# mikemey/cellcomm

Hardware: NVIDIA B200
Metric: BiGAN train cells/sec (higher is better)
Workload: dtype bf16

## Files before the change

cellcomm_b200/csrc/common.cuh:

```cuda
#pragma once
#include <cuda_bf16.h>
#include <cuda_runtime.h>
#include <stdint.h>

#include <atomic>
#include <cstdarg>
#include <cstdio>
#include <string>

#include "../../include/cellcomm_b200.h"

namespace cc {

void set_error(const char* fmt, ...);
extern std::atomic<long long> g_launches;

inline void count_launch(int n = 1) { g_launches.fetch_add(n, std::memory_order_relaxed); }

#define CC_CHECK_CUDA(expr)                                                            \
  do {                                                                                 \
    cudaError_t _e = (expr);                                                           \
    if (_e != cudaSuccess) {                                                           \
      cc::set_error("%s failed: %s (%s:%d)", #expr, cudaGetErrorString(_e), __FILE__,  \
                    __LINE__);                                                         \
      return -2;                                                                       \
    }                                                                                  \
  } while (0)

#define CC_REQUIRE(cond, ...)      \
  do {                             \
    if (!(cond)) {                 \
      cc::set_error(__VA_ARGS__);  \
      return -1;                   \
    }                              \
  } while (0)

#define CC_CHECK_LAUNCH()               \
  do {                                  \
    cc::count_launch();                 \
    CC_CHECK_CUDA(cudaGetLastError());  \
  } while (0)

typedef __nv_bfloat16 bf16;

__device__ __forceinline__ float bf2f(bf16 v) { return __bfloat162float(v); }
__device__ __forceinline__ bf16 f2bf(float v) { return __float2bfloat16_rn(v); }

__device__ __forceinline__ float sigmoidf_(float x) { return 1.f / (1.f + __expf(-x)); }

struct Philox {
  static constexpr uint32_t kM0 = 0xD2511F53u, kM1 = 0xCD9E8D57u;
  static constexpr uint32_t kW0 = 0x9E3779B9u, kW1 = 0xBB67AE85u;
  __host__ __device__ static inline void round(uint32_t (&c)[4], uint32_t k0, uint32_t k1) {
    uint64_t p0 = (uint64_t)kM0 * c[0];
    uint64_t p1 = (uint64_t)kM1 * c[2];
    uint32_t hi0 = (uint32_t)(p0 >> 32), lo0 = (uint32_t)p0;
    uint32_t hi1 = (uint32_t)(p1 >> 32), lo1 = (uint32_t)p1;
    uint32_t n0 = hi1 ^ c[1] ^ k0;
    uint32_t n2 = hi0 ^ c[3] ^ k1;
    c[0] = n0;
    c[1] = lo1;
    c[2] = n2;
    c[3] = lo0;
  }
  __host__ __device__ static inline void block(uint64_t seed, uint64_t ctr_hi, uint64_t ctr_lo,
                                               uint32_t (&out)[4]) {
    uint32_t c[4] = {(uint32_t)ctr_lo, (uint32_t)(ctr_lo >> 32), (uint32_t)ctr_hi,
                     (uint32_t)(ctr_hi >> 32)};
    uint32_t k0 = (uint32_t)seed, k1 = (uint32_t)(seed >> 32);
#pragma unroll
    for (int i = 0; i < 10; ++i) {
      round(c, k0, k1);
      k0 += kW0;
      k1 += kW1;
    }
    out[0] = c[0];
    out[1] = c[1];
    out[2] = c[2];
    out[3] = c[3];
  }
};

__host__ __device__ inline float u32_to_unit(uint32_t x) { return (float)(x >> 8) * (1.0f / 16777216.0f); }

}
```

cellcomm_b200/csrc/gather.cu:

```cuda
#include "common.cuh"

namespace cc {

constexpr int GATHER_THREADS = 256;

__global__ void __launch_bounds__(GATHER_THREADS)
gather_rows_kernel(const long long* __restrict__ rowptr, const int* __restrict__ colidx,
                   const float* __restrict__ values, const long long* __restrict__ row_idx,
                   long long row_start, long long n_rows, long long n_cols,
                   bf16* __restrict__ out16, long long ld16, float* __restrict__ out32,
                   long long ld32, int use_smem) {
  extern __shared__ __align__(16) unsigned char smem[];
  bf16* srow = reinterpret_cast<bf16*>(smem);
  const int tid = threadIdx.x;
  for (long long i = blockIdx.x; i < n_rows; i += gridDim.x) {
    const long long r = row_idx ? row_idx[i] : row_start + i;
    const long long beg = rowptr[r], end = rowptr[r + 1];
    if (out16 != nullptr) {
      bf16* orow = out16 + i * ld16;
      if (use_smem) {
        const long long nvec = n_cols / 8, nz = (n_cols + 7) / 8;
        uint4* s4 = reinterpret_cast<uint4*>(srow);
        for (long long v = tid; v < nz; v += GATHER_THREADS) s4[v] = make_uint4(0, 0, 0, 0);
        __syncthreads();
        for (long long e = beg + tid; e < end; e += GATHER_THREADS)
          srow[colidx[e]] = f2bf(values[e]);
        __syncthreads();
        uint4* o4 = reinterpret_cast<uint4*>(orow);
        for (long long v = tid; v < nvec; v += GATHER_THREADS) o4[v] = s4[v];
        for (long long c = nvec * 8 + tid; c < n_cols; c += GATHER_THREADS) orow[c] = srow[c];
        __syncthreads();
      } else {
        for (long long c = tid; c < n_cols; c += GATHER_THREADS) orow[c] = f2bf(0.f);
        __syncthreads();
        for (long long e = beg + tid; e < end; e += GATHER_THREADS)
          orow[colidx[e]] = f2bf(values[e]);
        __syncthreads();
      }
    }
    if (out32 != nullptr) {
      float* orow = out32 + i * ld32;
      for (long long c = tid; c < n_cols; c += GATHER_THREADS) orow[c] = 0.f;
      __syncthreads();
      for (long long e = beg + tid; e < end; e += GATHER_THREADS) orow[colidx[e]] = values[e];
      __syncthreads();
    }
  }
}

}

extern "C" int cc_gather_rows(const int64_t* rowptr_dev, const int32_t* colidx_dev,
                              const float* values_dev, const int64_t* row_idx_dev,
                              int64_t row_start, int64_t n_rows, int64_t n_cols, void* out16,
                              int64_t ld16, float* out32, int64_t ld32, cc_stream_t stream) {
  using namespace cc;
  if (n_rows <= 0) return 0;
  CC_REQUIRE(out16 == nullptr || ld16 >= n_cols, "cc_gather_rows: ld16 %lld < cols %lld",
             (long long)ld16, (long long)n_cols);
  CC_REQUIRE(out32 == nullptr || ld32 >= n_cols, "cc_gather_rows: ld32 %lld < cols %lld",
             (long long)ld32, (long long)n_cols);
  static int sms = 0, max_smem = 0;
  if (sms == 0) {
    int dev = 0;
    CC_CHECK_CUDA(cudaGetDevice(&dev));
    CC_CHECK_CUDA(cudaDeviceGetAttribute(&sms, cudaDevAttrMultiProcessorCount, dev));
    CC_CHECK_CUDA(cudaDeviceGetAttribute(&max_smem, cudaDevAttrMaxSharedMemoryPerBlockOptin, dev));
    CC_CHECK_CUDA(cudaFuncSetAttribute(gather_rows_kernel,
                                       cudaFuncAttributeMaxDynamicSharedMemorySize, max_smem));
  }
  size_t smem = 0;
  int use_smem = 0;
  if (out16 != nullptr && ld16 % 8 == 0 && (((uintptr_t)out16) & 15) == 0 &&
      (size_t)(n_cols + 7) / 8 * 16 <= (size_t)max_smem) {
    use_smem = 1;
    smem = (size_t)(n_cols + 7) / 8 * 16;
  }
  long long grid = n_rows;
  const long long cap = (long long)sms * 16;
  if (grid > cap) grid = cap;
  gather_rows_kernel<<<(unsigned)grid, GATHER_THREADS, smem, (cudaStream_t)stream>>>(
      (const long long*)rowptr_dev, colidx_dev, values_dev, (const long long*)row_idx_dev,
      row_start, n_rows, n_cols, (bf16*)out16, ld16, out32, ld32, use_smem);
  CC_CHECK_LAUNCH();
  return 0;
}
```

cellcomm_b200/csrc/gemm_sm100.cu:

```cuda
#include <cuda.h>

#include <mutex>
#include <unordered_map>

#include "common.cuh"

namespace cc {

constexpr int BM = 128;
constexpr int BK = 64;
constexpr int UMMA_K = 16;
constexpr int MAX_SEG = CC_GEMM_MAX_SEG;

struct EpiParams {
  int M, N;
  float alpha;
  const float* bias;
  int act;
  const bf16* dact_y;
  long long ld_dact;
  int dact;
  bf16* out16;
  long long ld16;
  int beta16;
  bf16* out16_lo;
  long long ld16_lo;
  float* out32;
  long long ld32;
  int beta32;
  float* rms_p32;
  float* rms_ms;
  float* rms_mom;
  bf16* rms_p16;
  long long rms_ld;
  float rms_lr, rms_rho, rms_momentum, rms_eps;
  int rms_cs;
  int rms_blocked;
  int rms_row0;
  bf16* rms_p16lo;
  int rms_keep_operands;
  int route_world;
  unsigned int route_shard;
  long long route_off0;
  float* route_base[CC_PEER_MAX];
};

struct GemmParams {
  EpiParams epi;
  int nseg;
  int kblocks[MAX_SEG];
  int total_kblocks;
  int kb_per_split;
  int psplits;
  float* partial;
  long long partial_ld;
  long long partial_stride;
  unsigned long long adesc_hi, bdesc_hi;
  unsigned int a_kstep, b_kstep;
  unsigned int idesc;
  int bn_eff;
  int b_boxes;
  int b_half_rows;
  int cluster;
  int pair;
  unsigned int stage_tx;
};

struct TmaMaps {
  CUtensorMap a[MAX_SEG];
  CUtensorMap b[MAX_SEG];
};

__device__ __forceinline__ uint32_t smem_u32(const void* p) {
  return (uint32_t)__cvta_generic_to_shared(p);
}
__device__ __forceinline__ void mbar_init(uint32_t bar, uint32_t count) {
  asm volatile("mbarrier.init.shared::cta.b64 [%0], %1;" ::"r"(bar), "r"(count));
}
__device__ __forceinline__ void mbar_expect_tx(uint32_t bar, uint32_t bytes) {
  asm volatile("mbarrier.arrive.expect_tx.shared::cta.b64 _, [%0], %1;" ::"r"(bar), "r"(bytes)
               : "memory");
}
__device__ __forceinline__ bool mbar_try_wait(uint32_t bar, uint32_t parity) {
  uint32_t ok;
  asm volatile(
      "{\n\t.reg .pred p;\n\t"
      "mbarrier.try_wait.parity.shared::cta.b64 p, [%1], %2;\n\t"
      "selp.u32 %0, 1, 0, p;\n\t}"
      : "=r"(ok)
      : "r"(bar), "r"(parity)
      : "memory");
  return ok != 0;
}
__device__ __forceinline__ void mbar_wait(uint32_t bar, uint32_t parity, int tag) {
  long long t0 = 0;
  uint32_t spins = 0;
  while (!mbar_try_wait(bar, parity)) {
    if (++spins == 4096u) t0 = clock64();
    if (spins > 4096u && (spins & 1023u) == 0 && clock64() - t0 > 4000000000LL) {
      printf("cc_gemm: mbarrier timeout tag=%d block=(%d,%d,%d) thread=%d parity=%u\n", tag,
             blockIdx.x, blockIdx.y, blockIdx.z, threadIdx.x, parity);
      __trap();
    }
  }
}
__device__ __forceinline__ void tma_load_2d(uint32_t dst, const CUtensorMap* map, uint32_t bar,
                                            int c0, int c1) {
  asm volatile(
      "cp.async.bulk.tensor.2d.shared::cluster.global.mbarrier::complete_tx::bytes [%0], [%1, "
      "{%3, %4}], [%2];" ::"r"(dst),
      "l"(map), "r"(bar), "r"(c0), "r"(c1)
      : "memory");
}
__device__ __forceinline__ void tcgen05_fence_before() {
  asm volatile("tcgen05.fence::before_thread_sync;" ::: "memory");
}
__device__ __forceinline__ void tcgen05_fence_after() {
  asm volatile("tcgen05.fence::after_thread_sync;" ::: "memory");
}
__device__ __forceinline__ void umma_bf16(uint32_t tmem_d, uint64_t adesc, uint64_t bdesc,
                                          uint32_t idesc, uint32_t accumulate) {
  asm volatile(
      "{\n\t.reg .pred p;\n\t"
      "setp.ne.b32 p, %4, 0;\n\t"
      "tcgen05.mma.cta_group::1.kind::f16 [%0], %1, %2, %3, p;\n\t}" ::"r"(tmem_d),
      "l"(adesc), "l"(bdesc), "r"(idesc), "r"(accumulate)
      : "memory");
}
__device__ __forceinline__ void umma_commit(uint32_t bar) {
  asm volatile("tcgen05.commit.cta_group::1.mbarrier::arrive::one.shared::cluster.b64 [%0];" ::"r"(
                   bar)
               : "memory");
}
__device__ __forceinline__ void tmem_ld32(uint32_t taddr, uint32_t (&r)[32]) {
  asm volatile(
      "tcgen05.ld.sync.aligned.32x32b.x32.b32 "
      "{%0, %1, %2, %3, %4, %5, %6, %7, %8, %9, %10, %11, %12, %13, %14, %15, "
      "%16, %17, %18, %19, %20, %21, %22, %23, %24, %25, %26, %27, %28, %29, %30, %31}, [%32];"
      : "=r"(r[0]), "=r"(r[1]), "=r"(r[2]), "=r"(r[3]), "=r"(r[4]), "=r"(r[5]), "=r"(r[6]),
        "=r"(r[7]), "=r"(r[8]), "=r"(r[9]), "=r"(r[10]), "=r"(r[11]), "=r"(r[12]), "=r"(r[13]),
        "=r"(r[14]), "=r"(r[15]), "=r"(r[16]), "=r"(r[17]), "=r"(r[18]), "=r"(r[19]),
        "=r"(r[20]), "=r"(r[21]), "=r"(r[22]), "=r"(r[23]), "=r"(r[24]), "=r"(r[25]),
        "=r"(r[26]), "=r"(r[27]), "=r"(r[28]), "=r"(r[29]), "=r"(r[30]), "=r"(r[31])
      : "r"(taddr));
}
__device__ __forceinline__ void tmem_ld_wait() {
  asm volatile("tcgen05.wait::ld.sync.aligned;" ::: "memory");
}

__device__ __forceinline__ bool elect_one() {
  uint32_t pred;
  asm volatile(
      "{\n\t.reg .pred p;\n\t"
      "elect.sync _|p, 0xffffffff;\n\t"
      "selp.u32 %0, 1, 0, p;\n\t}"
      : "=r"(pred));
  return pred != 0;
}

__device__ __forceinline__ void epilogue_store32(const EpiParams& e, int r, int c0, float (&v)[32]) {
  if (r >= e.M) return;
  const int ncols = min(32, e.N - c0);
  if (ncols <= 0) return;
#pragma unroll
  for (int j = 0; j < 32; ++j) {
    float x = v[j] * e.alpha;
    if (e.bias != nullptr && j < ncols) x += __ldg(e.bias + c0 + j);
    if (e.act == CC_ACT_SIGMOID) x = sigmoidf_(x);
    else if (e.act == CC_ACT_RELU) x = fmaxf(x, 0.f);
    v[j] = x;
  }
  if (e.dact != 0) {
    const bf16* yrow = e.dact_y + (long long)r * e.ld_dact + c0;
#pragma unroll
    for (int j = 0; j < 32; ++j) {
      if (j < ncols) {
        float y = bf2f(yrow[j]);
        v[j] *= (e.dact == CC_ACT_SIGMOID) ? y * (1.f - y) : (y > 0.f ? 1.f : 0.f);
      }
    }
  }
  if (e.out32 != nullptr) {
    float* o = e.out32 + (long long)r * e.ld32 + c0;
    if (ncols == 32 && (((uintptr_t)o) & 15) == 0 && !e.beta32) {
#pragma unroll
      for (int j = 0; j < 32; j += 4)
        *reinterpret_cast<float4*>(o + j) = make_float4(v[j], v[j + 1], v[j + 2], v[j + 3]);
    } else {
#pragma unroll
      for (int j = 0; j < 32; ++j)
        if (j < ncols) o[j] = e.beta32 ? o[j] + v[j] : v[j];
    }
  }
  if (e.out16 != nullptr) {
    bf16* o = e.out16 + (long long)r * e.ld16 + c0;
    if (ncols == 32 && (((uintptr_t)o) & 15) == 0 && !e.beta16) {
#pragma unroll
      for (int j = 0; j < 32; j += 8) {
        __nv_bfloat162 p0 = __floats2bfloat162_rn(v[j], v[j + 1]);
        __nv_bfloat162 p1 = __floats2bfloat162_rn(v[j + 2], v[j + 3]);
        __nv_bfloat162 p2 = __floats2bfloat162_rn(v[j + 4], v[j + 5]);
        __nv_bfloat162 p3 = __floats2bfloat162_rn(v[j + 6], v[j + 7]);
        uint4 u;
        u.x = *reinterpret_cast<uint32_t*>(&p0);
        u.y = *reinterpret_cast<uint32_t*>(&p1);
        u.z = *reinterpret_cast<uint32_t*>(&p2);
        u.w = *reinterpret_cast<uint32_t*>(&p3);
        *reinterpret_cast<uint4*>(o + j) = u;
      }
    } else {
#pragma unroll
      for (int j = 0; j < 32; ++j)
        if (j < ncols) o[j] = f2bf(e.beta16 ? bf2f(o[j]) + v[j] : v[j]);
    }
    if (e.out16_lo != nullptr) {
      bf16* l = e.out16_lo + (long long)r * e.ld16_lo + c0;
#pragma unroll
      for (int j = 0; j < 32; ++j)
        if (j < ncols) l[j] = f2bf(v[j] - bf2f(f2bf(v[j])));
    }
  }
}

constexpr int EPI_LD = 36;

__device__ __forceinline__ float4 act4(float4 v, int act) {
  if (act == CC_ACT_SIGMOID) {
// ... 136 lines not shown
          if (e.rms_cs & 1) {
            __stcs(reinterpret_cast<float4*>(e.rms_ms + off), ss);
            __stcs(reinterpret_cast<float4*>(e.rms_mom + off), mm);
            __stcs(reinterpret_cast<float4*>(e.rms_p32 + off), ww);
          } else {
            *reinterpret_cast<float4*>(e.rms_ms + off) = ss;
            *reinterpret_cast<float4*>(e.rms_mom + off) = mm;
            *reinterpret_cast<float4*>(e.rms_p32 + off) = ww;
          }
          if (e.rms_p16 != nullptr) {
            __nv_bfloat162 lo = __floats2bfloat162_rn(ww.x, ww.y);
            __nv_bfloat162 hi = __floats2bfloat162_rn(ww.z, ww.w);
            uint2 u;
            u.x = *reinterpret_cast<uint32_t*>(&lo);
            u.y = *reinterpret_cast<uint32_t*>(&hi);
            *reinterpret_cast<uint2*>(e.rms_p16 + off) = u;
          }
        }
      }
    } else {
      for_each_valid(g, nrow, ncol, [&](int t, int k, float& gv) {
        const long long off = off0 + t * step + k;
        const float ms = e.rms_rho * e.rms_ms[off] + (1.f - e.rms_rho) * gv * gv;
        const float mo = e.rms_momentum * e.rms_mom[off] + e.rms_lr * gv * rsqrtf(ms + e.rms_eps);
        const float w = e.rms_p32[off] - mo;
        e.rms_ms[off] = ms;
        e.rms_mom[off] = mo;
        e.rms_p32[off] = w;
        if (e.rms_p16 != nullptr) e.rms_p16[off] = f2bf(w);
      });
    }
  }
  if (e.route_world > 0) {
    const long long rel0 = e.route_off0 + (long long)rbase * e.ld32 + c;
    const long long step = 4 * e.ld32;
    const unsigned last = (unsigned)e.route_world - 1u;
    const bool vec = ncol == 4 && (e.ld32 & 3) == 0 && ((c & 3) == 0);
#pragma unroll
    for (int t = 0; t < 8; ++t) {
      if (t < nrow) {
        const long long rel = rel0 + t * step;
        const unsigned owner = min((unsigned)((unsigned long long)rel / e.route_shard), last);
        float* dst = e.route_base[owner] + rel;
        if (vec) {
          *reinterpret_cast<float4*>(dst) = g[t];
        } else {
          dst[0] = g[t].x;
          if (ncol > 1) dst[1] = g[t].y;
          if (ncol > 2) dst[2] = g[t].z;
          if (ncol > 3) dst[3] = g[t].w;
        }
      }
    }
  } else if (e.out32 != nullptr) {
    float* o = e.out32 + out32_off + (long long)rbase * e.ld32 + c;
    const long long step = 4 * e.ld32;
    if (ncol == 4 && !e.beta32 && (e.ld32 & 3) == 0 && ((c & 3) == 0) &&
        ((((uintptr_t)e.out32) & 15) == 0)) {
#pragma unroll
      for (int t = 0; t < 8; ++t)
        if (t < nrow) *reinterpret_cast<float4*>(o + t * step) = g[t];
    } else {
      const int beta = e.beta32;
      for_each_valid(g, nrow, ncol, [&](int t, int k, float& gv) {
        float* ot = o + t * step + k;
        *ot = beta ? *ot + gv : gv;
      });
    }
  }
  if (e.out16 != nullptr) {
    bf16* o = e.out16 + (long long)rbase * e.ld16 + c;
    const long long step = 4 * e.ld16;
    if (ncol == 4 && !e.beta16 && (e.ld16 & 3) == 0 && ((c & 3) == 0) &&
        ((((uintptr_t)e.out16) & 7) == 0)) {
#pragma unroll
      for (int t = 0; t < 8; ++t) {
        if (t < nrow) {
          __nv_bfloat162 lo = __floats2bfloat162_rn(g[t].x, g[t].y);
          __nv_bfloat162 hi = __floats2bfloat162_rn(g[t].z, g[t].w);
          uint2 u;
          u.x = *reinterpret_cast<uint32_t*>(&lo);
          u.y = *reinterpret_cast<uint32_t*>(&hi);
          *reinterpret_cast<uint2*>(o + t * step) = u;
        }
      }
    } else {
      const int beta = e.beta16;
      for_each_valid(g, nrow, ncol, [&](int t, int k, float& gv) {
        bf16* ot = o + t * step + k;
        *ot = f2bf(beta ? bf2f(*ot) + gv : gv);
      });
    }
    if (e.out16_lo != nullptr) {
      bf16* l = e.out16_lo + (long long)rbase * e.ld16_lo + c;
      const long long lstep = 4 * e.ld16_lo;
      if (ncol == 4 && (e.ld16_lo & 3) == 0 && ((c & 3) == 0) && ((((uintptr_t)e.out16_lo) & 7) == 0)) {
#pragma unroll
        for (int t = 0; t < 8; ++t) {
          if (t < nrow) {
            const float4 v = g[t];
            __nv_bfloat162 lo = __floats2bfloat162_rn(v.x - bf2f(f2bf(v.x)), v.y - bf2f(f2bf(v.y)));
            __nv_bfloat162 hi = __floats2bfloat162_rn(v.z - bf2f(f2bf(v.z)), v.w - bf2f(f2bf(v.w)));
            uint2 u;
            u.x = *reinterpret_cast<uint32_t*>(&lo);
            u.y = *reinterpret_cast<uint32_t*>(&hi);
            *reinterpret_cast<uint2*>(l + t * lstep) = u;
          }
        }
      } else {
        for_each_valid(g, nrow, ncol, [&](int t, int k, float& gv) {
          l[t * lstep + k] = f2bf(gv - bf2f(f2bf(gv)));
        });
      }
    }
  }
}

template <int BN, int STAGES, bool A_MN, bool B_MN>
__global__ void __launch_bounds__(128, 2)
gemm_tcgen05_kernel(const __grid_constant__ TmaMaps maps, const GemmParams p) {
  constexpr uint32_t A_BYTES = BM * BK * 2;
  constexpr uint32_t B_BYTES = BN * BK * 2;
  constexpr uint32_t STAGE_BYTES = A_BYTES + B_BYTES;
  constexpr uint32_t TMEM_COLS = BN;

  extern __shared__ uint8_t smem_raw[];
  const uint32_t smem_base = (smem_u32(smem_raw) + 1023u) & ~1023u;
  const uint32_t bar_base = smem_base + STAGES * STAGE_BYTES;
  auto full_bar = [&](int s) { return bar_base + 8u * s; };
  auto empty_bar = [&](int s) { return bar_base + 8u * (STAGES + s); };
  const uint32_t tmem_full_bar = bar_base + 8u * (2 * STAGES);
  const uint32_t tmem_slot = bar_base + 8u * (2 * STAGES + 1);
  uint8_t* smem_gen = smem_raw + (smem_base - smem_u32(smem_raw));
  volatile uint32_t* tmem_slot_ptr =
      reinterpret_cast<volatile uint32_t*>(smem_gen + STAGES * STAGE_BYTES + 8u * (2 * STAGES + 1));

  const int warp = threadIdx.x >> 5;
  const int lane = threadIdx.x & 31;
  const int m0 = blockIdx.y * BM;
  const int n0 = blockIdx.x * BN;
  const int kb_begin = blockIdx.z * p.kb_per_split;
  const int kb_end = min(p.total_kblocks, kb_begin + p.kb_per_split);
  const int nkb = kb_end - kb_begin;

  if (threadIdx.x == 0) {
#pragma unroll
    for (int s = 0; s < STAGES; ++s) {
      mbar_init(full_bar(s), 1);
      mbar_init(empty_bar(s), 1);
    }
    mbar_init(tmem_full_bar, 1);
    asm volatile("fence.mbarrier_init.release.cluster;" ::: "memory");
    asm volatile("fence.proxy.async.shared::cta;" ::: "memory");
  }
  if (warp == 1) {
    asm volatile("tcgen05.alloc.cta_group::1.sync.aligned.shared::cta.b32 [%0], %1;" ::"r"(tmem_slot),
                 "r"(TMEM_COLS)
                 : "memory");
    asm volatile("tcgen05.relinquish_alloc_permit.cta_group::1.sync.aligned;" ::: "memory");
  }
  tcgen05_fence_before();
  __syncthreads();
  tcgen05_fence_after();
  const uint32_t tmem_acc = *tmem_slot_ptr;

  if (warp == 0) {
    int seg = 0, kb_in_seg = kb_begin;
    while (seg < p.nseg - 1 && kb_in_seg >= p.kblocks[seg]) {
      kb_in_seg -= p.kblocks[seg];
      ++seg;
    }
    for (int i = 0; i < nkb; ++i) {
      const int s = i % STAGES;
      const uint32_t ph = (uint32_t)(i / STAGES) & 1u;
      mbar_wait(empty_bar(s), ph ^ 1u, 1);
      if (elect_one()) {
        const uint32_t a_dst = smem_base + s * STAGE_BYTES;
        const uint32_t b_dst = a_dst + A_BYTES;
        const int k0 = kb_in_seg * BK;
        mbar_expect_tx(full_bar(s), STAGE_BYTES);
        if (A_MN) {
#pragma unroll
          for (int j = 0; j < BM / 64; ++j)
            tma_load_2d(a_dst + j * (64 * BK * 2), &maps.a[seg], full_bar(s), m0 + 64 * j, k0);
        } else {
          tma_load_2d(a_dst, &maps.a[seg], full_bar(s), k0, m0);
        }
        if (B_MN) {
#pragma unroll
          for (int j = 0; j < BN / 64; ++j)
            tma_load_2d(b_dst + j * (64 * BK * 2), &maps.b[seg], full_bar(s), n0 + 64 * j, k0);
        } else {
          tma_load_2d(b_dst, &maps.b[seg], full_bar(s), k0, n0);
        }
      }
      __syncwarp();
      if (++kb_in_seg >= p.kblocks[seg] && seg < p.nseg - 1) {
        kb_in_seg = 0;
        ++seg;
      }
    }
  } else if (warp == 1) {
    for (int i = 0; i < nkb; ++i) {
      const int s = i % STAGES;
      const uint32_t ph = (uint32_t)(i / STAGES) & 1u;
      mbar_wait(full_bar(s), ph, 2);
      tcgen05_fence_after();
      if (elect_one()) {
        const uint32_t a_src = smem_base + s * STAGE_BYTES;
        const uint32_t b_src = a_src + A_BYTES;
#pragma unroll
        for (int k = 0; k < BK / UMMA_K; ++k) {
          const uint64_t adesc = p.adesc_hi | (uint64_t)(((a_src + k * p.a_kstep) & 0x3FFFFu) >> 4);
          const uint64_t bdesc = p.bdesc_hi | (uint64_t)(((b_src + k * p.b_kstep) & 0x3FFFFu) >> 4);
          umma_bf16(tmem_acc, adesc, bdesc, p.idesc, (i > 0 || k > 0) ? 1u : 0u);
        }
        umma_commit(empty_bar(s));
        if (i == nkb - 1) umma_commit(tmem_full_bar);
      }
      __syncwarp();
    }
  }

  mbar_wait(tmem_full_bar, 0, 3);
  tcgen05_fence_after();
  {
    const int r = m0 + warp * 32 + lane;
    const uint32_t t_row = tmem_acc + ((uint32_t)(warp * 32) << 16);
    const bool split = (p.partial != nullptr);
#pragma unroll 1
    for (int c = 0; c < BN; c += 32) {
      if (n0 + c >= p.epi.N) break;
      uint32_t raw[32];
      tmem_ld32(t_row + (uint32_t)c, raw);
      tmem_ld_wait();
      float v[32];
#pragma unroll
      for (int j = 0; j < 32; ++j) v[j] = __uint_as_float(raw[j]);
      if (split) {
        if (r < p.epi.M) {
          float* o = p.partial + (long long)blockIdx.z * p.partial_stride +
                     (long long)r * p.partial_ld + n0 + c;
#pragma unroll
          for (int j = 0; j < 32; j += 4)
            *reinterpret_cast<float4*>(o + j) = make_float4(v[j], v[j + 1], v[j + 2], v[j + 3]);
        }
      } else {
        epilogue_store32(p.epi, r, n0 + c, v);
      }
    }
  }
  tcgen05_fence_before();
  __syncthreads();
  if (warp == 1) {
    asm volatile("tcgen05.dealloc.cta_group::1.sync.aligned.b32 %0, %1;" ::"r"(tmem_acc),
                 "r"(TMEM_COLS)
                 : "memory");
  }
}

__device__ __forceinline__ void mbar_arrive(uint32_t bar) {
  asm volatile("mbarrier.arrive.shared::cta.b64 _, [%0];" ::"r"(bar) : "memory");
}
__device__ __forceinline__ uint32_t cluster_ctarank() {
  uint32_t r;
  asm volatile("mov.u32 %0, %%cluster_ctarank;" : "=r"(r));
  return r;
}
__device__ __forceinline__ void cluster_sync_all() {
  asm volatile("barrier.cluster.arrive.release.aligned;" ::: "memory");
  asm volatile("barrier.cluster.wait.acquire.aligned;" ::: "memory");
}
__device__ __forceinline__ void tma_load_2d_mc(uint32_t dst, const CUtensorMap* map, uint32_t bar,
                                               int c0, int c1, uint16_t mask) {
  asm volatile(
      "cp.async.bulk.tensor.2d.shared::cluster.global.mbarrier::complete_tx::bytes"
      ".multicast::cluster [%0], [%1, {%3, %4}], [%2], %5;" ::"r"(dst),
      "l"(map), "r"(bar), "r"(c0), "r"(c1), "h"(mask)
      : "memory");
}
__device__ __forceinline__ uint64_t l2_policy_evict_last() {
  uint64_t pol;
  asm volatile("createpolicy.fractional.L2::evict_last.b64 %0, 1.0;" : "=l"(pol));
  return pol;
}
__device__ __forceinline__ void tma_load_2d_pol(uint32_t dst, const CUtensorMap* map, uint32_t bar,
                                                int c0, int c1, uint64_t pol) {
  asm volatile(
      "cp.async.bulk.tensor.2d.shared::cluster.global.mbarrier::complete_tx::bytes.L2::cache_hint "
      "[%0], [%1, {%3, %4}], [%2], %5;" ::"r"(dst),
      "l"(map), "r"(bar), "r"(c0), "r"(c1), "l"(pol)
      : "memory");
}
__device__ __forceinline__ void tma_load_2d_mc_pol(uint32_t dst, const CUtensorMap* map,
                                                   uint32_t bar, int c0, int c1, uint16_t mask,
                                                   uint64_t pol) {
  asm volatile(
      "cp.async.bulk.tensor.2d.shared::cluster.global.mbarrier::complete_tx::bytes"
      ".multicast::cluster.L2::cache_hint [%0], [%1, {%3, %4}], [%2], %5, %6;" ::"r"(dst),
      "l"(map), "r"(bar), "r"(c0), "r"(c1), "h"(mask), "l"(pol)
      : "memory");
}
__device__ __forceinline__ void umma_commit_mc(uint32_t bar, uint16_t mask) {
  asm volatile(
      "tcgen05.commit.cta_group::1.mbarrier::arrive::one.shared::cluster.multicast::cluster.b64 "
      "[%0], %1;" ::"r"(bar),
      "h"(mask)
      : "memory");
}

__device__ __forceinline__ uint32_t mapa_cluster(uint32_t local, uint32_t cta) {
  uint32_t r;
  asm volatile("mapa.shared::cluster.u32 %0, %1, %2;" : "=r"(r) : "r"(local), "r"(cta));
  return r;
}
__device__ __forceinline__ void mbar_arrive_cluster(uint32_t cluster_addr) {
  asm volatile("mbarrier.arrive.release.cluster.shared::cluster.b64 _, [%0];" ::"r"(cluster_addr)
// ... 10 lines not shown
__device__ __forceinline__ void umma_bf16_pair(uint32_t tmem_d, uint64_t adesc, uint64_t bdesc,
                                               uint32_t idesc, uint32_t accumulate) {
  asm volatile(
      "{\n\t.reg .pred p;\n\t"
      "setp.ne.b32 p, %4, 0;\n\t"
      "tcgen05.mma.cta_group::2.kind::f16 [%0], %1, %2, %3, p;\n\t}" ::"r"(tmem_d),
      "l"(adesc), "l"(bdesc), "r"(idesc), "r"(accumulate)
      : "memory");
}
__device__ __forceinline__ void umma_commit_pair(uint32_t bar, uint16_t mask) {
  asm volatile(
      "tcgen05.commit.cta_group::2.mbarrier::arrive::one.shared::cluster.multicast::cluster.b64 "
      "[%0], %1;" ::"r"(bar),
      "h"(mask)
      : "memory");
}

__device__ __forceinline__ void rms_blocked_chunk(const EpiParams& e, int lane, int r0, int c0,
                                                  const uint32_t (&raw)[32]) {
  const int r = r0 + lane;
  if (r >= e.M) return;
  const int row = e.rms_row0 + r;
  const long long sb =
      ((long long)(row >> 5) * (e.rms_ld >> 5) + (c0 >> 5)) * 1024 + (long long)(row & 31) * 4;
  float* pw = e.rms_p32 + sb;
  float* ps = e.rms_ms + sb;
  float* pm = e.rms_mom + sb;
  float4 w[8], s[8], m[8];
#pragma unroll
  for (int t = 0; t < 8; ++t) {
    w[t] = __ldcs(reinterpret_cast<const float4*>(pw + t * 128));
    s[t] = __ldcs(reinterpret_cast<const float4*>(ps + t * 128));
    m[t] = __ldcs(reinterpret_cast<const float4*>(pm + t * 128));
  }
  const float rho = e.rms_rho, omr = 1.f - e.rms_rho, mu = e.rms_momentum, lr = e.rms_lr,
              eps = e.rms_eps;
  const int nvalid = e.N - c0;
  uint32_t h[16], hl[16];
#pragma unroll
  for (int t = 0; t < 8; ++t) {
    float g0 = (4 * t + 0 < nvalid) ? __uint_as_float(raw[4 * t + 0]) : 0.f;
    float g1 = (4 * t + 1 < nvalid) ? __uint_as_float(raw[4 * t + 1]) : 0.f;
    float g2 = (4 * t + 2 < nvalid) ? __uint_as_float(raw[4 * t + 2]) : 0.f;
    float g3 = (4 * t + 3 < nvalid) ? __uint_as_float(raw[4 * t + 3]) : 0.f;
    float4 ss, mm, ww;
    ss.x = rho * s[t].x + omr * g0 * g0;
    ss.y = rho * s[t].y + omr * g1 * g1;
    ss.z = rho * s[t].z + omr * g2 * g2;
    ss.w = rho * s[t].w + omr * g3 * g3;
    mm.x = mu * m[t].x + lr * g0 * rsqrtf(ss.x + eps);
    mm.y = mu * m[t].y + lr * g1 * rsqrtf(ss.y + eps);
    mm.z = mu * m[t].z + lr * g2 * rsqrtf(ss.z + eps);
    mm.w = mu * m[t].w + lr * g3 * rsqrtf(ss.w + eps);
    ww.x = w[t].x - mm.x;
    ww.y = w[t].y - mm.y;
    ww.z = w[t].z - mm.z;
    ww.w = w[t].w - mm.w;
    __stcs(reinterpret_cast<float4*>(ps + t * 128), ss);
    __stcs(reinterpret_cast<float4*>(pm + t * 128), mm);
    __stcs(reinterpret_cast<float4*>(pw + t * 128), ww);
    __nv_bfloat162 lo = __floats2bfloat162_rn(ww.x, ww.y);
    __nv_bfloat162 hi = __floats2bfloat162_rn(ww.z, ww.w);
    h[2 * t] = *reinterpret_cast<uint32_t*>(&lo);
    h[2 * t + 1] = *reinterpret_cast<uint32_t*>(&hi);
    if (e.rms_p16lo != nullptr) {
      __nv_bfloat162 l0 = __floats2bfloat162_rn(ww.x - __uint_as_float(h[2 * t] << 16),
                                                ww.y - __uint_as_float(h[2 * t] & 0xFFFF0000u));
      __nv_bfloat162 l1 = __floats2bfloat162_rn(ww.z - __uint_as_float(h[2 * t + 1] << 16),
                                                ww.w - __uint_as_float(h[2 * t + 1] & 0xFFFF0000u));
      hl[2 * t] = *reinterpret_cast<uint32_t*>(&l0);
      hl[2 * t + 1] = *reinterpret_cast<uint32_t*>(&l1);
    }
    if (e.out32 != nullptr)
      *reinterpret_cast<float4*>(e.out32 + (long long)r * e.ld32 + c0 + 4 * t) =
          make_float4(g0, g1, g2, g3);
  }
  if (e.rms_p16 != nullptr) {
    uint4* dst = reinterpret_cast<uint4*>(e.rms_p16 + (long long)r * e.rms_ld + c0);
#pragma unroll
    for (int t = 0; t < 4; ++t) dst[t] = make_uint4(h[4 * t], h[4 * t + 1], h[4 * t + 2], h[4 * t + 3]);
  }
  if (e.rms_p16lo != nullptr) {
    uint4* dst = reinterpret_cast<uint4*>(e.rms_p16lo + (long long)r * e.rms_ld + c0);
#pragma unroll
    for (int t = 0; t < 4; ++t)
      dst[t] = make_uint4(hl[4 * t], hl[4 * t + 1], hl[4 * t + 2], hl[4 * t + 3]);
  }
}

template <int BN, int STAGES, bool A_MN, bool B_MN, bool MATH, int EPI_WARPS, bool N_FAST = false,
          int CLUSTER = 1, bool PAIR = false, bool RMS_DIRECT = false>
__global__ void __launch_bounds__(64 + 32 * EPI_WARPS, 1)
gemm_tcgen05_persistent_kernel(const __grid_constant__ TmaMaps maps,
                               const __grid_constant__ GemmParams p,
                               const int tiles_m, const int tiles_n) {
  static_assert(!PAIR || CLUSTER == 2, "a CTA pair is a cluster of two");
  constexpr uint32_t A_BYTES = BM * BK * 2;
  constexpr uint32_t B_BYTES = (PAIR ? BN / 2 : BN) * BK * 2;
  constexpr uint32_t STAGE_BYTES = A_BYTES + B_BYTES;
  constexpr uint32_t TMEM_COLS = 2 * BN;
  static_assert(TMEM_COLS <= 512, "TMEM has 512 columns");
  static_assert(CLUSTER == 1 || CLUSTER == 2, "cluster of 1 or 2 CTAs");

  extern __shared__ uint8_t smem_raw[];
  const uint32_t smem_base = (smem_u32(smem_raw) + 1023u) & ~1023u;
  const uint32_t bar_base = smem_base + STAGES * STAGE_BYTES;
  auto full_bar = [&](int s) { return bar_base + 8u * s; };
  auto empty_bar = [&](int s) { return bar_base + 8u * (STAGES + s); };
  auto tfull_bar = [&](int a) { return bar_base + 8u * (2 * STAGES + a); };
  auto tempty_bar = [&](int a) { return bar_base + 8u * (2 * STAGES + 2 + a); };
  const uint32_t tmem_slot = bar_base + 8u * (2 * STAGES + 4);
  uint8_t* smem_gen = smem_raw + (smem_base - smem_u32(smem_raw));
  volatile uint32_t* tmem_slot_ptr =
      reinterpret_cast<volatile uint32_t*>(smem_gen + STAGES * STAGE_BYTES + 8u * (2 * STAGES + 4));
  float* epi_stage = reinterpret_cast<float*>(smem_gen + STAGES * STAGE_BYTES + 8u * (2 * STAGES + 6));

  const int warp = threadIdx.x >> 5;
  const int lane = threadIdx.x & 31;
  const int nkb = p.total_kblocks;
  const int rank = (CLUSTER == 2) ? (int)cluster_ctarank() : 0;
  const int tiles_mu = (tiles_m + CLUSTER - 1) / CLUSTER;
  const int num_tiles = tiles_mu * tiles_n;
  const int psplits = p.psplits > 1 ? p.psplits : 1;
  const int num_units = num_tiles * psplits;
  const int unit0 = (int)blockIdx.x / CLUSTER, unit_step = (int)gridDim.x / CLUSTER;
  auto unit_tile = [&](int u) { return psplits > 1 ? u % num_tiles : u; };
  auto unit_split = [&](int u) { return psplits > 1 ? u / num_tiles : 0; };
  auto unit_m0 = [&](int u) {
    const int t = unit_tile(u);
    return ((N_FAST ? t / tiles_n : t % tiles_mu) * CLUSTER + rank) * BM;
  };
  auto unit_n0 = [&](int u) {
    const int t = unit_tile(u);
    return (N_FAST ? t % tiles_n : t / tiles_mu) * p.bn_eff;
  };
  auto unit_kb0 = [&](int u) { return unit_split(u) * p.kb_per_split; };
  auto unit_nkb = [&](int u) {
    return psplits > 1 ? min(p.kb_per_split, p.total_kblocks - unit_kb0(u)) : p.total_kblocks;
  };

  if (threadIdx.x == 0) {
#pragma unroll
    for (int s = 0; s < STAGES; ++s) {
      mbar_init(full_bar(s), PAIR ? 2 : 1);
      mbar_init(empty_bar(s), PAIR ? 1 : CLUSTER);
    }
#pragma unroll
    for (int a = 0; a < 2; ++a) {
      mbar_init(tfull_bar(a), 1);
      mbar_init(tempty_bar(a), PAIR ? 2 * EPI_WARPS : EPI_WARPS);
    }
    asm volatile("fence.mbarrier_init.release.cluster;" ::: "memory");
    asm volatile("fence.proxy.async.shared::cta;" ::: "memory");
  }
  if (warp == 1) {
    if (PAIR) {
      asm volatile("tcgen05.alloc.cta_group::2.sync.aligned.shared::cta.b32 [%0], %1;" ::"r"(tmem_slot),
                   "r"(TMEM_COLS)
                   : "memory");
      asm volatile("tcgen05.relinquish_alloc_permit.cta_group::2.sync.aligned;" ::: "memory");
    } else {
      asm volatile("tcgen05.alloc.cta_group::1.sync.aligned.shared::cta.b32 [%0], %1;" ::"r"(tmem_slot),
                   "r"(TMEM_COLS)
                   : "memory");
      asm volatile("tcgen05.relinquish_alloc_permit.cta_group::1.sync.aligned;" ::: "memory");
    }
  }
  tcgen05_fence_before();
  __syncthreads();
  if (CLUSTER == 2) cluster_sync_all();
  tcgen05_fence_after();
  const uint32_t tmem_acc = *tmem_slot_ptr;

  if (warp == 0 && PAIR) {
    uint32_t it = 0;
    const int half = p.bn_eff / 2;
    for (int u = unit0; u < num_units; u += unit_step) {
      const int m0 = unit_m0(u), n0 = unit_n0(u) + rank * half;
      int seg = 0, kb_in_seg = 0;
      for (int i = 0; i < nkb; ++i, ++it) {
        const int s = it % STAGES;
        const uint32_t ph = (it / STAGES) & 1u;
        mbar_wait(empty_bar(s), ph ^ 1u, 11);
        if (elect_one()) {
          const uint32_t a_dst = smem_base + s * STAGE_BYTES;
          const uint32_t b_dst = a_dst + A_BYTES;
          const uint32_t lbar = mapa_cluster(full_bar(s), 0);
          const int k0 = kb_in_seg * BK;
          if (rank == 0) mbar_expect_tx(full_bar(s), 2 * p.stage_tx);
          else mbar_arrive_cluster(lbar);
          if (A_MN) {
#pragma unroll
            for (int j = 0; j < BM / 64; ++j)
              tma_load_2d_pair(a_dst + j * (64 * BK * 2), &maps.a[seg], lbar, m0 + 64 * j, k0);
          } else {
            tma_load_2d_pair(a_dst, &maps.a[seg], lbar, k0, m0);
          }
          if (B_MN) {
#pragma unroll
            for (int j = 0; j < BN / 128; ++j)
              if (j < p.b_boxes)
                tma_load_2d_pair(b_dst + j * (64 * BK * 2), &maps.b[seg], lbar, n0 + 64 * j, k0);
          } else {
            tma_load_2d_pair(b_dst, &maps.b[seg], lbar, k0, n0);
          }
        }
        __syncwarp();
        if (++kb_in_seg >= p.kblocks[seg] && seg < p.nseg - 1) {
          kb_in_seg = 0;
          ++seg;
        }
      }
    }
  } else if (warp == 0) {
    uint32_t it = 0;
    const uint64_t keep = (RMS_DIRECT && p.epi.rms_keep_operands) ? l2_policy_evict_last() : 0;
    for (int u = unit0; u < num_units; u += unit_step) {
      const int m0 = unit_m0(u), n0 = unit_n0(u);
      const int nkb_u = unit_nkb(u);
      int seg = 0, kb_in_seg = unit_kb0(u);
      while (seg < p.nseg - 1 && kb_in_seg >= p.kblocks[seg]) {
        kb_in_seg -= p.kblocks[seg];
        ++seg;
      }
      for (int i = 0; i < nkb_u; ++i, ++it) {
        const int s = it % STAGES;
        const uint32_t ph = (it / STAGES) & 1u;
        mbar_wait(empty_bar(s), ph ^ 1u, 11);
        if (elect_one()) {
          const uint32_t a_dst = smem_base + s * STAGE_BYTES;
          const uint32_t b_dst = a_dst + A_BYTES;
          const int k0 = kb_in_seg * BK;
          mbar_expect_tx(full_bar(s), p.stage_tx);
          if (RMS_DIRECT && A_MN && B_MN && keep != 0) {
#pragma unroll
            for (int j = 0; j < BM / 64; ++j)
              tma_load_2d_pol(a_dst + j * (64 * BK * 2), &maps.a[seg], full_bar(s), m0 + 64 * j, k0,
                              keep);
#pragma unroll
            for (int j = 0; j < BN / 64; ++j) {
              if (j >= p.b_boxes) continue;
              if (CLUSTER == 2) {
                if ((j & 1) == rank)
                  tma_load_2d_mc_pol(b_dst + j * (64 * BK * 2), &maps.b[seg], full_bar(s),
                                     n0 + 64 * j, k0, (uint16_t)3, keep);
              } else {
                tma_load_2d_pol(b_dst + j * (64 * BK * 2), &maps.b[seg], full_bar(s), n0 + 64 * j,
                                k0, keep);
              }
            }
          } else if (A_MN) {
#pragma unroll
            for (int j = 0; j < BM / 64; ++j)
              tma_load_2d(a_dst + j * (64 * BK * 2), &maps.a[seg], full_bar(s), m0 + 64 * j, k0);
          } else {
            tma_load_2d(a_dst, &maps.a[seg], full_bar(s), k0, m0);
          }
          if (RMS_DIRECT && A_MN && B_MN && keep != 0) {
          } else if (CLUSTER == 2) {
            if (B_MN) {
#pragma unroll
              for (int j = 0; j < BN / 64; ++j)
                if (j < p.b_boxes && (j & 1) == rank)
                  tma_load_2d_mc(b_dst + j * (64 * BK * 2), &maps.b[seg], full_bar(s), n0 + 64 * j,
                                 k0, (uint16_t)3);
            } else {
              tma_load_2d_mc(b_dst + rank * p.b_half_rows * (BK * 2), &maps.b[seg], full_bar(s), k0,
                             n0 + rank * p.b_half_rows, (uint16_t)3);
            }
          } else if (B_MN) {
#pragma unroll
            for (int j = 0; j < BN / 64; ++j)
              if (j < p.b_boxes)
                tma_load_2d(b_dst + j * (64 * BK * 2), &maps.b[seg], full_bar(s), n0 + 64 * j, k0);
          } else {
            tma_load_2d(b_dst, &maps.b[seg], full_bar(s), k0, n0);
          }
        }
        __syncwarp();
        if (++kb_in_seg >= p.kblocks[seg] && seg < p.nseg - 1) {
          kb_in_seg = 0;
          ++seg;
        }
      }
    }
  } else if (warp == 1) {
    uint32_t it = 0, tl = 0;
    for (int u = unit0; (!PAIR || rank == 0) && u < num_units; u += unit_step, ++tl) {
      const uint32_t acc = tl & 1u, aph = (tl >> 1) & 1u;
      mbar_wait(tempty_bar(acc), aph ^ 1u, 12);
      tcgen05_fence_after();
      const uint32_t d_tmem = tmem_acc + acc * BN;
      const int nkb = unit_nkb(u);
      for (int i = 0; i < nkb; ++i, ++it) {
        const int s = it % STAGES;
        const uint32_t ph = (it / STAGES) & 1u;
        mbar_wait(full_bar(s), ph, 13);
        tcgen05_fence_after();
        if (elect_one()) {
          const uint32_t a_src = smem_base + s * STAGE_BYTES;
          const uint32_t b_src = a_src + A_BYTES;
#pragma unroll
          for (int k = 0; k < BK / UMMA_K; ++k) {
            const uint64_t adesc = p.adesc_hi | (uint64_t)(((a_src + k * p.a_kstep) & 0x3FFFFu) >> 4);
            const uint64_t bdesc = p.bdesc_hi | (uint64_t)(((b_src + k * p.b_kstep) & 0x3FFFFu) >> 4);
            if (PAIR) umma_bf16_pair(d_tmem, adesc, bdesc, p.idesc, (i > 0 || k > 0) ? 1u : 0u);
            else umma_bf16(d_tmem, adesc, bdesc, p.idesc, (i > 0 || k > 0) ? 1u : 0u);
          }
          if (PAIR) {
            umma_commit_pair(empty_bar(s), (uint16_t)3);
            if (i == nkb - 1) umma_commit_pair(tfull_bar(acc), (uint16_t)3);
          } else {
            if (CLUSTER == 2) umma_commit_mc(empty_bar(s), (uint16_t)3);
            else umma_commit(empty_bar(s));
            if (i == nkb - 1) umma_commit(tfull_bar(acc));
          }
        }
        __syncwarp();
      }
    }
  } else {
    const int q = warp & 3;
    const int ew = warp - 2;
    constexpr int COLS_PER_WARP = BN / (EPI_WARPS / 4);
    const int col_lo = (ew >> 2) * COLS_PER_WARP;
    uint32_t tl = 0;
    for (int u = unit0; u < num_units; u += unit_step, ++tl) {
      const int m0 = unit_m0(u), n0 = unit_n0(u);
      const uint32_t acc = tl & 1u, aph = (tl >> 1) & 1u;
      mbar_wait(tfull_bar(acc), aph, 14);
      tcgen05_fence_after();
      const uint32_t t_row = tmem_acc + ((uint32_t)(q * 32) << 16) + acc * BN;
      if (m0 < p.epi.M) {
#pragma unroll 1
        for (int c = col_lo; c < col_lo + COLS_PER_WARP; c += 32) {
          if (c >= p.bn_eff || n0 + c >= p.epi.N) break;
          uint32_t raw[32];
          tmem_ld32(t_row + (uint32_t)c, raw);
          tmem_ld_wait();
          if constexpr (RMS_DIRECT) rms_blocked_chunk(p.epi, lane, m0 + q * 32, n0 + c, raw);
          else epilogue_chunk<MATH>(p.epi, epi_stage + ew * (32 * EPI_LD), lane, m0 + q * 32, n0 + c, raw,
                                    (long long)unit_split(u) * p.partial_stride);
        }
      }
      tcgen05_fence_before();
      __syncwarp();
      if (lane == 0) {
        if (PAIR) mbar_arrive_cluster(mapa_cluster(tempty_bar(acc), 0));
        else mbar_arrive(tempty_bar(acc));
      }
    }
  }
  tcgen05_fence_before();
  __syncthreads();
  if (CLUSTER == 2) cluster_sync_all();
  if (warp == 1) {
    if (PAIR)
      asm volatile("tcgen05.dealloc.cta_group::2.sync.aligned.b32 %0, %1;" ::"r"(tmem_acc),
                   "r"(TMEM_COLS)
                   : "memory");
    else
      asm volatile("tcgen05.dealloc.cta_group::1.sync.aligned.b32 %0, %1;" ::"r"(tmem_acc),
                   "r"(TMEM_COLS)
                   : "memory");
  }
}

}
#include "wgrad_rmsprop_kernel.cuh"
namespace cc {

__global__ void splitk_finalize_kernel(const EpiParams e, const float* __restrict__ partial,
                                       long long partial_ld, long long partial_stride, int splits) {
  const int groups = (e.N + 3) / 4;
  const long long idx = (long long)blockIdx.x * blockDim.x + threadIdx.x;
  if (idx >= (long long)e.M * groups) return;
  const int r = (int)(idx / groups);
  const int c0 = (int)(idx % groups) * 4;
  const float* src = partial + (long long)r * partial_ld + c0;
  float4 a = make_float4(0.f, 0.f, 0.f, 0.f);
  for (int s0 = 0; s0 < splits; s0 += 8) {
    float4 q[8];
#pragma unroll
    for (int u = 0; u < 8; ++u)
      q[u] = (s0 + u < splits)
                 ? __ldcs(reinterpret_cast<const float4*>(src + (long long)(s0 + u) * partial_stride))
                 : make_float4(0.f, 0.f, 0.f, 0.f);
#pragma unroll
    for (int u = 0; u < 8; ++u) {
      if (s0 + u < splits) {
        a.x += q[u].x;
        a.y += q[u].y;
        a.z += q[u].z;
        a.w += q[u].w;
      }
    }
  }
  float v[4] = {a.x, a.y, a.z, a.w};
  const int ncols = min(4, e.N - c0);
#pragma unroll
  for (int j = 0; j < 4; ++j) {
    float x = v[j] * e.alpha;
    if (e.bias != nullptr && j < ncols) x += __ldg(e.bias + c0 + j);
    if (e.act == CC_ACT_SIGMOID) x = sigmoidf_(x);
    else if (e.act == CC_ACT_RELU) x = fmaxf(x, 0.f);
    v[j] = x;
  }
  if (e.dact != 0) {
    const bf16* yrow = e.dact_y + (long long)r * e.ld_dact + c0;
#pragma unroll
    for (int j = 0; j < 4; ++j) {
      if (j < ncols) {
        const float y = bf2f(yrow[j]);
        v[j] *= (e.dact == CC_ACT_SIGMOID) ? y * (1.f - y) : (y > 0.f ? 1.f : 0.f);
      }
    }
  }
  if (e.out32 != nullptr) {
    float* o = e.out32 + (long long)r * e.ld32 + c0;
    if (ncols == 4 && (((uintptr_t)o) & 15) == 0 && !e.beta32) {
      *reinterpret_cast<float4*>(o) = make_float4(v[0], v[1], v[2], v[3]);
    } else {
#pragma unroll
      for (int j = 0; j < 4; ++j)
        if (j < ncols) o[j] = e.beta32 ? o[j] + v[j] : v[j];
    }
  }
  if (e.out16 != nullptr) {
    bf16* o = e.out16 + (long long)r * e.ld16 + c0;
    if (ncols == 4 && (((uintptr_t)o) & 7) == 0 && !e.beta16) {
      __nv_bfloat162 p0 = __floats2bfloat162_rn(v[0], v[1]);
      __nv_bfloat162 p1 = __floats2bfloat162_rn(v[2], v[3]);
      uint2 u;
      u.x = *reinterpret_cast<uint32_t*>(&p0);
      u.y = *reinterpret_cast<uint32_t*>(&p1);
      *reinterpret_cast<uint2*>(o) = u;
    } else {
#pragma unroll
      for (int j = 0; j < 4; ++j)
        if (j < ncols) o[j] = f2bf(e.beta16 ? bf2f(o[j]) + v[j] : v[j]);
    }
    if (e.out16_lo != nullptr) {
      bf16* l = e.out16_lo + (long long)r * e.ld16_lo + c0;
#pragma unroll
      for (int j = 0; j < 4; ++j)
        if (j < ncols) l[j] = f2bf(v[j] - bf2f(f2bf(v[j])));
    }
  }
}

typedef CUresult (*PFN_encodeTiled)(CUtensorMap*, CUtensorMapDataType, cuuint32_t, void*,
                                    const cuuint64_t*, const cuuint64_t*, const cuuint32_t*,
                                    const cuuint32_t*, CUtensorMapInterleave, CUtensorMapSwizzle,
                                    CUtensorMapL2promotion, CUtensorMapFloatOOBfill);

static PFN_encodeTiled get_encode_fn() {
  static PFN_encodeTiled fn = nullptr;
  static std::once_flag once;
  std::call_once(once, [] {
    void* ptr = nullptr;
    cudaDriverEntryPointQueryResult qres;
    if (cudaGetDriverEntryPoint("cuTensorMapEncodeTiled", &ptr, cudaEnableDefault, &qres) ==
            cudaSuccess &&
        qres == cudaDriverEntryPointSuccess)
      fn = (PFN_encodeTiled)ptr;
  });
  return fn;
}

struct MapKey {
  const void* ptr;
  uint64_t inner, outer, ld;
  uint32_t box_inner, box_outer;
  uint32_t kind;
  bool operator==(const MapKey& o) const {
    return ptr == o.ptr && inner == o.inner && outer == o.outer && ld == o.ld &&
           box_inner == o.box_inner && box_outer == o.box_outer && kind == o.kind;
  }
};
struct MapKeyHash {
  size_t operator()(const MapKey& k) const {
    uint64_t h = (uint64_t)(uintptr_t)k.ptr * 0x9E3779B97F4A7C15ull;
    h ^= k.inner + 0x9E3779B97F4A7C15ull + (h << 6) + (h >> 2);
    h ^= k.outer + 0x9E3779B97F4A7C15ull + (h << 6) + (h >> 2);
    h ^= k.ld + 0x9E3779B97F4A7C15ull + (h << 6) + (h >> 2);
    h ^= ((uint64_t)k.box_inner << 32 | k.box_outer) + 0x9E3779B97F4A7C15ull + (h << 6) + (h >> 2);
    h ^= k.kind + 0x9E3779B97F4A7C15ull + (h << 6) + (h >> 2);
    return (size_t)h;
  }
};

enum MapKind : uint32_t {
  MAP_BF16_SW128 = 0,
  MAP_F32_SW128 = 1,
  MAP_BF16_SW64 = 2,
  MAP_F32_SW128_L2_256 = 3
};

static int make_map_kind(CUtensorMap* out, const void* ptr, uint64_t inner, uint64_t outer,
                         uint64_t ld, uint32_t box_inner, uint32_t box_outer, MapKind kind) {
  static std::mutex mu;
  static std::unordered_map<MapKey, CUtensorMap, MapKeyHash> cache;
  MapKey key{ptr, inner, outer, ld, box_inner, box_outer, (uint32_t)kind};
  {
    std::lock_guard<std::mutex> g(mu);
    auto it = cache.find(key);
    if (it != cache.end()) {
      *out = it->second;
      return 0;
    }
  }
  const bool f32 = kind == MAP_F32_SW128 || kind == MAP_F32_SW128_L2_256;
  const uint64_t esize = f32 ? 4 : 2;
  PFN_encodeTiled enc = get_encode_fn();
  CC_REQUIRE(enc != nullptr, "cuTensorMapEncodeTiled is unavailable (no CUDA driver?)");
  CC_REQUIRE(((uintptr_t)ptr & 15) == 0, "cc_gemm: operand base %p is not 16-byte aligned", ptr);
  CC_REQUIRE((ld * esize) % 16 == 0, "cc_gemm: operand ld=%llu is not a multiple of 16 bytes",
             (unsigned long long)ld);
  CC_REQUIRE(inner > 0 && outer > 0, "cc_gemm: empty operand");
  cuuint64_t dims[2] = {inner, outer};
  cuuint64_t strides[1] = {ld * esize};
  cuuint32_t box[2] = {box_inner, box_outer};
  cuuint32_t estr[2] = {1, 1};
  CUresult r = enc(out,
                   f32 ? CU_TENSOR_MAP_DATA_TYPE_FLOAT32 : CU_TENSOR_MAP_DATA_TYPE_BFLOAT16,
                   2, const_cast<void*>(ptr), dims, strides, box, estr,
                   CU_TENSOR_MAP_INTERLEAVE_NONE,
                   kind == MAP_BF16_SW64 ? CU_TENSOR_MAP_SWIZZLE_64B : CU_TENSOR_MAP_SWIZZLE_128B,
                   (kind == MAP_BF16_SW128 || kind == MAP_F32_SW128_L2_256)
                       ? CU_TENSOR_MAP_L2_PROMOTION_L2_256B
                       : CU_TENSOR_MAP_L2_PROMOTION_L2_128B,
                   CU_TENSOR_MAP_FLOAT_OOB_FILL_NONE);
  CC_REQUIRE(r == CUDA_SUCCESS,
             "cuTensorMapEncodeTiled failed (%d) ptr=%p inner=%llu outer=%llu ld=%llu box=%ux%u",
             (int)r, ptr, (unsigned long long)inner, (unsigned long long)outer,
             (unsigned long long)ld, box_inner, box_outer);
  {
    std::lock_guard<std::mutex> g(mu);
    if (cache.size() > (1u << 16)) cache.clear();
    cache.emplace(key, *out);
  }
  return 0;
}

static int make_map(CUtensorMap* out, const void* ptr, uint64_t inner, uint64_t outer, uint64_t ld,
                    uint32_t box_inner, uint32_t box_outer) {
  return make_map_kind(out, ptr, inner, outer, ld, box_inner, box_outer, MAP_BF16_SW128);
}

static uint64_t desc_hi(uint32_t lbo_bytes, uint32_t sbo_bytes) {
  uint64_t d = 0;
  d |= (uint64_t)((lbo_bytes >> 4) & 0x3FFF) << 16;
  d |= (uint64_t)((sbo_bytes >> 4) & 0x3FFF) << 32;
  d |= (uint64_t)1 << 46;
  d |= (uint64_t)2 << 61;
  return d;
}

static int env_int(const char* name, int dflt) {
  const char* v = getenv(name);
  return v ? atoi(v) : dflt;
}

struct GemmEnv {
  int sms;
  int bn;
  int splits;
  int persistent;
  int cluster;
  int rms_cluster;
  int bn_eff;
  int mn_lbo;
  int mn_sbo;
  int mn_kstep;
  int k_lbo;
  int k_sbo;
  int rms_cs;
  int rms_warps;
  int rms_nfast;
  int rms_tma;
  int rms_p16_tma;
  int rms_interleave;
  int rms_pair;
  int pair;
  int rms_l2_256;
  int rms_keep;
  int persistent_splitk;
};
static GemmEnv g_env;
static std::atomic<int> g_env_state{0};
static std::mutex g_env_mu;
static int g_num_sms = 0;

static const GemmEnv& gemm_env() {
  if (g_env_state.load(std::memory_order_acquire) == 0) {
    std::lock_guard<std::mutex> lock(g_env_mu);
    GemmEnv e;
    e.sms = env_int("CC_GEMM_SMS", 0);
    e.bn = env_int("CC_GEMM_BN", 0);
    e.splits = env_int("CC_GEMM_SPLITS", 0);
    e.persistent = env_int("CC_GEMM_PERSISTENT", 1);
    e.cluster = env_int("CC_GEMM_CLUSTER", 2);
    e.rms_cluster = env_int("CC_GEMM_RMS_CLUSTER", -1);
    e.bn_eff = env_int("CC_GEMM_BN_EFF", 0);
    e.mn_lbo = env_int("CC_GEMM_MN_LBO", 64 * BK * 2);
    e.mn_sbo = env_int("CC_GEMM_MN_SBO", 1024);
    e.mn_kstep = env_int("CC_GEMM_MN_KSTEP", UMMA_K * 128);
    e.k_lbo = env_int("CC_GEMM_K_LBO", 16);
    e.k_sbo = env_int("CC_GEMM_K_SBO", 1024);
    e.rms_cs = env_int("CC_GEMM_RMS_CS", 1);
    e.rms_warps = env_int("CC_GEMM_RMS_WARPS", 8);
    e.rms_nfast = env_int("CC_GEMM_RMS_NFAST", -1);
    e.rms_tma = env_int("CC_GEMM_RMS_TMA", -1);
    e.rms_p16_tma = env_int("CC_GEMM_RMS_P16_TMA", 0);
    e.rms_interleave = env_int("CC_GEMM_RMS_INTERLEAVE", 1);
    e.rms_pair = env_int("CC_GEMM_RMS_PAIR", 0);
    e.pair = env_int("CC_GEMM_PAIR", 0);
    e.rms_l2_256 = env_int("CC_GEMM_RMS_L2_256", 0);
    e.rms_keep = env_int("CC_GEMM_RMS_KEEP_OPERANDS", 0);
    e.persistent_splitk = env_int("CC_GEMM_PERSISTENT_SPLITK", 1);
    g_env = e;
    g_env_state.store(1, std::memory_order_release);
  }
  return g_env;
}

template <int BN, int STAGES>
static constexpr size_t smem_bytes() {
  return (size_t)STAGES * (BM * BK * 2 + BN * BK * 2) + 8 * (2 * STAGES + 2) + 1024;
}

template <int BN, int STAGES, bool A_MN, bool B_MN>
static int launch_cfg(const TmaMaps& maps, const GemmParams& p, dim3 grid, cudaStream_t st) {
  auto kern = gemm_tcgen05_kernel<BN, STAGES, A_MN, B_MN>;
  static bool attr_set = false;
  constexpr size_t smem = smem_bytes<BN, STAGES>();
  if (!attr_set) {
    CC_CHECK_CUDA(cudaFuncSetAttribute(kern, cudaFuncAttributeMaxDynamicSharedMemorySize, (int)smem));
    attr_set = true;
  }
  kern<<<grid, 128, smem, st>>>(maps, p);
  CC_CHECK_LAUNCH();
  return 0;
}

template <int BN, int STAGES>
static int launch_major(const TmaMaps& maps, const GemmParams& p, dim3 grid, bool a_mn, bool b_mn,
                        cudaStream_t st) {
  if (!a_mn && b_mn) return launch_cfg<BN, STAGES, false, true>(maps, p, grid, st);
  if (!a_mn && !b_mn) return launch_cfg<BN, STAGES, false, false>(maps, p, grid, st);
  if (a_mn && b_mn) return launch_cfg<BN, STAGES, true, true>(maps, p, grid, st);
  return launch_cfg<BN, STAGES, true, false>(maps, p, grid, st);
}

template <int BN, int STAGES, int EPI_WARPS, bool PAIR = false, bool RMS_DIRECT = false>
static constexpr size_t smem_bytes_persistent() {
  return (size_t)STAGES * (BM * BK * 2 + (PAIR ? BN / 2 : BN) * BK * 2) + 8 * (2 * STAGES + 6) + 16 +
         (RMS_DIRECT ? 0 : EPI_WARPS * 32 * EPI_LD * 4) + 1024;
}

template <int BN, int STAGES, bool A_MN, bool B_MN, bool MATH, int EPI_WARPS, bool N_FAST, int CLUSTER,
          bool PAIR = false, bool RMS_DIRECT = false>
static int launch_persistent_one(const TmaMaps& maps, const GemmParams& p, int mt, int nt,
                                 int num_sms, cudaStream_t st) {
  auto kern = gemm_tcgen05_persistent_kernel<BN, STAGES, A_MN, B_MN, MATH, EPI_WARPS, N_FAST, CLUSTER,
                                             PAIR, RMS_DIRECT>;
  static bool attr_set = false;
  static int max_ctas = 0;
  constexpr size_t smem = smem_bytes_persistent<BN, STAGES, EPI_WARPS, PAIR, RMS_DIRECT>();
  static_assert(smem <= 232448, "shared memory per CTA");
  constexpr int threads = 64 + 32 * EPI_WARPS;
  if (!attr_set) {
    CC_CHECK_CUDA(cudaFuncSetAttribute(kern, cudaFuncAttributeMaxDynamicSharedMemorySize, (int)smem));
    max_ctas = num_sms;
    if (CLUSTER > 1) {
      cudaLaunchConfig_t q{};
      q.gridDim = dim3((unsigned)(num_sms / CLUSTER * CLUSTER));
      q.blockDim = dim3(threads);
      q.dynamicSmemBytes = smem;
      cudaLaunchAttribute qa[1];
      qa[0].id = cudaLaunchAttributeClusterDimension;
      qa[0].val.clusterDim.x = CLUSTER;
      qa[0].val.clusterDim.y = 1;
      qa[0].val.clusterDim.z = 1;
      q.attrs = qa;
      q.numAttrs = 1;
      int nclusters = 0;
      CC_CHECK_CUDA(cudaOccupancyMaxActiveClusters(&nclusters, kern, &q));
      CC_REQUIRE(nclusters >= 1, "cc_gemm: no %d-CTA cluster fits on this device", CLUSTER);
      if (nclusters * CLUSTER < max_ctas) max_ctas = nclusters * CLUSTER;
    }
    attr_set = true;
  }
  const int units = ((mt + CLUSTER - 1) / CLUSTER) * nt * (p.psplits > 1 ? p.psplits : 1);
  int grid = units * CLUSTER < max_ctas ? units * CLUSTER : max_ctas / CLUSTER * CLUSTER;
  cudaLaunchConfig_t cfg{};
  cfg.gridDim = dim3((unsigned)grid);
  cfg.blockDim = dim3(threads);
  cfg.dynamicSmemBytes = smem;
  cfg.stream = st;
  cudaLaunchAttribute attr[1];
  attr[0].id = cudaLaunchAttributeClusterDimension;
  attr[0].val.clusterDim.x = CLUSTER;
  attr[0].val.clusterDim.y = 1;
  attr[0].val.clusterDim.z = 1;
  cfg.attrs = attr;
  cfg.numAttrs = 1;
  CC_CHECK_CUDA(cudaLaunchKernelEx(&cfg, kern, maps, p, mt, nt));
  count_launch();
  return 0;
}

template <int BN, int STAGES, int EPI_WARPS>
static constexpr int pair_stages() {
  return BN == 256 ? (EPI_WARPS == 8 ? 5 : 6) : STAGES;
}

template <int BN, int STAGES, bool A_MN, bool B_MN, bool MATH, int EPI_WARPS = 4, bool N_FAST = false>
static int launch_persistent_cfg(const TmaMaps& maps, const GemmParams& p, int mt, int nt,
                                 int num_sms, cudaStream_t st) {
  if (BN == 256 && p.cluster == 2 && p.pair)
    return launch_persistent_one<BN, pair_stages<BN, STAGES, EPI_WARPS>(), A_MN, B_MN, MATH, EPI_WARPS,
                                 N_FAST, 2, BN == 256>(maps, p, mt, nt, num_sms, st);
  if (p.cluster == 2)
    return launch_persistent_one<BN, STAGES, A_MN, B_MN, MATH, EPI_WARPS, N_FAST, 2>(maps, p, mt, nt, num_sms, st);
  return launch_persistent_one<BN, STAGES, A_MN, B_MN, MATH, EPI_WARPS, N_FAST, 1>(maps, p, mt, nt, num_sms, st);
}

template <int BN, int STAGES, bool MATH>
static int launch_persistent_m(const TmaMaps& maps, const GemmParams& p, int mt, int nt,
                               int num_sms, bool a_mn, bool b_mn, cudaStream_t st) {
  if (!a_mn && b_mn) return launch_persistent_cfg<BN, STAGES, false, true, MATH>(maps, p, mt, nt, num_sms, st);
  if (!a_mn && !b_mn) return launch_persistent_cfg<BN, STAGES, false, false, MATH>(maps, p, mt, nt, num_sms, st);
  if (a_mn && b_mn) return launch_persistent_cfg<BN, STAGES, true, true, MATH>(maps, p, mt, nt, num_sms, st);
  return launch_persistent_cfg<BN, STAGES, true, false, MATH>(maps, p, mt, nt, num_sms, st);
}

template <int BN, int STAGES>
static int launch_persistent(const TmaMaps& maps, const GemmParams& p, int mt, int nt, int num_sms,
                             bool a_mn, bool b_mn, cudaStream_t st) {
  const EpiParams& e = p.epi;
  const bool math = e.alpha != 1.f || e.bias != nullptr || e.act != 0 || e.dact != 0;
  if (math) return launch_persistent_m<BN, STAGES, true>(maps, p, mt, nt, num_sms, a_mn, b_mn, st);
  return launch_persistent_m<BN, STAGES, false>(maps, p, mt, nt, num_sms, a_mn, b_mn, st);
}

template <bool N_FAST, int CLUSTER, bool PAIR = false>
static int launch_rms_tma(const RmsMaps& maps, const GemmParams& p, int mt, int nt, int num_sms,
                          cudaStream_t st) {
  static_assert(!PAIR || CLUSTER == 2, "the CTA pair is a cluster of two");
  void (*kern)(const RmsMaps, const GemmParams, const int, const int);
  if (PAIR) kern = wgrad_rmsprop_pair_kernel<N_FAST>;
  else kern = wgrad_rmsprop_tma_kernel<N_FAST, CLUSTER>;
  static bool attr_set = false;
  static int max_ctas = 0;
  constexpr size_t smem = PAIR ? RMSP_SMEM_BYTES : RMS_SMEM_BYTES;
  constexpr int threads = 64 + 32 * RMS_EPI_WARPS;
  if (!attr_set) {
    CC_CHECK_CUDA(cudaFuncSetAttribute(kern, cudaFuncAttributeMaxDynamicSharedMemorySize, (int)smem));
    max_ctas = num_sms;
    if (CLUSTER > 1) {
      cudaLaunchConfig_t q{};
      q.gridDim = dim3((unsigned)(num_sms / CLUSTER * CLUSTER));
      q.blockDim = dim3(threads);
      q.dynamicSmemBytes = smem;
      cudaLaunchAttribute qa[1];
      qa[0].id = cudaLaunchAttributeClusterDimension;
      qa[0].val.clusterDim.x = CLUSTER;
      qa[0].val.clusterDim.y = 1;
      qa[0].val.clusterDim.z = 1;
      q.attrs = qa;
      q.numAttrs = 1;
      int nclusters = 0;
      CC_CHECK_CUDA(cudaOccupancyMaxActiveClusters(&nclusters, kern, &q));
      CC_REQUIRE(nclusters >= 1, "cc_gemm: no %d-CTA cluster fits on this device", CLUSTER);
      if (nclusters * CLUSTER < max_ctas) max_ctas = nclusters * CLUSTER;
    }
    attr_set = true;
  }
  const int units = ((mt + CLUSTER - 1) / CLUSTER) * nt;
  int grid = units * CLUSTER < max_ctas ? units * CLUSTER : max_ctas / CLUSTER * CLUSTER;
  cudaLaunchConfig_t cfg{};
  cfg.gridDim = dim3((unsigned)grid);
  cfg.blockDim = dim3(threads);
  cfg.dynamicSmemBytes = smem;
  cfg.stream = st;
  cudaLaunchAttribute attr[1];
  attr[0].id = cudaLaunchAttributeClusterDimension;
  attr[0].val.clusterDim.x = CLUSTER;
  attr[0].val.clusterDim.y = 1;
  attr[0].val.clusterDim.z = 1;
  cfg.attrs = attr;
  cfg.numAttrs = 1;
  CC_CHECK_CUDA(cudaLaunchKernelEx(&cfg, kern, maps, p, mt, nt));
  count_launch();
  return 0;
}

int gemm_impl(const cc_gemm_desc* d, cudaStream_t st) {
  const GemmEnv& ENV = gemm_env();
  CC_REQUIRE(d != nullptr, "cc_gemm: null descriptor");
  CC_REQUIRE(d->M > 0 && d->N > 0, "cc_gemm: empty output %dx%d", d->M, d->N);
  CC_REQUIRE(d->nseg >= 1 && d->nseg <= MAX_SEG, "cc_gemm: nseg=%d out of range", d->nseg);
  CC_REQUIRE(d->out16 != nullptr || d->out32 != nullptr || d->rms_p32 != nullptr,
             "cc_gemm: no output");
  CC_REQUIRE(d->rms_p32 == nullptr || (d->rms_ms != nullptr && d->rms_mom != nullptr),
             "cc_gemm: fused RMSprop needs ms and mom");
  CC_REQUIRE(d->route_world >= 0 && d->route_world <= CC_PEER_MAX, "cc_gemm: route_world=%d",
             d->route_world);
  CC_REQUIRE(d->out16_lo == nullptr || (d->out16 != nullptr && d->beta16 == 0),
             "cc_gemm: out16_lo needs a plain out16 (the high-order term)");
  if (d->rms_blocked) {
    CC_REQUIRE(d->rms_p32 != nullptr && d->a_mn_major && d->b_mn_major && d->N > 128 &&
                   d->alpha == 1.f && d->bias == nullptr && d->act == 0 && d->dact_y == nullptr &&
                   d->out16 == nullptr && d->beta32 == 0 && d->route_world == 0 &&
                   d->force_splits <= 1 && (d->force_bn == 0 || d->force_bn == 256),
               "cc_gemm: rms_blocked is for plain weight-gradient GEMMs (X^T dZ, N > 128)");
    CC_REQUIRE(d->rms_row0 >= 0 && (d->rms_ld & 31) == 0 &&
                   ((((uintptr_t)d->rms_p32) | ((uintptr_t)d->rms_ms) | ((uintptr_t)d->rms_mom) |
                     ((uintptr_t)d->rms_p16) | ((uintptr_t)d->rms_p16_lo) | ((uintptr_t)d->out32)) & 15) == 0 &&
                   (d->out32 == nullptr || (d->ld32 & 3) == 0),
               "cc_gemm: rms_blocked needs 16-byte aligned blocks, rms_ld %% 32 == 0 (rms_ld=%lld)",
               (long long)d->rms_ld);
  }
  CC_REQUIRE(d->rms_p16_lo == nullptr || d->rms_blocked,
             "cc_gemm: rms_p16_lo is written by the blocked fused-optimiser epilogue only");
  if (d->route_world > 0) {
    CC_REQUIRE(d->out32 != nullptr && d->beta32 == 0 && d->workspace == nullptr &&
                   d->rms_p32 == nullptr,
               "cc_gemm: a routed output needs a plain fp32 output without split-K");
    CC_REQUIRE(d->route_shard > 0 && (d->route_shard & 7) == 0 && d->route_shard < (1ll << 32) &&
                   d->route_off0 >= 0 && (d->route_off0 & 3) == 0,
               "cc_gemm: route_shard=%lld route_off0=%lld", (long long)d->route_shard,
               (long long)d->route_off0);
    for (int q = 0; q < d->route_world; ++q)
      CC_REQUIRE(d->route_base[q] != nullptr, "cc_gemm: route_base[%d] is null", q);
  }
  if (g_num_sms == 0) {
    int dev = 0;
    CC_CHECK_CUDA(cudaGetDevice(&dev));
    CC_CHECK_CUDA(cudaDeviceGetAttribute(&g_num_sms, cudaDevAttrMultiProcessorCount, dev));
    const int cap = ENV.sms;
    if (cap >= 2 && cap < g_num_sms) g_num_sms = cap / 2 * 2;
  }
  const bool a_mn = d->a_mn_major != 0, b_mn = d->b_mn_major != 0;

  int bn = d->force_bn ? d->force_bn : ENV.bn;
  if (bn == 0) bn = (d->N > 128) ? 256 : 128;
  CC_REQUIRE(bn == 128 || bn == 256, "cc_gemm: BN=%d unsupported", bn);

  GemmParams p{};
  TmaMaps maps;
  memset(&maps, 0, sizeof(maps));
  p.nseg = d->nseg;
  int total = 0;
  for (int s = 0; s < d->nseg; ++s) {
    CC_REQUIRE(d->k[s] > 0, "cc_gemm: segment %d has k=%d", s, d->k[s]);
    p.kblocks[s] = (d->k[s] + BK - 1) / BK;
    total += p.kblocks[s];
  }
  p.total_kblocks = total;

  const int mt = (d->M + BM - 1) / BM;
  int nt = (d->N + bn - 1) / bn;
  int splits = 1;
  const long long Mpad = (long long)mt * BM, Npad = (long long)nt * bn;
  if (d->workspace != nullptr && d->rms_p32 == nullptr) {
    int want = d->force_splits ? d->force_splits : ENV.splits;
    if (want == 0) {
      const int tiles = mt * nt;
      if (2 * tiles <= g_num_sms && total >= 8) {
        want = (2 * g_num_sms) / tiles;
        if (want < 1) want = 1;
        if (want > total / 4) want = total / 4;
      } else {
        want = 1;
      }
    }
    if (want > total) want = total;
    const long long cap = d->workspace_elems / (Mpad * Npad);
    if (want > cap) want = (int)cap;
    if (want >= 2) splits = want;
  }
  p.kb_per_split = (total + splits - 1) / splits;
  splits = (total + p.kb_per_split - 1) / p.kb_per_split;
  if (splits >= 2) {
    p.partial = d->workspace;
    p.partial_ld = Npad;
    p.partial_stride = Mpad * Npad;
  } else {
    p.partial = nullptr;
    p.kb_per_split = total;
    splits = 1;
  }
  const bool psk = splits >= 2 && ENV.persistent != 0 && ENV.persistent_splitk != 0;
  const bool persistent =
      (splits == 1 || psk) && (ENV.persistent != 0 || d->rms_p32 != nullptr ||
                               d->route_world > 0);

  const bool rms_cluster = ENV.rms_cluster < 0 ? total > 8 : ENV.rms_cluster != 0;
  p.cluster = (persistent && mt >= 2 && ENV.cluster == 2 &&
               (d->rms_p32 == nullptr || rms_cluster)) ? 2 : 1;
  int bn_eff = bn;
  if (persistent && bn == 256 && d->rms_p32 == nullptr && splits == 1) {
    const int forced = ENV.bn_eff;
    if (forced >= 32 && forced <= 256 && forced % 32 == 0) {
      bn_eff = forced;
    } else {
      long long best = -1;
      const int mu = (mt + p.cluster - 1) / p.cluster, slots = g_num_sms / p.cluster;
      for (int cand = 256; cand >= 128; cand -= 64) {
        const long long units = (long long)mu * ((d->N + cand - 1) / cand);
        const long long cost = ((units + slots - 1) / slots) * (cand + 128);
        if (best < 0 || cost < best) {
          best = cost;
          bn_eff = cand;
        }
      }
    }
    nt = (d->N + bn_eff - 1) / bn_eff;
  }
  p.bn_eff = bn_eff;
  p.b_boxes = (bn_eff + 63) / 64;
  p.b_half_rows = bn_eff / 2;
  p.stage_tx = (unsigned)(BM * BK * 2 + (b_mn ? p.b_boxes * 64 * BK * 2 : bn_eff * BK * 2));
  p.pair = (p.cluster == 2 && bn == 256 && ENV.pair != 0 && splits == 1 &&
            (b_mn ? bn_eff % 128 == 0 : bn_eff % 32 == 0)) ? 1 : 0;
  if (p.pair) {
    p.b_boxes = bn_eff / 128;
    p.stage_tx = (unsigned)(BM * BK * 2 + (bn_eff / 2) * BK * 2);
  }

  for (int s = 0; s < d->nseg; ++s) {
    int rc;
    if (a_mn)
      rc = make_map(&maps.a[s], d->a[s], (uint64_t)d->M, (uint64_t)d->k[s], (uint64_t)d->lda[s], 64, BK);
    else
      rc = make_map(&maps.a[s], d->a[s], (uint64_t)d->k[s], (uint64_t)d->M, (uint64_t)d->lda[s], BK, BM);
    if (rc) return rc;
    if (b_mn)
      rc = make_map(&maps.b[s], d->b[s], (uint64_t)d->N, (uint64_t)d->k[s], (uint64_t)d->ldb[s], 64, BK);
    else
      rc = make_map(&maps.b[s], d->b[s], (uint64_t)d->k[s], (uint64_t)d->N, (uint64_t)d->ldb[s], BK,
                    (uint32_t)(persistent ? (p.cluster == 2 ? bn_eff / 2 : bn_eff) : bn));
    if (rc) return rc;
  }

  const uint32_t mn_lbo = (uint32_t)ENV.mn_lbo;
  const uint32_t mn_sbo = (uint32_t)ENV.mn_sbo;
  const uint32_t mn_kstep = (uint32_t)ENV.mn_kstep;
  const uint32_t k_lbo = (uint32_t)ENV.k_lbo;
  const uint32_t k_sbo = (uint32_t)ENV.k_sbo;
  p.adesc_hi = a_mn ? desc_hi(mn_lbo, mn_sbo) : desc_hi(k_lbo, k_sbo);
  p.bdesc_hi = b_mn ? desc_hi(mn_lbo, mn_sbo) : desc_hi(k_lbo, k_sbo);
  p.a_kstep = a_mn ? mn_kstep : UMMA_K * 2;
  p.b_kstep = b_mn ? mn_kstep : UMMA_K * 2;
  p.idesc = (1u << 4) | (1u << 7) | (1u << 10) | ((a_mn ? 1u : 0u) << 15) |
            ((b_mn ? 1u : 0u) << 16) | ((uint32_t)((persistent ? bn_eff : bn) >> 3) << 17) |
            ((uint32_t)(((persistent && p.pair) ? 2 * BM : BM) >> 4) << 24);

  EpiParams& e = p.epi;
  e.M = d->M;
  e.N = d->N;
  e.alpha = d->alpha;
  e.bias = d->bias;
  e.act = d->act;
  e.dact_y = (const bf16*)d->dact_y;
  e.ld_dact = d->ld_dact;
  e.dact = d->dact_y ? d->dact : 0;
  e.out16 = (bf16*)d->out16;
  e.ld16 = d->ld16;
  e.beta16 = d->beta16;
  e.out16_lo = (bf16*)d->out16_lo;
  e.ld16_lo = d->ld16_lo;
  e.out32 = d->out32;
  e.ld32 = d->ld32;
  e.beta32 = d->beta32;
  e.rms_p32 = d->rms_p32;
  e.rms_ms = d->rms_ms;
  e.rms_mom = d->rms_mom;
  e.rms_p16 = (bf16*)d->rms_p16;
  e.rms_ld = d->rms_ld;
  e.rms_lr = d->rms_lr;
  e.rms_rho = d->rms_rho;
  e.rms_momentum = d->rms_momentum;
  e.rms_eps = d->rms_eps;
  e.rms_cs = (ENV.rms_cs ? 1 : 0) | (ENV.rms_l2_256 ? 8 : 0);
  e.rms_blocked = d->rms_blocked;
  e.rms_row0 = d->rms_row0;
  e.rms_p16lo = d->rms_blocked ? (bf16*)d->rms_p16_lo : nullptr;
  e.rms_keep_operands = ENV.rms_keep;
  e.route_world = d->route_world;
  e.route_shard = (unsigned)d->route_shard;
  e.route_off0 = d->route_off0;
  for (int q = 0; q < CC_PEER_MAX; ++q)
    e.route_base[q] = q < d->route_world ? d->route_base[q] : nullptr;

  if (persistent) {
    if (bn == 256 && d->rms_p32 != nullptr && a_mn && b_mn && d->alpha == 1.f &&
        d->bias == nullptr && d->act == 0 && e.dact == 0 && ENV.rms_warps == 8) {
      int nfast = ENV.rms_nfast;
      if (nfast < 0) nfast = ((long long)total * BK * d->N * 2 <= (48ll << 20)) ? 1 : 0;
      if (d->rms_blocked) {
        if (p.cluster == 2)
          return nfast ? launch_persistent_one<256, 4, true, true, false, 8, true, 2, false, true>(
                             maps, p, mt, nt, g_num_sms, st)
                       : launch_persistent_one<256, 4, true, true, false, 8, false, 2, false, true>(
                             maps, p, mt, nt, g_num_sms, st);
        return nfast ? launch_persistent_one<256, 4, true, true, false, 8, true, 1, false, true>(
                           maps, p, mt, nt, g_num_sms, st)
                     : launch_persistent_one<256, 4, true, true, false, 8, false, 1, false, true>(
                           maps, p, mt, nt, g_num_sms, st);
      }
      int use_tma = ENV.rms_tma;
      if (use_tma < 0) use_tma = total <= 4 ? 1 : 0;
      const bool tma_ok =
          use_tma != 0 && (d->rms_ld & 7) == 0 && d->beta32 == 0 &&
          ((((uintptr_t)d->rms_p32) | ((uintptr_t)d->rms_ms) | ((uintptr_t)d->rms_mom) |
            ((uintptr_t)d->rms_p16)) & 15) == 0 && d->out16 == nullptr;
      if (tma_ok) {
        RmsMaps rm;
        memset(&rm, 0, sizeof(rm));
        for (int s = 0; s < d->nseg; ++s) {
          rm.a[s] = maps.a[s];
          rm.b[s] = maps.b[s];
        }
        const MapKind sk = ENV.rms_l2_256 ? MAP_F32_SW128_L2_256 : MAP_F32_SW128;
        int rc = make_map_kind(&rm.p32, d->rms_p32, (uint64_t)d->N, (uint64_t)d->M,
                               (uint64_t)d->rms_ld, 32, 32, sk);
        if (!rc) rc = make_map_kind(&rm.ms, d->rms_ms, (uint64_t)d->N, (uint64_t)d->M,
                                    (uint64_t)d->rms_ld, 32, 32, sk);
        if (!rc) rc = make_map_kind(&rm.mom, d->rms_mom, (uint64_t)d->N, (uint64_t)d->M,
                                    (uint64_t)d->rms_ld, 32, 32, sk);
        if (!rc && d->rms_p16 != nullptr)
          rc = make_map_kind(&rm.p16, d->rms_p16, (uint64_t)d->N, (uint64_t)d->M,
                             (uint64_t)d->rms_ld, 32, 32, MAP_BF16_SW64);
        if (rc) return rc;
        if (ENV.rms_p16_tma == 0) p.epi.rms_cs |= 2;
        if (ENV.rms_interleave != 0) p.epi.rms_cs |= 4;
        p.idesc = (p.idesc & ~(0x1Fu << 24)) | ((uint32_t)(BM >> 4) << 24);
        if (p.cluster == 2 && ENV.rms_pair != 0)
          return nfast ? launch_rms_tma<true, 2, true>(rm, p, mt, nt, g_num_sms, st)
                       : launch_rms_tma<false, 2, true>(rm, p, mt, nt, g_num_sms, st);
        if (p.cluster == 2)
          return nfast ? launch_rms_tma<true, 2>(rm, p, mt, nt, g_num_sms, st)
                       : launch_rms_tma<false, 2>(rm, p, mt, nt, g_num_sms, st);
        return nfast ? launch_rms_tma<true, 1>(rm, p, mt, nt, g_num_sms, st)
                     : launch_rms_tma<false, 1>(rm, p, mt, nt, g_num_sms, st);
      }
      if (nfast != 0)
        return launch_persistent_cfg<256, 3, true, true, false, 8, true>(maps, p, mt, nt, g_num_sms, st);
      return launch_persistent_cfg<256, 3, true, true, false, 8>(maps, p, mt, nt, g_num_sms, st);
    }
    if (splits >= 2) {
      CC_REQUIRE(d->rms_p32 == nullptr, "cc_gemm: fused RMSprop is not available with split-K");
      GemmParams pp = p;
      pp.psplits = splits;
      EpiParams pe{};
      pe.M = d->M;
      pe.N = d->N;
      pe.alpha = 1.f;
      pe.out32 = p.partial;
      pe.ld32 = p.partial_ld;
      pp.epi = pe;
      int rc = bn == 256
                   ? launch_persistent_m<256, 4, false>(maps, pp, mt, nt, g_num_sms, a_mn, b_mn, st)
                   : launch_persistent_m<128, 6, false>(maps, pp, mt, nt, g_num_sms, a_mn, b_mn, st);
      if (rc) return rc;
      const long long work = (long long)d->M * ((d->N + 3) / 4);
      const int threads = 256;
      splitk_finalize_kernel<<<(unsigned)((work + threads - 1) / threads), threads, 0, st>>>(
          p.epi, p.partial, p.partial_ld, p.partial_stride, splits);
      CC_CHECK_LAUNCH();
      return 0;
    }
    if (bn == 256) return launch_persistent<256, 4>(maps, p, mt, nt, g_num_sms, a_mn, b_mn, st);
    return launch_persistent<128, 6>(maps, p, mt, nt, g_num_sms, a_mn, b_mn, st);
  }
  CC_REQUIRE(d->rms_p32 == nullptr, "cc_gemm: fused RMSprop is not available with split-K");

  dim3 grid((unsigned)nt, (unsigned)mt, (unsigned)splits);
  int rc;
  if (bn == 256)
    rc = launch_major<256, 2>(maps, p, grid, a_mn, b_mn, st);
  else
    rc = launch_major<128, 3>(maps, p, grid, a_mn, b_mn, st);
  if (rc) return rc;
  if (splits >= 2) {
    const long long work = (long long)d->M * ((d->N + 3) / 4);
    const int threads = 256;
    splitk_finalize_kernel<<<(unsigned)((work + threads - 1) / threads), threads, 0, st>>>(
        p.epi, p.partial, p.partial_ld, p.partial_stride, splits);
    CC_CHECK_LAUNCH();
  }
  return 0;
}

}

extern "C" void cc_reload_env(void) {
  std::lock_guard<std::mutex> lock(cc::g_env_mu);
  cc::g_env_state.store(0, std::memory_order_release);
  cc::g_num_sms = 0;
}

extern "C" int cc_gemm(const cc_gemm_desc* desc, cc_stream_t stream) {
  return cc::gemm_impl(desc, (cudaStream_t)stream);
}

extern "C" int64_t cc_gemm_workspace_elems(int32_t M, int32_t N) {
  const long long Mpad = ((long long)M + 127) / 128 * 128, Npad = ((long long)N + 255) / 256 * 256;
  long long a = 296LL * 128 * 256 * 2;
  long long b = 8 * Mpad * Npad;
  return a > b ? a : b;
}
```

cellcomm_b200/csrc/generate.cu:

```cuda
#include "common.cuh"

namespace cc {

constexpr int kFillVec = 4;

__device__ __forceinline__ float4 load_vec4(const float* __restrict__ row, long long c,
                                            long long cols, bool vec) {
  if (vec) return *reinterpret_cast<const float4*>(row + c);
  float4 v = make_float4(0.f, 0.f, 0.f, 0.f);
  if (c + 0 < cols) v.x = row[c + 0];
  if (c + 1 < cols) v.y = row[c + 1];
  if (c + 2 < cols) v.z = row[c + 2];
  if (c + 3 < cols) v.w = row[c + 3];
  return v;
}

__device__ __forceinline__ void round4(float4 v, long long c, long long cols, float (&f)[4]) {
  f[0] = rintf(v.x);
  f[1] = rintf(v.y);
  f[2] = rintf(v.z);
  f[3] = rintf(v.w);
#pragma unroll
  for (int k = 0; k < 4; ++k)
    if (c + k >= cols) f[k] = 0.f;
}

__device__ __forceinline__ int nz4(const float (&f)[4]) {
  return (f[0] != 0.f) + (f[1] != 0.f) + (f[2] != 0.f) + (f[3] != 0.f);
}

template <typename T>
__device__ __forceinline__ T block_inclusive_scan(T v, T* scratch, T* total) {
  const int lane = threadIdx.x & 31, warp = threadIdx.x >> 5, nwarps = blockDim.x >> 5;
#pragma unroll
  for (int o = 1; o < 32; o <<= 1) {
    const T u = __shfl_up_sync(0xffffffffu, v, o);
    if (lane >= o) v += u;
  }
  if (lane == 31) scratch[warp] = v;
  __syncthreads();
  if (warp == 0) {
    T w = lane < nwarps ? scratch[lane] : T(0);
#pragma unroll
    for (int o = 1; o < 32; o <<= 1) {
      const T u = __shfl_up_sync(0xffffffffu, w, o);
      if (lane >= o) w += u;
    }
    scratch[lane] = w;
  }
  __syncthreads();
  if (warp > 0) v += scratch[warp - 1];
  *total = scratch[nwarps - 1];
  __syncthreads();
  return v;
}

template <bool VEC>
__global__ void __launch_bounds__(512, 4)
round_csr_count_kernel(const float* __restrict__ x, long long ldx, long long cols,
                       long long* __restrict__ rowptr) {
  __shared__ long long scratch[32];
  const long long r = blockIdx.x;
  const float* row = x + r * ldx;
  long long n = 0;
  for (long long c = 4ll * threadIdx.x; c < cols; c += 4ll * blockDim.x) {
    float f[4];
    round4(load_vec4(row, c, cols, VEC), c, cols, f);
    n += nz4(f);
  }
  long long total;
  block_inclusive_scan(n, scratch, &total);
  if (threadIdx.x == 0) rowptr[1 + r] = total;
}

__global__ void __launch_bounds__(1024)
round_csr_scan_kernel(long long rows, long long* __restrict__ rowptr) {
  __shared__ long long scratch[32];
  long long carry = rowptr[0];
  for (long long r0 = 0; r0 < rows; r0 += blockDim.x) {
    const long long r = r0 + threadIdx.x;
    const long long v = r < rows ? rowptr[1 + r] : 0;
    long long total;
    const long long incl = block_inclusive_scan(v, scratch, &total);
    if (r < rows) rowptr[1 + r] = carry + incl;
    carry += total;
  }
}

template <bool VEC>
__global__ void __launch_bounds__(512, 2)
round_csr_fill_kernel(const float* __restrict__ x, long long ldx, long long cols,
                      const long long* __restrict__ rowptr, int* __restrict__ colidx,
                      float* __restrict__ values) {
  static_assert(kFillVec <= 4, "four 16-bit count fields in a uint64");
  __shared__ unsigned long long scratch[32];
  const long long r = blockIdx.x;
  const float* row = x + r * ldx;
  long long out = rowptr[r] - rowptr[0];
  if (rowptr[r + 1] == rowptr[r]) return;
  const long long B = blockDim.x;
  for (long long base = 0; base < cols; base += 4 * kFillVec * B) {
    float f[kFillVec][4];
    unsigned long long packed = 0;
#pragma unroll
    for (int j = 0; j < kFillVec; ++j) {
      const long long c = base + 4 * (j * B + threadIdx.x);
      if (c < cols) {
        round4(load_vec4(row, c, cols, VEC), c, cols, f[j]);
      } else {
        f[j][0] = f[j][1] = f[j][2] = f[j][3] = 0.f;
      }
      packed |= (unsigned long long)nz4(f[j]) << (16 * j);
    }
    if (!__syncthreads_or(packed != 0)) continue;
    unsigned long long total;
    const unsigned long long incl = block_inclusive_scan(packed, scratch, &total);
    const unsigned long long excl = incl - packed;
    long long pos = out;
#pragma unroll
    for (int j = 0; j < kFillVec; ++j) {
      long long o = pos + (long long)((excl >> (16 * j)) & 0xffffu);
      const long long c = base + 4 * (j * B + threadIdx.x);
#pragma unroll
      for (int k = 0; k < 4; ++k)
        if (f[j][k] != 0.f) {
          colidx[o] = (int)(c + k);
          values[o] = f[j][k];
          ++o;
        }
      pos += (long long)((total >> (16 * j)) & 0xffffu);
    }
    out = pos;
  }
}

static int row_threads(long long cols, int per_thread) {
  int t = 32;
  while (t < 512 && (long long)t * per_thread < cols) t <<= 1;
  return t;
}

static int check_tile(const char* fn, const float* x, int64_t ldx, int64_t rows, int64_t cols,
                      const void* rowptr) {
  CC_REQUIRE(rows >= 0 && cols >= 0, "%s: rows %lld / cols %lld < 0", fn, (long long)rows,
             (long long)cols);
  CC_REQUIRE(ldx >= cols, "%s: ldx %lld < cols %lld", fn, (long long)ldx, (long long)cols);
  CC_REQUIRE(cols <= INT32_MAX, "%s: cols %lld do not fit the int32 column index", fn,
             (long long)cols);
  CC_REQUIRE(rows <= INT32_MAX, "%s: %lld rows: launch one tile at a time", fn, (long long)rows);
  CC_REQUIRE(rows == 0 || ((cols == 0 || x != nullptr) && rowptr != nullptr), "%s: null pointer",
             fn);
  return 0;
}

static bool vec_ok(const float* x, int64_t ldx) {
  return ldx % 4 == 0 && (((uintptr_t)x) & 15) == 0;
}

}

extern "C" int cc_round_csr_count(const float* x, int64_t ldx, int64_t rows, int64_t cols,
                                  int64_t* rowptr, cc_stream_t stream) {
  using namespace cc;
  if (int rc = check_tile("cc_round_csr_count", x, ldx, rows, cols, rowptr)) return rc;
  if (rows == 0) return 0;
  cudaStream_t st = (cudaStream_t)stream;
  const int threads = row_threads(cols, 4 * 4);
  if (vec_ok(x, ldx))
    round_csr_count_kernel<true><<<(unsigned)rows, threads, 0, st>>>(x, ldx, cols,
                                                                     (long long*)rowptr);
  else
    round_csr_count_kernel<false><<<(unsigned)rows, threads, 0, st>>>(x, ldx, cols,
                                                                      (long long*)rowptr);
  CC_CHECK_LAUNCH();
  round_csr_scan_kernel<<<1, 1024, 0, st>>>(rows, (long long*)rowptr);
  CC_CHECK_LAUNCH();
  return 0;
}

extern "C" int cc_round_csr_fill(const float* x, int64_t ldx, int64_t rows, int64_t cols,
                                 const int64_t* rowptr, int32_t* colidx, float* values,
                                 cc_stream_t stream) {
  using namespace cc;
  if (int rc = check_tile("cc_round_csr_fill", x, ldx, rows, cols, rowptr)) return rc;
  if (rows == 0 || cols == 0) return 0;
  cudaStream_t st = (cudaStream_t)stream;
  const int threads = row_threads(cols, 4 * kFillVec);
  if (vec_ok(x, ldx))
    round_csr_fill_kernel<true><<<(unsigned)rows, threads, 0, st>>>(
        x, ldx, cols, (const long long*)rowptr, colidx, values);
  else
    round_csr_fill_kernel<false><<<(unsigned)rows, threads, 0, st>>>(
        x, ldx, cols, (const long long*)rowptr, colidx, values);
  CC_CHECK_LAUNCH();
  return 0;
}
```

cellcomm_b200/csrc/score.cu:

```cuda
#include "common.cuh"

namespace cc {

constexpr long long kScoreMaxCols = 1ll << 18;

template <bool VEC>
__global__ void __launch_bounds__(512, 4)
recon_sqerr_kernel(const float* __restrict__ pred, long long ld, long long cols,
                   const long long* __restrict__ rowptr, const int* __restrict__ colidx,
                   const float* __restrict__ values, long long row0, float scale,
                   float* __restrict__ out) {
  extern __shared__ unsigned bits[];
  __shared__ float warp_sum[32];
  const long long r = blockIdx.x;
  const float* row = pred + r * ld;
  const long long beg = rowptr[row0 + r], end = rowptr[row0 + r + 1];
  const long long words = (cols + 31) >> 5;
  for (long long w = threadIdx.x; w < words; w += blockDim.x) bits[w] = 0u;
  __syncthreads();
  for (long long e = beg + threadIdx.x; e < end; e += blockDim.x) {
    const long long c = colidx[e];
    if (c >= 0 && c < cols) atomicOr(&bits[c >> 5], 1u << (c & 31));
  }
  __syncthreads();

  float acc = 0.f;
  for (long long c = 4ll * threadIdx.x; c < cols; c += 4ll * blockDim.x) {
    float p[4];
    if (VEC) {
      const float4 v = *reinterpret_cast<const float4*>(row + c);
      p[0] = v.x, p[1] = v.y, p[2] = v.z, p[3] = v.w;
    } else {
#pragma unroll
      for (int k = 0; k < 4; ++k) p[k] = c + k < cols ? row[c + k] : 0.f;
    }
    const unsigned m = bits[c >> 5] >> (c & 31);
#pragma unroll
    for (int k = 0; k < 4; ++k)
      if (c + k < cols && !((m >> k) & 1u)) acc += p[k] * p[k];
  }
  for (long long e = beg + threadIdx.x; e < end; e += blockDim.x) {
    const long long c = colidx[e];
    if (c >= 0 && c < cols) {
      const float d = row[c] - values[e];
      acc += d * d;
    }
  }

  const int lane = threadIdx.x & 31, warp = threadIdx.x >> 5, nwarps = blockDim.x >> 5;
#pragma unroll
  for (int o = 16; o > 0; o >>= 1) acc += __shfl_xor_sync(0xffffffffu, acc, o);
  if (lane == 0) warp_sum[warp] = acc;
  __syncthreads();
  if (warp == 0) {
    float s = lane < nwarps ? warp_sum[lane] : 0.f;
#pragma unroll
    for (int o = 16; o > 0; o >>= 1) s += __shfl_xor_sync(0xffffffffu, s, o);
    if (lane == 0) out[r] = scale * s;
  }
}

}

extern "C" int cc_recon_sqerr(const float* pred, int64_t ld, int64_t rows, int64_t cols,
                              const int64_t* rowptr, const int32_t* colidx, const float* values,
                              int64_t row0, float scale, float* out, cc_stream_t stream) {
  using namespace cc;
  CC_REQUIRE(rows >= 0 && cols >= 0 && row0 >= 0, "cc_recon_sqerr: rows %lld / cols %lld / "
             "row0 %lld < 0", (long long)rows, (long long)cols, (long long)row0);
  CC_REQUIRE(ld >= cols, "cc_recon_sqerr: ld %lld < cols %lld", (long long)ld, (long long)cols);
  CC_REQUIRE(cols <= kScoreMaxCols, "cc_recon_sqerr: %lld columns exceed the %lld the "
             "shared-memory bitmap holds", (long long)cols, kScoreMaxCols);
  CC_REQUIRE(rows <= INT32_MAX, "cc_recon_sqerr: %lld rows: launch one tile at a time",
             (long long)rows);
  if (rows == 0) return 0;
  CC_REQUIRE((cols == 0 || pred != nullptr) && rowptr != nullptr && out != nullptr,
             "cc_recon_sqerr: null pointer");
  int threads = 32;
  while (threads < 512 && (long long)threads * 16 < cols) threads <<= 1;
  const size_t smem = (size_t)((cols + 31) >> 5) * sizeof(unsigned);
  cudaStream_t st = (cudaStream_t)stream;
  const bool vec = ld % 4 == 0 && (((uintptr_t)pred) & 15) == 0;
  if (vec)
    recon_sqerr_kernel<true><<<(unsigned)rows, threads, smem, st>>>(
        pred, ld, cols, (const long long*)rowptr, colidx, values, row0, scale, out);
  else
    recon_sqerr_kernel<false><<<(unsigned)rows, threads, smem, st>>>(
        pred, ld, cols, (const long long*)rowptr, colidx, values, row0, scale, out);
  CC_CHECK_LAUNCH();
  return 0;
}
```

cellcomm_b200/csrc/tail_kernels.cu:

```cuda
#include "common.cuh"

namespace cc {

static int num_sms() {
  static int n = 0;
  if (n == 0) {
    int dev = 0;
    if (cudaGetDevice(&dev) != cudaSuccess ||
        cudaDeviceGetAttribute(&n, cudaDevAttrMultiProcessorCount, dev) != cudaSuccess)
      n = 148;
  }
  return n;
}

static unsigned ew_grid(long long work, int threads) {
  long long blocks = (work + threads - 1) / threads;
  const long long cap = (long long)num_sms() * 8;
  if (blocks > cap) blocks = cap;
  if (blocks < 1) blocks = 1;
  return (unsigned)blocks;
}

struct alignas(16) bf16x8 {
  __nv_bfloat162 v[4];
};

struct Mat {
  void* p;
  long long ld;
  int f32;
};
static inline Mat mat(const void* p, long long ld, int f32) {
  return Mat{const_cast<void*>(p), ld, f32};
}

__device__ __forceinline__ void load8(const Mat& m, long long r, long long c0, int n,
                                      float (&f)[8]) {
  if (m.f32) {
    const float* p = reinterpret_cast<const float*>(m.p) + r * m.ld + c0;
    if (n == 8 && (m.ld % 4) == 0 && ((((uintptr_t)m.p) & 15) == 0)) {
      const float4 a = *reinterpret_cast<const float4*>(p);
      const float4 b = *reinterpret_cast<const float4*>(p + 4);
      f[0] = a.x; f[1] = a.y; f[2] = a.z; f[3] = a.w;
      f[4] = b.x; f[5] = b.y; f[6] = b.z; f[7] = b.w;
    } else {
#pragma unroll
      for (int i = 0; i < 8; ++i) f[i] = (i < n) ? p[i] : 0.f;
    }
  } else {
    const bf16* p = reinterpret_cast<const bf16*>(m.p) + r * m.ld + c0;
    if (n == 8 && (m.ld % 8) == 0 && ((((uintptr_t)m.p) & 15) == 0)) {
      bf16x8 q = *reinterpret_cast<const bf16x8*>(p);
#pragma unroll
      for (int i = 0; i < 4; ++i) {
        float2 t = __bfloat1622float2(q.v[i]);
        f[2 * i] = t.x;
        f[2 * i + 1] = t.y;
      }
    } else {
#pragma unroll
      for (int i = 0; i < 8; ++i) f[i] = (i < n) ? bf2f(p[i]) : 0.f;
    }
  }
}
__device__ __forceinline__ void store8(const Mat& m, long long r, long long c0, int n,
                                       const float (&f)[8]) {
  if (m.f32) {
    float* p = reinterpret_cast<float*>(m.p) + r * m.ld + c0;
    if (n == 8 && (m.ld % 4) == 0 && ((((uintptr_t)m.p) & 15) == 0)) {
      *reinterpret_cast<float4*>(p) = make_float4(f[0], f[1], f[2], f[3]);
      *reinterpret_cast<float4*>(p + 4) = make_float4(f[4], f[5], f[6], f[7]);
    } else {
#pragma unroll
      for (int i = 0; i < 8; ++i)
        if (i < n) p[i] = f[i];
    }
  } else {
    bf16* p = reinterpret_cast<bf16*>(m.p) + r * m.ld + c0;
    if (n == 8 && (m.ld % 8) == 0 && ((((uintptr_t)m.p) & 15) == 0)) {
      bf16x8 q;
#pragma unroll
      for (int i = 0; i < 4; ++i) q.v[i] = __floats2bfloat162_rn(f[2 * i], f[2 * i + 1]);
      *reinterpret_cast<bf16x8*>(p) = q;
    } else {
#pragma unroll
      for (int i = 0; i < 8; ++i)
        if (i < n) p[i] = f2bf(f[i]);
    }
  }
}
__device__ __forceinline__ float load1(const Mat& m, long long r, long long c) {
  return m.f32 ? reinterpret_cast<const float*>(m.p)[r * m.ld + c]
               : bf2f(reinterpret_cast<const bf16*>(m.p)[r * m.ld + c]);
}
__device__ __forceinline__ void store1(const Mat& m, long long r, long long c, float v) {
  if (m.f32) reinterpret_cast<float*>(m.p)[r * m.ld + c] = v;
  else reinterpret_cast<bf16*>(m.p)[r * m.ld + c] = f2bf(v);
}

template <typename F>
__device__ __forceinline__ void for_each_chunk8(long long rows, long long cols, F f) {
  const long long cpr = (cols + 7) / 8;
  const long long T = (long long)gridDim.x * blockDim.x;
  const long long tid = (long long)blockIdx.x * blockDim.x + threadIdx.x;
  if (cpr <= T && cpr < (1ll << 31)) {
    const unsigned lanes = (unsigned)(T / cpr);
    const unsigned lane = (unsigned)(tid / cpr);
    if (lane >= lanes) return;
    const long long c0 = (tid - (long long)lane * cpr) * 8;
    const int n = (int)min((long long)8, cols - c0);
    for (long long r = lane; r < rows; r += lanes) f(r, c0, n);
  } else {
    const long long total = rows * cpr;
    for (long long i = tid; i < total; i += T) {
      const long long r = i / cpr;
      const long long c0 = (i - r * cpr) * 8;
      const int n = (int)min((long long)8, cols - c0);
      f(r, c0, n);
    }
  }
}

__device__ __forceinline__ void load8_param(const float* __restrict__ p, long long c0, int n,
                                            float (&f)[8]) {
  if (n == 8 && ((((uintptr_t)(p + c0)) & 15) == 0)) {
    const float4 a = __ldg(reinterpret_cast<const float4*>(p + c0));
    const float4 b = __ldg(reinterpret_cast<const float4*>(p + c0 + 4));
    f[0] = a.x; f[1] = a.y; f[2] = a.z; f[3] = a.w;
    f[4] = b.x; f[5] = b.y; f[6] = b.z; f[7] = b.w;
  } else {
#pragma unroll
    for (int i = 0; i < 8; ++i) f[i] = (i < n) ? __ldg(p + c0 + i) : 0.f;
  }
}

__device__ __forceinline__ void rng8(uint64_t seed, uint64_t step, uint32_t stream_id, long long r,
                                     long long c0, long long cols, float (&u)[8]) {
  const uint64_t blocks_per_row = (uint64_t)((cols + 3) / 4);
  const uint64_t hi = ((uint64_t)stream_id << 40) ^ step;
  uint32_t o[4];
  Philox::block(seed, hi, (uint64_t)r * blocks_per_row + (uint64_t)(c0 / 4), o);
#pragma unroll
  for (int i = 0; i < 4; ++i) u[i] = u32_to_unit(o[i]);
  Philox::block(seed, hi, (uint64_t)r * blocks_per_row + (uint64_t)(c0 / 4) + 1, o);
#pragma unroll
  for (int i = 0; i < 4; ++i) u[4 + i] = u32_to_unit(o[i]);
}

__global__ void dropout_kernel(const Mat x, const Mat out, long long rows, long long cols,
                               float rate, const uint8_t* __restrict__ mask, long long ldm,
                               uint64_t seed, const uint64_t* __restrict__ counter,
                               uint32_t stream_id) {
  const float scale = 1.f / (1.f - rate);
  const uint64_t step = counter ? *counter : 0;
  for_each_chunk8(rows, cols, [&](long long r, long long c0, int n) {
    float f[8];
    load8(x, r, c0, n, f);
    if (mask != nullptr) {
      const uint8_t* m = mask + r * ldm + c0;
#pragma unroll
      for (int i = 0; i < 8; ++i)
        if (i < n) f[i] = m[i] ? f[i] * scale : 0.f;
    } else {
      float u[8];
      rng8(seed, step, stream_id, r, c0, cols, u);
#pragma unroll
      for (int i = 0; i < 8; ++i) f[i] = (u[i] >= rate) ? f[i] * scale : 0.f;
    }
    store8(out, r, c0, n, f);
  });
}

__global__ void dropout_mask_kernel(uint8_t* __restrict__ mask, long long ldm, long long rows,
                                    long long cols, float rate, uint64_t seed,
                                    const uint64_t* __restrict__ counter, uint32_t stream_id) {
  const uint64_t step = counter ? *counter : 0;
  for_each_chunk8(rows, cols, [&](long long r, long long c0, int n) {
    float u[8];
    rng8(seed, step, stream_id, r, c0, cols, u);
    for (int i = 0; i < n; ++i) mask[r * ldm + c0 + i] = (u[i] >= rate) ? 1 : 0;
  });
}

__global__ void uniform_kernel(float* __restrict__ out32, bf16* __restrict__ out16, long long ld,
                               long long rows, long long cols, uint64_t seed,
                               const uint64_t* __restrict__ counter, uint32_t stream_id) {
  const uint64_t step = counter ? *counter : 0;
  for_each_chunk8(rows, cols, [&](long long r, long long c0, int n) {
    float u[8];
    rng8(seed, step, stream_id, r, c0, cols, u);
    for (int i = 0; i < n; ++i) {
      if (out32) out32[r * ld + c0 + i] = u[i];
      if (out16) out16[r * ld + c0 + i] = f2bf(u[i]);
    }
  });
}

__global__ void counter_add_kernel(uint64_t* counter, uint64_t inc) { *counter += inc; }

__global__ void act_bwd_kernel(const Mat dy, const Mat y, const Mat dz, long long rows,
                               long long cols, int act) {
  for_each_chunk8(rows, cols, [&](long long r, long long c0, int n) {
    float g[8], a[8];
    load8(dy, r, c0, n, g);
    load8(y, r, c0, n, a);
#pragma unroll
    for (int i = 0; i < 8; ++i)
      g[i] *= (act == CC_ACT_SIGMOID) ? a[i] * (1.f - a[i])
                                      : (act == CC_ACT_RELU ? (a[i] > 0.f ? 1.f : 0.f) : 1.f);
    store8(dz, r, c0, n, g);
  });
}

__global__ void copy2d_kernel(const Mat src, const Mat dst, long long rows, long long cols,
                              int beta, float scale) {
  for_each_chunk8(rows, cols, [&](long long r, long long c0, int n) {
    float f[8];
    load8(src, r, c0, n, f);
#pragma unroll
    for (int i = 0; i < 8; ++i) f[i] *= scale;
    if (beta) {
      float o[8];
      load8(dst, r, c0, n, o);
#pragma unroll
      for (int i = 0; i < 8; ++i) f[i] += o[i];
    }
    store8(dst, r, c0, n, f);
  });
}

__global__ void split_kernel(const Mat x, const Mat hi, const Mat lo, long long rows,
                             long long cols) {
  for_each_chunk8(rows, cols, [&](long long r, long long c0, int n) {
    float f[8], h[8], l[8];
    load8(x, r, c0, n, f);
#pragma unroll
    for (int i = 0; i < 8; ++i) {
      h[i] = bf2f(f2bf(f[i]));
      l[i] = f[i] - h[i];
    }
    store8(hi, r, c0, n, h);
    store8(lo, r, c0, n, l);
  });
}

__global__ void round_kernel(const Mat x, const Mat out, float* __restrict__ out32,
                             long long ldo32, long long rows, long long cols) {
  for_each_chunk8(rows, cols, [&](long long r, long long c0, int n) {
    float f[8];
    load8(x, r, c0, n, f);
#pragma unroll
    for (int i = 0; i < 8; ++i) f[i] = rintf(f[i]);
    if (out.p) store8(out, r, c0, n, f);
    if (out32)
      for (int i = 0; i < n; ++i) out32[r * ldo32 + c0 + i] = f[i];
  });
}

__global__ void bias_act_kernel(const float* __restrict__ bias, int act, bf16* __restrict__ out16,
                                long long ld16, float* __restrict__ out32, long long ld32,
                                long long rows, long long cols) {
  for (long long i = (long long)blockIdx.x * blockDim.x + threadIdx.x; i < rows * cols;
       i += (long long)gridDim.x * blockDim.x) {
    const long long r = i / cols, c = i - r * cols;
    float v = bias ? bias[c] : 0.f;
    if (act == CC_ACT_SIGMOID) v = sigmoidf_(v);
    else if (act == CC_ACT_RELU) v = fmaxf(v, 0.f);
    if (out16) out16[r * ld16 + c] = f2bf(v);
    if (out32) out32[r * ld32 + c] = v;
  }
}

__global__ void fill_f32_kernel(float* dst, float v, long long n) {
  for (long long i = (long long)blockIdx.x * blockDim.x + threadIdx.x; i < n;
       i += (long long)gridDim.x * blockDim.x)
    dst[i] = v;
}

__device__ __forceinline__ void load_quad(const Mat& m, long long r, long long c, int nv,
                                          float (&x)[4]) {
  if (m.f32) {
    const float* p = reinterpret_cast<const float*>(m.p) + r * m.ld + c;
    if (nv == 4 && (m.ld & 3) == 0 && ((((uintptr_t)m.p) & 15) == 0)) {
      const float4 t = *reinterpret_cast<const float4*>(p);
      x[0] = t.x; x[1] = t.y; x[2] = t.z; x[3] = t.w;
    } else {
#pragma unroll
      for (int i = 0; i < 4; ++i) x[i] = (i < nv) ? p[i] : 0.f;
    }
  } else {
    const bf16* p = reinterpret_cast<const bf16*>(m.p) + r * m.ld + c;
    if (nv == 4 && (m.ld & 3) == 0 && ((((uintptr_t)m.p) & 7) == 0)) {
      const uint2 t = *reinterpret_cast<const uint2*>(p);
      const float2 lo = __bfloat1622float2(*reinterpret_cast<const __nv_bfloat162*>(&t.x));
      const float2 hi = __bfloat1622float2(*reinterpret_cast<const __nv_bfloat162*>(&t.y));
      x[0] = lo.x; x[1] = lo.y; x[2] = hi.x; x[3] = hi.y;
    } else {
#pragma unroll
      for (int i = 0; i < 4; ++i) x[i] = (i < nv) ? bf2f(p[i]) : 0.f;
    }
  }
}
__device__ __forceinline__ void store_quad(const Mat& m, long long r, long long c, int nv,
                                           const float (&x)[4]) {
  if (m.f32) {
    float* p = reinterpret_cast<float*>(m.p) + r * m.ld + c;
    if (nv == 4 && (m.ld & 3) == 0 && ((((uintptr_t)m.p) & 15) == 0)) {
      *reinterpret_cast<float4*>(p) = make_float4(x[0], x[1], x[2], x[3]);
    } else {
#pragma unroll
      for (int i = 0; i < 4; ++i)
        if (i < nv) p[i] = x[i];
    }
  } else {
    bf16* p = reinterpret_cast<bf16*>(m.p) + r * m.ld + c;
    if (nv == 4 && (m.ld & 3) == 0 && ((((uintptr_t)m.p) & 7) == 0)) {
      __nv_bfloat162 lo = __floats2bfloat162_rn(x[0], x[1]);
      __nv_bfloat162 hi = __floats2bfloat162_rn(x[2], x[3]);
      uint2 t;
      t.x = *reinterpret_cast<uint32_t*>(&lo);
      t.y = *reinterpret_cast<uint32_t*>(&hi);
      *reinterpret_cast<uint2*>(p) = t;
    } else {
#pragma unroll
      for (int i = 0; i < 4; ++i)
        if (i < nv) p[i] = f2bf(x[i]);
    }
  }
}

template <int MODE>
__global__ void __launch_bounds__(256)
colreduce_kernel(const Mat a, const Mat b, long long rows, long long cols,
                 const float* __restrict__ mean, const float* __restrict__ rstd,
                 float* __restrict__ out, int accumulate, int act, float* __restrict__ part,
                 unsigned int* __restrict__ tickets,
                 const Mat dz = Mat{nullptr, 0, 0}, const Mat dzlo = Mat{nullptr, 0, 0}) {
  __shared__ float s0[8][128], s1[8][128];
  const int tx = threadIdx.x, ty = threadIdx.y;
  const long long c = (long long)blockIdx.x * 128 + tx * 4;
  const long long rows_per_slab = (rows + gridDim.y - 1) / gridDim.y;
  const long long r_begin = (long long)blockIdx.y * rows_per_slab;
  const long long r_end = min(rows, r_begin + rows_per_slab);
  const int nv = (int)max(0ll, min(4ll, cols - c));
  float acc0[4] = {0.f, 0.f, 0.f, 0.f}, acc1[4] = {0.f, 0.f, 0.f, 0.f};
  float mu[4] = {0.f, 0.f, 0.f, 0.f}, rs[4] = {0.f, 0.f, 0.f, 0.f};
  if (MODE == 2) {
#pragma unroll
    for (int i = 0; i < 4; ++i)
      if (i < nv) { mu[i] = mean[c + i]; rs[i] = rstd[c + i]; }
  }
  const bool need_b = MODE == 2 || (MODE == 3 && act != 0);
  auto consume = [&](long long r, const float (&x)[4], const float (&y)[4]) {
    if (MODE == 0) {
#pragma unroll
      for (int i = 0; i < 4; ++i) acc0[i] += x[i];
    } else if (MODE == 1) {
#pragma unroll
      for (int i = 0; i < 4; ++i) { acc0[i] += x[i]; acc1[i] += x[i] * x[i]; }
    } else if (MODE == 2) {
#pragma unroll
      for (int i = 0; i < 4; ++i) { acc0[i] += x[i]; acc1[i] += x[i] * ((y[i] - mu[i]) * rs[i]); }
    } else {
      float v[4];
#pragma unroll
      for (int i = 0; i < 4; ++i) {
        v[i] = x[i] * (act == CC_ACT_SIGMOID ? y[i] * (1.f - y[i])
                                             : (act == CC_ACT_RELU ? (y[i] > 0.f ? 1.f : 0.f) : 1.f));
        acc0[i] += v[i];
      }
      if (dz.p != nullptr) store_quad(dz, r, c, nv, v);
      if (dzlo.p != nullptr) {
        float l[4];
#pragma unroll
        for (int i = 0; i < 4; ++i) l[i] = v[i] - bf2f(f2bf(v[i]));
        store_quad(dzlo, r, c, nv, l);
      }
    }
  };
  if (nv > 0) {
    long long r = r_begin + ty;
    for (; r + 24 < r_end; r += 32) {
      float x[4][4], y[4][4];
#pragma unroll
      for (int u = 0; u < 4; ++u) {
        load_quad(a, r + 8 * u, c, nv, x[u]);
        if (need_b) load_quad(b, r + 8 * u, c, nv, y[u]);
        else y[u][0] = y[u][1] = y[u][2] = y[u][3] = 0.f;
      }
#pragma unroll
      for (int u = 0; u < 4; ++u) consume(r + 8 * u, x[u], y[u]);
    }
    for (; r < r_end; r += 8) {
      float x[4], y[4] = {0.f, 0.f, 0.f, 0.f};
      load_quad(a, r, c, nv, x);
      if (need_b) load_quad(b, r, c, nv, y);
      consume(r, x, y);
    }
  }
#pragma unroll
  for (int i = 0; i < 4; ++i) {
    s0[ty][tx * 4 + i] = acc0[i];
    s1[ty][tx * 4 + i] = acc1[i];
  }
  __syncthreads();
  constexpr bool two = MODE == 1 || MODE == 2;
  const int j = ty * 32 + tx;
  const long long cc_ = (long long)blockIdx.x * 128 + j;
  if (part == nullptr) {
    if (ty < 4 && cc_ < cols && out != nullptr) {
      float t0 = 0.f, t1 = 0.f;
#pragma unroll
      for (int y = 0; y < 8; ++y) {
        t0 += s0[y][j];
        t1 += s1[y][j];
      }
      if (gridDim.y > 1 || accumulate) {
        atomicAdd(out + cc_, t0);
        if (two) atomicAdd(out + cols + cc_, t1);
      } else {
        out[cc_] = t0;
        if (two) out[cols + cc_] = t1;
      }
    }
    return;
  }
  if (ty < 4 && cc_ < cols) {
    float t0 = 0.f, t1 = 0.f;
#pragma unroll
    for (int y = 0; y < 8; ++y) {
      t0 += s0[y][j];
      t1 += s1[y][j];
    }
    part[(long long)blockIdx.y * cols + cc_] = t0;
    if (two) part[(long long)(gridDim.y + blockIdx.y) * cols + cc_] = t1;
  }
  __threadfence();
  __syncthreads();
  __shared__ bool last;
  if (tx == 0 && ty == 0) last = atomicAdd(tickets + blockIdx.x, 1u) == gridDim.y - 1;
  __syncthreads();
  if (!last) return;
  __threadfence();
  if (ty < 4 && cc_ < cols) {
    float t0 = 0.f, t1 = 0.f;
    for (unsigned y = 0; y < gridDim.y; ++y) {
      t0 += __ldcg(part + (long long)y * cols + cc_);
      if (two) t1 += __ldcg(part + (long long)(gridDim.y + y) * cols + cc_);
    }
    if (accumulate) {
      out[cc_] += t0;
      if (two) out[cols + cc_] += t1;
    } else {
      out[cc_] = t0;
      if (two) out[cols + cc_] = t1;
    }
  }
  if (tx == 0 && ty == 0) tickets[blockIdx.x] = 0u;
}

static long long reduce_tickets() { return 2ll * num_sms(); }

static void colreduce_grid(long long rows, long long cols, unsigned& gx, unsigned& gy) {
  gx = (unsigned)((cols + 127) / 128);
  gy = 1;
  const unsigned target = 2u * (unsigned)num_sms();
  if (gx < target) {
    gy = (target + gx - 1) / gx;
    const unsigned maxy = (unsigned)((rows + 63) / 64);
    if (gy > maxy) gy = maxy;
    if (gy < 1) gy = 1;
  }
}

static long long colreduce_ws_floats(long long rows, long long cols, int outputs) {
  unsigned gx, gy;
  colreduce_grid(rows, cols, gx, gy);
  return gy > 1 ? reduce_tickets() + (long long)outputs * gy * cols : 0;
}

static long long mse_blocks(long long rows, long long cols) {
  return ew_grid(rows * ((cols + 7) / 8), 256);
}

template <int MODE>
static int launch_colreduce(const Mat& a, const Mat& b, long long rows, long long cols,
                            const float* mean, const float* rstd, float* out, int accumulate,
                            float* ws, long long ws_floats, cudaStream_t st, int act = 0,
                            const Mat dz = Mat{nullptr, 0, 0}, const Mat dzlo = Mat{nullptr, 0, 0}) {
  constexpr int outputs = (MODE == 0 || MODE == 3) ? 1 : 2;
  unsigned gx, gy;
  colreduce_grid(rows, cols, gx, gy);
  const bool fixed = ws != nullptr && gy > 1 && out != nullptr;
  if (fixed) {
    const long long need = colreduce_ws_floats(rows, cols, outputs);
    CC_REQUIRE(ws_floats >= need,
               "column reduction of [%lld, %lld]: workspace of %lld floats, needs %lld "
               "(cc_reduce_ws_floats)", rows, cols, (long long)ws_floats, need);
  } else if (gy > 1 && !accumulate && out != nullptr) {
    const long long n = outputs * cols;
    fill_f32_kernel<<<ew_grid(n, 256), 256, 0, st>>>(out, 0.f, n);
    CC_CHECK_LAUNCH();
  }
  colreduce_kernel<MODE><<<dim3(gx, gy), dim3(32, 8), 0, st>>>(
      a, b, rows, cols, mean, rstd, out, accumulate, act,
      fixed ? ws + reduce_tickets() : nullptr, fixed ? reinterpret_cast<unsigned int*>(ws) : nullptr,
      dz, dzlo);
  CC_CHECK_LAUNCH();
  return 0;
}

__global__ void bn_finalize_kernel(const float* __restrict__ sums, long long cols, double inv_n,
                                   float eps, float momentum, float* __restrict__ moving_mean,
                                   float* __restrict__ moving_var, float* __restrict__ save_mean,
                                   float* __restrict__ save_rstd) {
  const long long c = (long long)blockIdx.x * blockDim.x + threadIdx.x;
  if (c >= cols) return;
  const double mean_d = (double)sums[c] * inv_n;
  double var_d = (double)sums[cols + c] * inv_n - mean_d * mean_d;
  const float mean = (float)mean_d;
  const float var = fmaxf((float)var_d, 0.f);
  save_mean[c] = mean;
  save_rstd[c] = rsqrtf(var + eps);
  if (moving_mean) moving_mean[c] = moving_mean[c] * momentum + mean * (1.f - momentum);
  if (moving_var) moving_var[c] = moving_var[c] * momentum + var * (1.f - momentum);
}

__global__ void bn_apply_kernel(const Mat x, const Mat y, long long rows, long long cols,
                                const float* __restrict__ gamma, const float* __restrict__ beta,
                                const float* __restrict__ mean, const float* __restrict__ stat,
                                int infer, float eps) {
  for_each_chunk8(rows, cols, [&](long long r, long long c0, int n) {
    float f[8], mu[8], st[8], ga[8], be[8];
    load8(x, r, c0, n, f);
    load8_param(mean, c0, n, mu);
    load8_param(stat, c0, n, st);
    load8_param(gamma, c0, n, ga);
    load8_param(beta, c0, n, be);
#pragma unroll
    for (int i = 0; i < 8; ++i) {
      if (i < n) {
        const float rs = infer ? rsqrtf(st[i] + eps) : st[i];
        f[i] = (f[i] - mu[i]) * (ga[i] * rs) + be[i];
      }
    }
    store8(y, r, c0, n, f);
  });
}

__global__ void bn_bwd_apply_kernel(const Mat dy, const Mat x, const Mat dx, long long rows,
                                    long long cols, const float* __restrict__ gamma,
                                    const float* __restrict__ mean, const float* __restrict__ rstd,
                                    const float* __restrict__ sums2, float inv_n) {
  for_each_chunk8(rows, cols, [&](long long r, long long c0, int n) {
    float g[8], a[8], mu[8], rs[8], ga[8], s0[8], s1[8];
    load8(dy, r, c0, n, g);
    load8(x, r, c0, n, a);
    load8_param(mean, c0, n, mu);
    load8_param(rstd, c0, n, rs);
    load8_param(gamma, c0, n, ga);
    load8_param(sums2, c0, n, s0);
    load8_param(sums2 + cols, c0, n, s1);
#pragma unroll
    for (int i = 0; i < 8; ++i) {
      if (i < n) {
        const float xhat = (a[i] - mu[i]) * rs[i];
        g[i] = ga[i] * rs[i] * (g[i] - s0[i] * inv_n - xhat * s1[i] * inv_n);
      }
    }
    store8(dx, r, c0, n, g);
  });
}

__global__ void bn_param_grad_kernel(const float* __restrict__ sums2, long long cols,
                                     float* __restrict__ dgamma, float* __restrict__ dbeta) {
  const long long c = (long long)blockIdx.x * blockDim.x + threadIdx.x;
  if (c >= cols) return;
  if (dbeta) dbeta[c] = sums2[c];
  if (dgamma) dgamma[c] = sums2[cols + c];
}

__global__ void bn_infer_bwd_kernel(const Mat dy, const Mat dx, long long rows, long long cols,
                                    const float* __restrict__ gamma,
                                    const float* __restrict__ var, float eps) {
  for_each_chunk8(rows, cols, [&](long long r, long long c0, int n) {
    float g[8];
    load8(dy, r, c0, n, g);
#pragma unroll
    for (int i = 0; i < 8; ++i)
      if (i < n) g[i] *= gamma[c0 + i] * rsqrtf(var[c0 + i] + eps);
    store8(dx, r, c0, n, g);
  });
}

__global__ void softmax_fwd_kernel(const Mat x, const Mat y, float* __restrict__ y32,
                                   long long ldy32, long long rows, long long cols) {
  const long long r = (long long)blockIdx.x * blockDim.x + threadIdx.x;
  if (r >= rows) return;
  float mx = -INFINITY;
  for (long long c = 0; c < cols; ++c) mx = fmaxf(mx, load1(x, r, c));
  float sum = 0.f;
  for (long long c = 0; c < cols; ++c) sum += __expf(load1(x, r, c) - mx);
  const float inv = 1.f / sum;
  for (long long c = 0; c < cols; ++c) {
    const float v = __expf(load1(x, r, c) - mx) * inv;
    if (y.p) store1(y, r, c, v);
    if (y32) y32[r * ldy32 + c] = v;
  }
}

__global__ void softmax_bwd_kernel(const Mat dy, const Mat y, const Mat dx, long long rows,
                                   long long cols) {
  const long long r = (long long)blockIdx.x * blockDim.x + threadIdx.x;
  if (r >= rows) return;
  float dot = 0.f;
  for (long long c = 0; c < cols; ++c) dot += load1(dy, r, c) * load1(y, r, c);
  for (long long c = 0; c < cols; ++c)
    store1(dx, r, c, load1(y, r, c) * (load1(dy, r, c) - dot));
}

__global__ void argmax_onehot_kernel(const float* __restrict__ p, long long ldp,
                                     bf16* __restrict__ out16, long long ldo,
                                     float* __restrict__ out32, long long ldo32, long long rows,
                                     long long cols) {
  const long long r = (long long)blockIdx.x * blockDim.x + threadIdx.x;
  if (r >= rows) return;
  long long best = 0;
  float bv = p[r * ldp];
  for (long long c = 1; c < cols; ++c) {
    const float v = p[r * ldp + c];
    if (v > bv) {
      bv = v;
      best = c;
    }
  }
  for (long long c = 0; c < cols; ++c) {
    const float v = (c == best) ? 1.f : 0.f;
    if (out16) out16[r * ldo + c] = f2bf(v);
    if (out32) out32[r * ldo32 + c] = v;
  }
}

__device__ __forceinline__ float block_sum(float v) {
  __shared__ float sh[32];
  const int lane = threadIdx.x & 31, w = threadIdx.x >> 5;
#pragma unroll
  for (int o = 16; o > 0; o >>= 1) v += __shfl_xor_sync(0xffffffffu, v, o);
  __syncthreads();
  if (lane == 0) sh[w] = v;
  __syncthreads();
  const int nw = (blockDim.x + 31) >> 5;
  v = (threadIdx.x < nw) ? sh[threadIdx.x] : 0.f;
  if (w == 0) {
#pragma unroll
    for (int o = 16; o > 0; o >>= 1) v += __shfl_xor_sync(0xffffffffu, v, o);
  }
  return v;
}

__global__ void bce_kernel(const float* __restrict__ x, long long ldx, long long rows,
                           int from_logits, float target, float inv_n,
                           float* __restrict__ loss_out, const Mat dz) {
  float acc = 0.f;
  for (long long r = threadIdx.x; r < rows; r += blockDim.x) {
    const float raw = x[r * ldx];
    float loss, p;
    if (from_logits) {
      loss = fmaxf(raw, 0.f) - raw * target + log1pf(expf(-fabsf(raw)));
      p = 1.f / (1.f + expf(-raw));
    } else {
      const float eps = 1e-7f;
      p = raw;
      const float q = fminf(fmaxf(raw, eps), 1.f - eps);
      loss = -(target * logf(q) + (1.f - target) * logf(1.f - q));
    }
    acc += loss;
    if (dz.p) store1(dz, r, 0, (p - target) * inv_n);
  }
  acc = block_sum(acc);
  if (threadIdx.x == 0) atomicAdd(loss_out, acc * inv_n);
}

__global__ void mse_kernel(const Mat pred, const Mat target, long long rows, long long cols,
                           float inv_total, float* __restrict__ loss_out, const Mat dpred,
                           float* __restrict__ part, unsigned int* __restrict__ ticket) {
  float acc = 0.f;
  for_each_chunk8(rows, cols, [&](long long r, long long c0, int n) {
    float a[8], t[8];
    load8(pred, r, c0, n, a);
    load8(target, r, c0, n, t);
    float g[8];
#pragma unroll
    for (int i = 0; i < 8; ++i) {
      const float d = (i < n) ? a[i] - t[i] : 0.f;
      acc += d * d;
      g[i] = 2.f * d * inv_total;
    }
    if (dpred.p) store8(dpred, r, c0, n, g);
  });
  acc = block_sum(acc);
  if (part == nullptr) {
    if (threadIdx.x == 0) atomicAdd(loss_out, acc * inv_total);
    return;
  }
  __shared__ bool last;
  if (threadIdx.x == 0) {
    part[blockIdx.x] = acc;
    __threadfence();
    last = atomicAdd(ticket, 1u) == gridDim.x - 1;
  }
  __syncthreads();
  if (!last) return;
  __threadfence();
  float t = 0.f;
  for (unsigned i = threadIdx.x; i < gridDim.x; i += blockDim.x) t += __ldcg(part + i);
  t = block_sum(t);
  if (threadIdx.x == 0) {
    *loss_out += t * inv_total;
    *ticket = 0u;
  }
}

__global__ void rmsprop_kernel(float* __restrict__ p32, bf16* __restrict__ p16,
                               const float* __restrict__ g, float* __restrict__ ms,
                               float* __restrict__ mom, long long rows, long long cols,
                               long long ld, float lr, float rho, float momentum, float eps,
                               float grad_scale) {
  const bool vec = (ld % 4 == 0) && ((((uintptr_t)p32) & 15) == 0) && ((((uintptr_t)g) & 15) == 0) &&
                   ((((uintptr_t)ms) & 15) == 0) && ((((uintptr_t)mom) & 15) == 0) &&
                   (p16 == nullptr || (((uintptr_t)p16) & 7) == 0);
  const long long cpr = (cols + 3) / 4;
  const long long total = rows * cpr;
  for (long long i = (long long)blockIdx.x * blockDim.x + threadIdx.x; i < total;
       i += (long long)gridDim.x * blockDim.x) {
    const long long r = i / cpr;
    const long long c0 = (i - r * cpr) * 4;
    const int n = (int)min((long long)4, cols - c0);
    const long long off = r * ld + c0;
    float w[4], gg[4], s[4], m[4];
    if (vec && n == 4) {
      float4 a = *reinterpret_cast<const float4*>(p32 + off);
      float4 b = *reinterpret_cast<const float4*>(g + off);
      float4 c = *reinterpret_cast<const float4*>(ms + off);
      float4 d = *reinterpret_cast<const float4*>(mom + off);
      w[0] = a.x; w[1] = a.y; w[2] = a.z; w[3] = a.w;
      gg[0] = b.x; gg[1] = b.y; gg[2] = b.z; gg[3] = b.w;
      s[0] = c.x; s[1] = c.y; s[2] = c.z; s[3] = c.w;
      m[0] = d.x; m[1] = d.y; m[2] = d.z; m[3] = d.w;
    } else {
#pragma unroll
      for (int k = 0; k < 4; ++k) {
        if (k < n) {
          w[k] = p32[off + k];
          gg[k] = g[off + k];
          s[k] = ms[off + k];
          m[k] = mom[off + k];
        } else {
          w[k] = gg[k] = s[k] = m[k] = 0.f;
        }
      }
    }
#pragma unroll
    for (int k = 0; k < 4; ++k) {
      const float gk = gg[k] * grad_scale;
      s[k] = rho * s[k] + (1.f - rho) * gk * gk;
      m[k] = momentum * m[k] + lr * gk * rsqrtf(s[k] + eps);
      w[k] -= m[k];
    }
    if (vec && n == 4) {
      *reinterpret_cast<float4*>(p32 + off) = make_float4(w[0], w[1], w[2], w[3]);
      *reinterpret_cast<float4*>(ms + off) = make_float4(s[0], s[1], s[2], s[3]);
      *reinterpret_cast<float4*>(mom + off) = make_float4(m[0], m[1], m[2], m[3]);
      if (p16) {
        __nv_bfloat162 lo = __floats2bfloat162_rn(w[0], w[1]);
        __nv_bfloat162 hi = __floats2bfloat162_rn(w[2], w[3]);
        uint2 u;
        u.x = *reinterpret_cast<uint32_t*>(&lo);
        u.y = *reinterpret_cast<uint32_t*>(&hi);
        *reinterpret_cast<uint2*>(p16 + off) = u;
      }
    } else {
#pragma unroll
      for (int k = 0; k < 4; ++k) {
        if (k < n) {
          p32[off + k] = w[k];
          ms[off + k] = s[k];
          mom[off + k] = m[k];
          if (p16) p16[off + k] = f2bf(w[k]);
        }
      }
    }
  }
}

}

using namespace cc;

#define ST(s) ((cudaStream_t)(s))
#define F32(mask, bit) (((mask) >> (bit)) & 1)
#define EW_LAUNCH(kern, rows, cols, stream, ...)                                        \
  do {                                                                                  \
    if ((rows) <= 0 || (cols) <= 0) return 0;                                           \
    const long long _work = (long long)(rows) * (((cols) + 7) / 8);                     \
    kern<<<ew_grid(_work, 256), 256, 0, ST(stream)>>>(__VA_ARGS__);                     \
    CC_CHECK_LAUNCH();                                                                  \
    return 0;                                                                           \
  } while (0)

extern "C" int64_t cc_reduce_ws_floats(int64_t rows, int64_t cols) {
  if (rows <= 0 || cols <= 0) return 0;
  long long need = reduce_tickets() + mse_blocks(rows, cols);
  const long long gx_max = (cols + 127) / 128;
  for (long long gx = 1; gx <= gx_max && gx < reduce_tickets(); ++gx) {
    const long long n = colreduce_ws_floats(rows, gx == gx_max ? cols : gx * 128, 2);
    if (n > need) need = n;
  }
  return need;
}

extern "C" int cc_colsum(const void* x, int64_t ld, int64_t rows, int64_t cols, float* out,
                         int32_t beta, int32_t dtypes, cc_stream_t stream) {
  return cc_colsum_ws(x, ld, rows, cols, out, beta, dtypes, nullptr, 0, stream);
}

extern "C" int cc_colsum_ws(const void* x, int64_t ld, int64_t rows, int64_t cols, float* out,
                            int32_t beta, int32_t dtypes, float* ws, int64_t ws_floats,
                            cc_stream_t stream) {
  if (cols <= 0) return 0;
  if (rows <= 0) {
    if (!beta) {
      fill_f32_kernel<<<ew_grid(cols, 256), 256, 0, ST(stream)>>>(out, 0.f, cols);
      CC_CHECK_LAUNCH();
    }
    return 0;
  }
  return launch_colreduce<0>(mat(x, ld, F32(dtypes, 0)), mat(nullptr, 0, 0), rows, cols, nullptr,
                             nullptr, out, beta, ws, ws_floats, ST(stream));
}

extern "C" int cc_bias_grad(const void* dy, int64_t lddy, const void* y, int64_t ldy, int64_t rows,
                            int64_t cols, int32_t act, float* out, int32_t beta, void* dz,
                            int64_t lddz, void* dz_lo, int64_t lddz_lo, int32_t dtypes,
                            cc_stream_t stream) {
  return cc_bias_grad_ws(dy, lddy, y, ldy, rows, cols, act, out, beta, dz, lddz, dz_lo, lddz_lo,
                         dtypes, nullptr, 0, stream);
}

extern "C" int cc_bias_grad_ws(const void* dy, int64_t lddy, const void* y, int64_t ldy,
                               int64_t rows, int64_t cols, int32_t act, float* out, int32_t beta,
                               void* dz, int64_t lddz, void* dz_lo, int64_t lddz_lo,
                               int32_t dtypes, float* ws, int64_t ws_floats, cc_stream_t stream) {
  if (cols <= 0) return 0;
  CC_REQUIRE(out != nullptr || dz != nullptr, "cc_bias_grad: nothing to compute");
  CC_REQUIRE(dz_lo == nullptr || (dz != nullptr && !F32(dtypes, 2)),
             "cc_bias_grad: dz_lo needs a bf16 dz (the high-order term)");
  if (rows <= 0) {
    if (!beta && out != nullptr) {
      fill_f32_kernel<<<ew_grid(cols, 256), 256, 0, ST(stream)>>>(out, 0.f, cols);
      CC_CHECK_LAUNCH();
    }
    return 0;
  }
  return launch_colreduce<3>(mat(dy, lddy, F32(dtypes, 0)), mat(y, ldy, F32(dtypes, 1)), rows, cols,
                             nullptr, nullptr, out, beta, ws, ws_floats, ST(stream), act,
                             mat(dz, lddz, F32(dtypes, 2)), mat(dz_lo, lddz_lo, 0));
}

extern "C" int cc_split_bf16(const void* x, int64_t ldx, void* hi, int64_t ldhi, void* lo,
                             int64_t ldlo, int64_t rows, int64_t cols, int32_t dtypes,
                             cc_stream_t stream) {
  EW_LAUNCH(split_kernel, rows, cols, stream, mat(x, ldx, F32(dtypes, 0)), mat(hi, ldhi, 0),
            mat(lo, ldlo, 0), rows, cols);
}

extern "C" int cc_dropout(const void* x, int64_t ldx, void* out, int64_t ldo, int64_t rows,
                          int64_t cols, float rate, const uint8_t* mask_u8, int64_t ldm,
                          uint64_t seed, const uint64_t* counter_dev, uint32_t stream_id,
                          int32_t dtypes, cc_stream_t stream) {
  CC_REQUIRE(rate >= 0.f && rate < 1.f, "cc_dropout: rate %f out of range", rate);
  EW_LAUNCH(dropout_kernel, rows, cols, stream, mat(x, ldx, F32(dtypes, 0)),
            mat(out, ldo, F32(dtypes, 1)), rows, cols, rate, mask_u8, ldm, seed, counter_dev,
            stream_id);
}

extern "C" int cc_dropout_mask(uint8_t* mask_u8, int64_t ldm, int64_t rows, int64_t cols,
                               float rate, uint64_t seed, const uint64_t* counter_dev,
                               uint32_t stream_id, cc_stream_t stream) {
  EW_LAUNCH(dropout_mask_kernel, rows, cols, stream, mask_u8, ldm, rows, cols, rate, seed,
            counter_dev, stream_id);
}

extern "C" int cc_uniform(float* out32, void* out16, int64_t ld, int64_t rows, int64_t cols,
                          uint64_t seed, const uint64_t* counter_dev, uint32_t stream_id,
                          cc_stream_t stream) {
  EW_LAUNCH(uniform_kernel, rows, cols, stream, out32, (bf16*)out16, ld, rows, cols, seed,
            counter_dev, stream_id);
}

extern "C" int cc_counter_add(uint64_t* counter_dev, uint64_t inc, cc_stream_t stream) {
  counter_add_kernel<<<1, 1, 0, ST(stream)>>>(counter_dev, inc);
  CC_CHECK_LAUNCH();
  return 0;
}

extern "C" int cc_act_bwd(const void* dy, int64_t lddy, const void* y, int64_t ldy, void* dz,
                          int64_t lddz, int64_t rows, int64_t cols, int32_t act, int32_t dtypes,
                          cc_stream_t stream) {
  EW_LAUNCH(act_bwd_kernel, rows, cols, stream, mat(dy, lddy, F32(dtypes, 0)),
            mat(y, ldy, F32(dtypes, 1)), mat(dz, lddz, F32(dtypes, 2)), rows, cols, act);
}

extern "C" int cc_copy2d(const void* src, int64_t lds, void* dst, int64_t ldd, int64_t rows,
                         int64_t cols, int32_t beta, float scale, int32_t dtypes,
                         cc_stream_t stream) {
  EW_LAUNCH(copy2d_kernel, rows, cols, stream, mat(src, lds, F32(dtypes, 0)),
            mat(dst, ldd, F32(dtypes, 1)), rows, cols, beta, scale);
}

extern "C" int cc_bn_stats(const void* x, int64_t ld, int64_t rows, int64_t cols, float* sums,
                           int32_t dtypes, cc_stream_t stream) {
  return cc_bn_stats_ws(x, ld, rows, cols, sums, dtypes, nullptr, 0, stream);
}

extern "C" int cc_bn_stats_ws(const void* x, int64_t ld, int64_t rows, int64_t cols, float* sums,
                              int32_t dtypes, float* ws, int64_t ws_floats, cc_stream_t stream) {
  if (cols <= 0) return 0;
  CC_REQUIRE(rows > 0, "cc_bn_stats: empty batch");
  return launch_colreduce<1>(mat(x, ld, F32(dtypes, 0)), mat(nullptr, 0, 0), rows, cols, nullptr,
                             nullptr, sums, 0, ws, ws_floats, ST(stream));
}

extern "C" int cc_bn_train_apply(const void* x, int64_t ldx, void* y, int64_t ldy, int64_t rows,
                                 int64_t cols, const float* sums, int64_t n_total,
                                 const float* gamma, const float* beta, float eps, float momentum,
                                 float* moving_mean, float* moving_var, float* save_mean,
                                 float* save_rstd, int32_t dtypes, cc_stream_t stream) {
  if (cols <= 0) return 0;
  CC_REQUIRE(n_total > 0, "cc_bn_train_apply: n_total must be positive");
  bn_finalize_kernel<<<(unsigned)((cols + 255) / 256), 256, 0, ST(stream)>>>(
      sums, cols, 1.0 / (double)n_total, eps, momentum, moving_mean, moving_var, save_mean,
      save_rstd);
  CC_CHECK_LAUNCH();
  EW_LAUNCH(bn_apply_kernel, rows, cols, stream, mat(x, ldx, F32(dtypes, 0)),
            mat(y, ldy, F32(dtypes, 1)), rows, cols, gamma, beta, save_mean, save_rstd, 0, eps);
}

extern "C" int cc_bn_infer(const void* x, int64_t ldx, void* y, int64_t ldy, int64_t rows,
                           int64_t cols, const float* gamma, const float* beta,
                           const float* moving_mean, const float* moving_var, float eps,
                           int32_t dtypes, cc_stream_t stream) {
  EW_LAUNCH(bn_apply_kernel, rows, cols, stream, mat(x, ldx, F32(dtypes, 0)),
            mat(y, ldy, F32(dtypes, 1)), rows, cols, gamma, beta, moving_mean, moving_var, 1, eps);
}

extern "C" int cc_bn_bwd_stats(const void* dy, int64_t lddy, const void* x, int64_t ldx,
                               int64_t rows, int64_t cols, const float* save_mean,
                               const float* save_rstd, float* sums2, int32_t dtypes,
                               cc_stream_t stream) {
  return cc_bn_bwd_stats_ws(dy, lddy, x, ldx, rows, cols, save_mean, save_rstd, sums2, dtypes,
                            nullptr, 0, stream);
}

extern "C" int cc_bn_bwd_stats_ws(const void* dy, int64_t lddy, const void* x, int64_t ldx,
                                  int64_t rows, int64_t cols, const float* save_mean,
                                  const float* save_rstd, float* sums2, int32_t dtypes, float* ws,
                                  int64_t ws_floats, cc_stream_t stream) {
  if (cols <= 0) return 0;
  CC_REQUIRE(rows > 0, "cc_bn_bwd_stats: empty batch");
  return launch_colreduce<2>(mat(dy, lddy, F32(dtypes, 0)), mat(x, ldx, F32(dtypes, 1)), rows, cols,
                             save_mean, save_rstd, sums2, 0, ws, ws_floats, ST(stream));
}

extern "C" int cc_bn_bwd_apply(const void* dy, int64_t lddy, const void* x, int64_t ldx, void* dx,
                               int64_t lddx, int64_t rows, int64_t cols, const float* gamma,
                               const float* save_mean, const float* save_rstd, const float* sums2,
                               int64_t n_total, float* dgamma, float* dbeta, int32_t dtypes,
                               cc_stream_t stream) {
  if (cols <= 0) return 0;
  if (dgamma || dbeta) {
    bn_param_grad_kernel<<<(unsigned)((cols + 255) / 256), 256, 0, ST(stream)>>>(sums2, cols,
                                                                                 dgamma, dbeta);
    CC_CHECK_LAUNCH();
  }
  if (dx == nullptr) return 0;
  EW_LAUNCH(bn_bwd_apply_kernel, rows, cols, stream, mat(dy, lddy, F32(dtypes, 0)),
            mat(x, ldx, F32(dtypes, 1)), mat(dx, lddx, F32(dtypes, 2)), rows, cols, gamma,
            save_mean, save_rstd, sums2, 1.f / (float)n_total);
}

extern "C" int cc_bn_infer_bwd(const void* dy, int64_t lddy, void* dx, int64_t lddx, int64_t rows,
                               int64_t cols, const float* gamma, const float* moving_var,
                               float eps, int32_t dtypes, cc_stream_t stream) {
  EW_LAUNCH(bn_infer_bwd_kernel, rows, cols, stream, mat(dy, lddy, F32(dtypes, 0)),
            mat(dx, lddx, F32(dtypes, 1)), rows, cols, gamma, moving_var, eps);
}

extern "C" int cc_softmax_fwd(const void* x, int64_t ldx, void* y, int64_t ldy, float* y32,
                              int64_t ldy32, int64_t rows, int64_t cols, int32_t dtypes,
                              cc_stream_t stream) {
  if (rows <= 0 || cols <= 0) return 0;
  softmax_fwd_kernel<<<(unsigned)((rows + 127) / 128), 128, 0, ST(stream)>>>(
      mat(x, ldx, F32(dtypes, 0)), mat(y, ldy, F32(dtypes, 1)), y32, ldy32, rows, cols);
  CC_CHECK_LAUNCH();
  return 0;
}

extern "C" int cc_softmax_bwd(const void* dy, int64_t lddy, const void* y, int64_t ldy, void* dx,
                              int64_t lddx, int64_t rows, int64_t cols, int32_t dtypes,
                              cc_stream_t stream) {
  if (rows <= 0 || cols <= 0) return 0;
  softmax_bwd_kernel<<<(unsigned)((rows + 127) / 128), 128, 0, ST(stream)>>>(
      mat(dy, lddy, F32(dtypes, 0)), mat(y, ldy, F32(dtypes, 1)), mat(dx, lddx, F32(dtypes, 2)),
      rows, cols);
  CC_CHECK_LAUNCH();
  return 0;
}

extern "C" int cc_bce_fwd_bwd(const float* x32, int64_t ldx, int64_t rows, int32_t from_logits,
                              float target, int64_t n_total, float* loss_out, void* dz,
                              int64_t lddz, int32_t dtypes, cc_stream_t stream) {
  CC_REQUIRE(rows > 0 && n_total > 0, "cc_bce_fwd_bwd: empty batch");
  bce_kernel<<<1, 256, 0, ST(stream)>>>(x32, ldx, rows, from_logits, target, 1.f / (float)n_total,
                                        loss_out, mat(dz, lddz, F32(dtypes, 0)));
  CC_CHECK_LAUNCH();
  return 0;
}

extern "C" int cc_mse_fwd_bwd(const void* pred, int64_t ldp, const void* target, int64_t ldt,
                              int64_t rows, int64_t cols, int64_t n_total, float* loss_out,
                              void* dpred, int64_t lddp, int32_t dtypes, cc_stream_t stream) {
  return cc_mse_fwd_bwd_ws(pred, ldp, target, ldt, rows, cols, n_total, loss_out, dpred, lddp,
                           dtypes, nullptr, 0, stream);
}

extern "C" int cc_mse_fwd_bwd_ws(const void* pred, int64_t ldp, const void* target, int64_t ldt,
                                 int64_t rows, int64_t cols, int64_t n_total, float* loss_out,
                                 void* dpred, int64_t lddp, int32_t dtypes, float* ws,
                                 int64_t ws_floats, cc_stream_t stream) {
  CC_REQUIRE(target != nullptr, "cc_mse_fwd_bwd: no target");
  if (rows <= 0 || cols <= 0) return 0;
  const float inv_total = 1.f / ((float)n_total * (float)cols);
  const long long blocks = mse_blocks(rows, cols);
  if (ws != nullptr) {
    const long long need = reduce_tickets() + blocks;
    CC_REQUIRE(ws_floats >= need,
               "cc_mse_fwd_bwd_ws of [%lld, %lld]: workspace of %lld floats, needs %lld "
               "(cc_reduce_ws_floats)", (long long)rows, (long long)cols, (long long)ws_floats,
               need);
  }
  mse_kernel<<<(unsigned)blocks, 256, 0, ST(stream)>>>(
      mat(pred, ldp, F32(dtypes, 0)), mat(target, ldt, F32(dtypes, 1)), rows, cols, inv_total,
      loss_out, mat(dpred, lddp, F32(dtypes, 2)), ws ? ws + reduce_tickets() : nullptr,
      reinterpret_cast<unsigned int*>(ws));
  CC_CHECK_LAUNCH();
  return 0;
}

extern "C" int cc_round_half_even(const void* x, int64_t ldx, void* out, int64_t ldo, float* out32,
                                  int64_t ldo32, int64_t rows, int64_t cols, int32_t dtypes,
                                  cc_stream_t stream) {
  EW_LAUNCH(round_kernel, rows, cols, stream, mat(x, ldx, F32(dtypes, 0)),
            mat(out, ldo, F32(dtypes, 1)), out32, ldo32, rows, cols);
}

extern "C" int cc_argmax_onehot(const float* p32, int64_t ldp, void* out16, int64_t ldo,
                                float* out32, int64_t ldo32, int64_t rows, int64_t cols,
                                cc_stream_t stream) {
  if (rows <= 0 || cols <= 0) return 0;
  argmax_onehot_kernel<<<(unsigned)((rows + 127) / 128), 128, 0, ST(stream)>>>(
      p32, ldp, (bf16*)out16, ldo, out32, ldo32, rows, cols);
  CC_CHECK_LAUNCH();
  return 0;
}

extern "C" int cc_rmsprop_step(float* p32, void* p16, const float* g, float* ms, float* mom,
                               int64_t rows, int64_t cols, int64_t ld, float lr, float rho,
                               float momentum, float eps, float grad_scale, cc_stream_t stream) {
  if (rows <= 0 || cols <= 0) return 0;
  const long long work = (long long)rows * ((cols + 3) / 4);
  static int bps = 0;
  if (bps == 0) {
    const char* v = getenv("CC_RMS_BLOCKS_PER_SM");
    bps = v ? atoi(v) : 8;
    if (bps < 1 || bps > 8) bps = 8;
  }
  long long blocks = (work + 255) / 256;
  if (blocks > (long long)num_sms() * bps) blocks = (long long)num_sms() * bps;
  rmsprop_kernel<<<(unsigned)blocks, 256, 0, ST(stream)>>>(p32, (bf16*)p16, g, ms, mom, rows,
                                                             cols, ld, lr, rho, momentum, eps,
                                                             grad_scale);
  CC_CHECK_LAUNCH();
  return 0;
}

extern "C" int cc_bias_act(const float* bias, int32_t act, void* out16, int64_t ld16, float* out32,
                           int64_t ld32, int64_t rows, int64_t cols, cc_stream_t stream) {
  if (rows <= 0 || cols <= 0) return 0;
  bias_act_kernel<<<ew_grid(rows * cols, 256), 256, 0, ST(stream)>>>(bias, act, (bf16*)out16, ld16,
                                                                    out32, ld32, rows, cols);
  CC_CHECK_LAUNCH();
  return 0;
}

extern "C" int cc_fill_f32(float* dst, float value, int64_t n, cc_stream_t stream) {
  if (n <= 0) return 0;
  fill_f32_kernel<<<ew_grid(n, 256), 256, 0, ST(stream)>>>(dst, value, n);
  CC_CHECK_LAUNCH();
  return 0;
}
```

cellcomm_b200/csrc/wgrad_rmsprop_kernel.cuh:

```cuda
#pragma once

namespace cc {

struct RmsMaps {
  CUtensorMap a[MAX_SEG];
  CUtensorMap b[MAX_SEG];
  CUtensorMap p32, ms, mom, p16;
};

__device__ __forceinline__ uint64_t l2_evict_first_policy() {
  uint64_t pol;
  asm volatile("createpolicy.fractional.L2::evict_first.b64 %0, 1.0;" : "=l"(pol));
  return pol;
}
__device__ __forceinline__ void tma_load_2d_hint(uint32_t dst, const CUtensorMap* map, uint32_t bar,
                                                 int c0, int c1, uint64_t pol) {
  asm volatile(
      "cp.async.bulk.tensor.2d.shared::cluster.global.mbarrier::complete_tx::bytes.L2::cache_hint "
      "[%0], [%1, {%3, %4}], [%2], %5;" ::"r"(dst),
      "l"(map), "r"(bar), "r"(c0), "r"(c1), "l"(pol)
      : "memory");
}
__device__ __forceinline__ void tma_store_2d_hint(const CUtensorMap* map, uint32_t src, int c0,
                                                  int c1, uint64_t pol) {
  asm volatile(
      "cp.async.bulk.tensor.2d.global.shared::cta.bulk_group.L2::cache_hint [%0, {%2, %3}], [%1], %4;" ::
          "l"(map),
      "r"(src), "r"(c0), "r"(c1), "l"(pol)
      : "memory");
}
__device__ __forceinline__ void bulk_commit() { asm volatile("cp.async.bulk.commit_group;" ::: "memory"); }
__device__ __forceinline__ void bulk_wait_read0() {
  asm volatile("cp.async.bulk.wait_group.read 0;" ::: "memory");
}
__device__ __forceinline__ void fence_proxy_async_smem() {
  asm volatile("fence.proxy.async.shared::cta;" ::: "memory");
}
__device__ __forceinline__ float4 lds128(uint32_t addr) {
  float4 v;
  asm volatile("ld.shared.v4.f32 {%0, %1, %2, %3}, [%4];"
               : "=f"(v.x), "=f"(v.y), "=f"(v.z), "=f"(v.w)
               : "r"(addr));
  return v;
}
__device__ __forceinline__ void sts128(uint32_t addr, float4 v) {
  asm volatile("st.shared.v4.f32 [%0], {%1, %2, %3, %4};" ::"r"(addr), "f"(v.x), "f"(v.y), "f"(v.z),
               "f"(v.w)
               : "memory");
}
__device__ __forceinline__ void sts128u(uint32_t addr, uint4 v) {
  asm volatile("st.shared.v4.b32 [%0], {%1, %2, %3, %4};" ::"r"(addr), "r"(v.x), "r"(v.y), "r"(v.z),
               "r"(v.w)
               : "memory");
}

constexpr int RMS_BN = 256;
constexpr int RMS_STAGES = 2;
constexpr int RMS_EPI_WARPS = 8;
constexpr uint32_t RMS_F32_BLOCK = 32 * 32 * 4;
constexpr uint32_t RMS_B16_BLOCK = 32 * 32 * 2;
constexpr uint32_t RMS_EPI_BUF = 3 * RMS_F32_BLOCK + RMS_B16_BLOCK;
constexpr uint32_t RMS_STAGE_BYTES = BM * BK * 2 + RMS_BN * BK * 2;
constexpr size_t RMS_SMEM_BYTES = (size_t)RMS_STAGES * RMS_STAGE_BYTES +
                                  (size_t)RMS_EPI_WARPS * RMS_EPI_BUF + 8 * (2 * RMS_STAGES + 4 + RMS_EPI_WARPS) +
                                  16 + 1024;

__device__ __forceinline__ void rms_epilogue_tile(const EpiParams& e, const RmsMaps& maps,
                                                  const uint32_t t_row, const int r0, const int n0,
                                                  const int col_lo, const int col_hi,
                                                  const int col_step, const int lane,
                                                  const uint32_t buf_w, const uint32_t sbar,
                                                  uint32_t& sphase, const uint64_t pol,
                                                  const bool p16_direct) {
  if (r0 >= e.M) return;
  const uint32_t buf_s = buf_w + RMS_F32_BLOCK;
  const uint32_t buf_m = buf_s + RMS_F32_BLOCK;
  const uint32_t buf_h = buf_m + RMS_F32_BLOCK;
  const bool has16 = e.rms_p16 != nullptr;
  const float rho = e.rms_rho, omr = 1.f - e.rms_rho, mu = e.rms_momentum, lr = e.rms_lr,
              eps = e.rms_eps;
  const uint32_t row128 = (uint32_t)lane * 128u, sw128 = (uint32_t)(lane & 7);
  const uint32_t row64 = (uint32_t)lane * 64u, sw64 = (uint32_t)((lane >> 1) & 3);
#pragma unroll 1
  for (int c = col_lo; c < col_hi; c += col_step) {
    const int c0 = n0 + c;
    if (c0 >= e.N) break;
    if (elect_one()) {
      bulk_wait_read0();
      mbar_expect_tx(sbar, 3 * RMS_F32_BLOCK);
      tma_load_2d_hint(buf_w, &maps.p32, sbar, c0, r0, pol);
      tma_load_2d_hint(buf_s, &maps.ms, sbar, c0, r0, pol);
      tma_load_2d_hint(buf_m, &maps.mom, sbar, c0, r0, pol);
    }
    __syncwarp();
    uint32_t raw[32];
    tmem_ld32(t_row + (uint32_t)c, raw);
    tmem_ld_wait();
    if (e.out32 != nullptr && r0 + lane < e.M) {
      float* o = e.out32 + (long long)(r0 + lane) * e.ld32 + c0;
      const int nc = min(32, e.N - c0);
      if (nc == 32 && (e.ld32 & 3) == 0) {
#pragma unroll
        for (int j = 0; j < 32; j += 4)
          *reinterpret_cast<uint4*>(o + j) = make_uint4(raw[j], raw[j + 1], raw[j + 2], raw[j + 3]);
      } else {
#pragma unroll
        for (int j = 0; j < 32; ++j)
          if (j < nc) o[j] = __uint_as_float(raw[j]);
      }
    }
    mbar_wait(sbar, sphase, 25);
    sphase ^= 1u;
#pragma unroll
    for (int j = 0; j < 8; ++j) {
      const uint32_t off = row128 + ((((uint32_t)j) ^ sw128) << 4);
      const float4 w = lds128(buf_w + off), s = lds128(buf_s + off), m = lds128(buf_m + off);
      const float g0 = __uint_as_float(raw[4 * j]), g1 = __uint_as_float(raw[4 * j + 1]),
                  g2 = __uint_as_float(raw[4 * j + 2]), g3 = __uint_as_float(raw[4 * j + 3]);
      float4 ss, mm, ww;
      ss.x = fmaf(rho, s.x, omr * g0 * g0);
      ss.y = fmaf(rho, s.y, omr * g1 * g1);
      ss.z = fmaf(rho, s.z, omr * g2 * g2);
      ss.w = fmaf(rho, s.w, omr * g3 * g3);
      mm.x = fmaf(mu, m.x, lr * g0 * rsqrtf(ss.x + eps));
      mm.y = fmaf(mu, m.y, lr * g1 * rsqrtf(ss.y + eps));
      mm.z = fmaf(mu, m.z, lr * g2 * rsqrtf(ss.z + eps));
      mm.w = fmaf(mu, m.w, lr * g3 * rsqrtf(ss.w + eps));
      ww.x = w.x - mm.x;
      ww.y = w.y - mm.y;
      ww.z = w.z - mm.z;
      ww.w = w.w - mm.w;
      sts128(buf_s + off, ss);
      sts128(buf_m + off, mm);
      sts128(buf_w + off, ww);
      __nv_bfloat162 lo = __floats2bfloat162_rn(ww.x, ww.y);
      __nv_bfloat162 hi = __floats2bfloat162_rn(ww.z, ww.w);
      raw[2 * j] = *reinterpret_cast<uint32_t*>(&lo);
      raw[2 * j + 1] = *reinterpret_cast<uint32_t*>(&hi);
    }
    if (has16 && !p16_direct) {
#pragma unroll
      for (int t = 0; t < 4; ++t)
        sts128u(buf_h + row64 + ((((uint32_t)t) ^ sw64) << 4),
                make_uint4(raw[4 * t], raw[4 * t + 1], raw[4 * t + 2], raw[4 * t + 3]));
    } else if (has16 && r0 + lane < e.M) {
      bf16* o = e.rms_p16 + (long long)(r0 + lane) * e.rms_ld + c0;
      if (c0 + 32 <= e.N) {
#pragma unroll
        for (int t = 0; t < 4; ++t)
          __stcs(reinterpret_cast<uint4*>(o) + t,
                 make_uint4(raw[4 * t], raw[4 * t + 1], raw[4 * t + 2], raw[4 * t + 3]));
      } else {
        const int nc = e.N - c0;
#pragma unroll
        for (int t = 0; t < 16; ++t) {
          if (2 * t < nc) o[2 * t] = __ushort_as_bfloat16((unsigned short)(raw[t] & 0xFFFFu));
          if (2 * t + 1 < nc) o[2 * t + 1] = __ushort_as_bfloat16((unsigned short)(raw[t] >> 16));
        }
      }
    }
    fence_proxy_async_smem();
    __syncwarp();
    if (elect_one()) {
      tma_store_2d_hint(&maps.ms, buf_s, c0, r0, pol);
      tma_store_2d_hint(&maps.mom, buf_m, c0, r0, pol);
      tma_store_2d_hint(&maps.p32, buf_w, c0, r0, pol);
      if (has16 && !p16_direct) tma_store_2d_hint(&maps.p16, buf_h, c0, r0, pol);
      bulk_commit();
    }
  }
}

template <bool N_FAST, int CLUSTER>
__global__ void __launch_bounds__(64 + 32 * RMS_EPI_WARPS, 1)
wgrad_rmsprop_tma_kernel(const __grid_constant__ RmsMaps maps, const __grid_constant__ GemmParams p,
                         const int tiles_m, const int tiles_n) {
  constexpr int BN = RMS_BN, STAGES = RMS_STAGES, EPI_WARPS = RMS_EPI_WARPS;
  constexpr uint32_t A_BYTES = BM * BK * 2;
  constexpr uint32_t STAGE_BYTES = RMS_STAGE_BYTES;
  constexpr uint32_t TMEM_COLS = 2 * BN;

  extern __shared__ uint8_t smem_raw[];
  const uint32_t smem_base = (smem_u32(smem_raw) + 1023u) & ~1023u;
  const uint32_t epi_base = smem_base + STAGES * STAGE_BYTES;
  const uint32_t bar_base = epi_base + EPI_WARPS * RMS_EPI_BUF;
  auto full_bar = [&](int s) { return bar_base + 8u * s; };
  auto empty_bar = [&](int s) { return bar_base + 8u * (STAGES + s); };
  auto tfull_bar = [&](int a) { return bar_base + 8u * (2 * STAGES + a); };
  auto tempty_bar = [&](int a) { return bar_base + 8u * (2 * STAGES + 2 + a); };
  auto state_bar = [&](int w) { return bar_base + 8u * (2 * STAGES + 4 + w); };
  const uint32_t tmem_slot = bar_base + 8u * (2 * STAGES + 4 + EPI_WARPS);
  uint8_t* smem_gen = smem_raw + (smem_base - smem_u32(smem_raw));
  volatile uint32_t* tmem_slot_ptr = reinterpret_cast<volatile uint32_t*>(
      smem_gen + (tmem_slot - smem_base));

  const int warp = threadIdx.x >> 5;
  const int lane = threadIdx.x & 31;
  const int nkb = p.total_kblocks;
  const int rank = (CLUSTER == 2) ? (int)cluster_ctarank() : 0;
  const int tiles_mu = (tiles_m + CLUSTER - 1) / CLUSTER;
  const int num_units = tiles_mu * tiles_n;
  const int unit0 = (int)blockIdx.x / CLUSTER, unit_step = (int)gridDim.x / CLUSTER;
  auto unit_m0 = [&](int u) { return ((N_FAST ? u / tiles_n : u % tiles_mu) * CLUSTER + rank) * BM; };
  auto unit_n0 = [&](int u) { return (N_FAST ? u % tiles_n : u / tiles_mu) * BN; };

  if (threadIdx.x == 0) {
#pragma unroll
    for (int s = 0; s < STAGES; ++s) {
      mbar_init(full_bar(s), 1);
      mbar_init(empty_bar(s), CLUSTER);
    }
#pragma unroll
    for (int a = 0; a < 2; ++a) {
      mbar_init(tfull_bar(a), 1);
      mbar_init(tempty_bar(a), EPI_WARPS);
    }
#pragma unroll
    for (int w = 0; w < EPI_WARPS; ++w) mbar_init(state_bar(w), 1);
    asm volatile("fence.mbarrier_init.release.cluster;" ::: "memory");
    asm volatile("fence.proxy.async.shared::cta;" ::: "memory");
  }
  if (warp == 1) {
    asm volatile("tcgen05.alloc.cta_group::1.sync.aligned.shared::cta.b32 [%0], %1;" ::"r"(tmem_slot),
                 "r"(TMEM_COLS)
                 : "memory");
    asm volatile("tcgen05.relinquish_alloc_permit.cta_group::1.sync.aligned;" ::: "memory");
  }
  tcgen05_fence_before();
  __syncthreads();
  if (CLUSTER == 2) cluster_sync_all();
  tcgen05_fence_after();
  const uint32_t tmem_acc = *tmem_slot_ptr;

  if (warp == 0) {
    uint32_t it = 0;
    for (int u = unit0; u < num_units; u += unit_step) {
      const int m0 = unit_m0(u), n0 = unit_n0(u);
      int seg = 0, kb_in_seg = 0;
      for (int i = 0; i < nkb; ++i, ++it) {
        const int s = it % STAGES;
        const uint32_t ph = (it / STAGES) & 1u;
        mbar_wait(empty_bar(s), ph ^ 1u, 21);
        if (elect_one()) {
          const uint32_t a_dst = smem_base + s * STAGE_BYTES;
          const uint32_t b_dst = a_dst + A_BYTES;
          const int k0 = kb_in_seg * BK;
          mbar_expect_tx(full_bar(s), STAGE_BYTES);
#pragma unroll
          for (int j = 0; j < BM / 64; ++j)
            tma_load_2d(a_dst + j * (64 * BK * 2), &maps.a[seg], full_bar(s), m0 + 64 * j, k0);
#pragma unroll
          for (int j = 0; j < BN / 64; ++j) {
            if (CLUSTER == 2) {
              if ((j & 1) == rank)
                tma_load_2d_mc(b_dst + j * (64 * BK * 2), &maps.b[seg], full_bar(s), n0 + 64 * j, k0,
                               (uint16_t)3);
            } else {
              tma_load_2d(b_dst + j * (64 * BK * 2), &maps.b[seg], full_bar(s), n0 + 64 * j, k0);
            }
          }
        }
        __syncwarp();
        if (++kb_in_seg >= p.kblocks[seg] && seg < p.nseg - 1) {
          kb_in_seg = 0;
          ++seg;
        }
      }
    }
  } else if (warp == 1) {
    uint32_t it = 0, tl = 0;
    for (int u = unit0; u < num_units; u += unit_step, ++tl) {
      const uint32_t acc = tl & 1u, aph = (tl >> 1) & 1u;
      mbar_wait(tempty_bar(acc), aph ^ 1u, 22);
      tcgen05_fence_after();
      const uint32_t d_tmem = tmem_acc + acc * BN;
      for (int i = 0; i < nkb; ++i, ++it) {
        const int s = it % STAGES;
        const uint32_t ph = (it / STAGES) & 1u;
        mbar_wait(full_bar(s), ph, 23);
        tcgen05_fence_after();
        if (elect_one()) {
          const uint32_t a_src = smem_base + s * STAGE_BYTES;
          const uint32_t b_src = a_src + A_BYTES;
#pragma unroll
          for (int k = 0; k < BK / UMMA_K; ++k) {
            const uint64_t adesc = p.adesc_hi | (uint64_t)(((a_src + k * p.a_kstep) & 0x3FFFFu) >> 4);
            const uint64_t bdesc = p.bdesc_hi | (uint64_t)(((b_src + k * p.b_kstep) & 0x3FFFFu) >> 4);
            umma_bf16(d_tmem, adesc, bdesc, p.idesc, (i > 0 || k > 0) ? 1u : 0u);
          }
          if (CLUSTER == 2) umma_commit_mc(empty_bar(s), (uint16_t)3);
          else umma_commit(empty_bar(s));
          if (i == nkb - 1) umma_commit(tfull_bar(acc));
        }
        __syncwarp();
      }
    }
  } else {
    const EpiParams& e = p.epi;
    const int q = warp & 3;
    const int ew = warp - 2;
    const int col_lo = (ew >> 2) * (BN / 2);
    const uint32_t buf_w = epi_base + ew * RMS_EPI_BUF;
    const uint32_t sbar = state_bar(ew);
    const uint64_t pol = l2_evict_first_policy();
    const bool interleave = (e.rms_cs & 4) != 0;
    uint32_t tl = 0, sphase = 0;
    for (int u = unit0; u < num_units; u += unit_step, ++tl) {
      const int m0 = unit_m0(u), n0 = unit_n0(u);
      const uint32_t acc = tl & 1u, aph = (tl >> 1) & 1u;
      mbar_wait(tfull_bar(acc), aph, 24);
      tcgen05_fence_after();
      rms_epilogue_tile(e, maps, tmem_acc + ((uint32_t)(q * 32) << 16) + acc * BN, m0 + q * 32, n0,
                        interleave ? (ew >> 2) * 32 : col_lo, interleave ? BN : col_lo + BN / 2,
                        interleave ? 64 : 32, lane, buf_w, sbar, sphase, pol, (e.rms_cs & 2) != 0);
      tcgen05_fence_before();
      __syncwarp();
      if (lane == 0) mbar_arrive(tempty_bar(acc));
    }
    __syncwarp();
    if (elect_one()) bulk_wait_read0();
  }
  tcgen05_fence_before();
  __syncthreads();
  if (CLUSTER == 2) cluster_sync_all();
  if (warp == 1) {
    asm volatile("tcgen05.dealloc.cta_group::1.sync.aligned.b32 %0, %1;" ::"r"(tmem_acc),
                 "r"(TMEM_COLS)
                 : "memory");
  }
}

constexpr int RMSP_STAGES = 4;
constexpr uint32_t RMSP_STAGE_BYTES = BM * BK * 2 + (RMS_BN / 2) * BK * 2;
constexpr uint32_t RMSP_EPI_BUF = 3 * RMS_F32_BLOCK;
constexpr size_t RMSP_SMEM_BYTES = (size_t)RMSP_STAGES * RMSP_STAGE_BYTES +
                                   (size_t)RMS_EPI_WARPS * RMSP_EPI_BUF +
                                   8 * (2 * RMSP_STAGES + 4 + RMS_EPI_WARPS) + 16 + 1024;

template <bool N_FAST>
__global__ void __launch_bounds__(64 + 32 * RMS_EPI_WARPS, 1)
wgrad_rmsprop_pair_kernel(const __grid_constant__ RmsMaps maps, const __grid_constant__ GemmParams p,
                          const int tiles_m, const int tiles_n) {
  constexpr int BN = RMS_BN, STAGES = RMSP_STAGES, EPI_WARPS = RMS_EPI_WARPS;
  constexpr uint32_t A_BYTES = BM * BK * 2;
  constexpr uint32_t STAGE_BYTES = RMSP_STAGE_BYTES;
  constexpr uint32_t TMEM_COLS = 2 * BN;

  extern __shared__ uint8_t smem_raw[];
  const uint32_t smem_base = (smem_u32(smem_raw) + 1023u) & ~1023u;
  const uint32_t epi_base = smem_base + STAGES * STAGE_BYTES;
  const uint32_t bar_base = epi_base + EPI_WARPS * RMSP_EPI_BUF;
  auto full_bar = [&](int s) { return bar_base + 8u * s; };
  auto empty_bar = [&](int s) { return bar_base + 8u * (STAGES + s); };
  auto tfull_bar = [&](int a) { return bar_base + 8u * (2 * STAGES + a); };
  auto tempty_bar = [&](int a) { return bar_base + 8u * (2 * STAGES + 2 + a); };
  auto state_bar = [&](int w) { return bar_base + 8u * (2 * STAGES + 4 + w); };
  const uint32_t tmem_slot = bar_base + 8u * (2 * STAGES + 4 + EPI_WARPS);
  uint8_t* smem_gen = smem_raw + (smem_base - smem_u32(smem_raw));
  volatile uint32_t* tmem_slot_ptr = reinterpret_cast<volatile uint32_t*>(
      smem_gen + (tmem_slot - smem_base));

  const int warp = threadIdx.x >> 5;
  const int lane = threadIdx.x & 31;
  const int nkb = p.total_kblocks;
  const int rank = (int)cluster_ctarank();
  const bool leader = rank == 0;
  const int tiles_mu = (tiles_m + 1) / 2;
  const int num_units = tiles_mu * tiles_n;
  const int unit0 = (int)blockIdx.x / 2, unit_step = (int)gridDim.x / 2;
  auto unit_m0 = [&](int u) { return ((N_FAST ? u / tiles_n : u % tiles_mu) * 2 + rank) * BM; };
  auto unit_n0 = [&](int u) { return (N_FAST ? u % tiles_n : u / tiles_mu) * BN; };

  if (threadIdx.x == 0) {
#pragma unroll
    for (int s = 0; s < STAGES; ++s) {
      mbar_init(full_bar(s), 2);
      mbar_init(empty_bar(s), 1);
    }
#pragma unroll
    for (int a = 0; a < 2; ++a) {
      mbar_init(tfull_bar(a), 1);
      mbar_init(tempty_bar(a), 2 * EPI_WARPS);
    }
#pragma unroll
    for (int w = 0; w < EPI_WARPS; ++w) mbar_init(state_bar(w), 1);
    asm volatile("fence.mbarrier_init.release.cluster;" ::: "memory");
    asm volatile("fence.proxy.async.shared::cta;" ::: "memory");
  }
  if (warp == 1) {
    asm volatile("tcgen05.alloc.cta_group::2.sync.aligned.shared::cta.b32 [%0], %1;" ::"r"(tmem_slot),
                 "r"(TMEM_COLS)
                 : "memory");
    asm volatile("tcgen05.relinquish_alloc_permit.cta_group::2.sync.aligned;" ::: "memory");
  }
  tcgen05_fence_before();
  __syncthreads();
  cluster_sync_all();
  tcgen05_fence_after();
  const uint32_t tmem_acc = *tmem_slot_ptr;

  if (warp == 0) {
    uint32_t it = 0;
    for (int u = unit0; u < num_units; u += unit_step) {
      const int m0 = unit_m0(u), n0 = unit_n0(u) + rank * (BN / 2);
      int seg = 0, kb_in_seg = 0;
      for (int i = 0; i < nkb; ++i, ++it) {
        const int s = it % STAGES;
        const uint32_t ph = (it / STAGES) & 1u;
        mbar_wait(empty_bar(s), ph ^ 1u, 31);
        if (elect_one()) {
          const uint32_t a_dst = smem_base + s * STAGE_BYTES;
          const uint32_t b_dst = a_dst + A_BYTES;
          const uint32_t lbar = mapa_cluster(full_bar(s), 0);
          const int k0 = kb_in_seg * BK;
          if (leader) mbar_expect_tx(full_bar(s), 2 * STAGE_BYTES);
          else mbar_arrive_cluster(lbar);
#pragma unroll
          for (int j = 0; j < BM / 64; ++j)
            tma_load_2d_pair(a_dst + j * (64 * BK * 2), &maps.a[seg], lbar, m0 + 64 * j, k0);
#pragma unroll
          for (int j = 0; j < BN / 128; ++j)
            tma_load_2d_pair(b_dst + j * (64 * BK * 2), &maps.b[seg], lbar, n0 + 64 * j, k0);
        }
        __syncwarp();
        if (++kb_in_seg >= p.kblocks[seg] && seg < p.nseg - 1) {
          kb_in_seg = 0;
          ++seg;
        }
      }
    }
  } else if (warp == 1) {
    if (leader) {
      const uint32_t idesc = (p.idesc & ~(0x1Fu << 24)) | ((uint32_t)((2 * BM) >> 4) << 24);
      uint32_t it = 0, tl = 0;
      for (int u = unit0; u < num_units; u += unit_step, ++tl) {
        const uint32_t acc = tl & 1u, aph = (tl >> 1) & 1u;
        mbar_wait(tempty_bar(acc), aph ^ 1u, 32);
        tcgen05_fence_after();
        const uint32_t d_tmem = tmem_acc + acc * BN;
        for (int i = 0; i < nkb; ++i, ++it) {
          const int s = it % STAGES;
          const uint32_t ph = (it / STAGES) & 1u;
          mbar_wait(full_bar(s), ph, 33);
          tcgen05_fence_after();
          if (elect_one()) {
            const uint32_t a_src = smem_base + s * STAGE_BYTES;
            const uint32_t b_src = a_src + A_BYTES;
#pragma unroll
            for (int k = 0; k < BK / UMMA_K; ++k) {
              const uint64_t adesc = p.adesc_hi | (uint64_t)(((a_src + k * p.a_kstep) & 0x3FFFFu) >> 4);
              const uint64_t bdesc = p.bdesc_hi | (uint64_t)(((b_src + k * p.b_kstep) & 0x3FFFFu) >> 4);
              umma_bf16_pair(d_tmem, adesc, bdesc, idesc, (i > 0 || k > 0) ? 1u : 0u);
            }
            umma_commit_pair(empty_bar(s), (uint16_t)3);
            if (i == nkb - 1) umma_commit_pair(tfull_bar(acc), (uint16_t)3);
          }
          __syncwarp();
        }
      }
    }
  } else {
    const EpiParams& e = p.epi;
    const int q = warp & 3;
    const int ew = warp - 2;
    const int col_lo = (ew >> 2) * (BN / 2);
    const uint32_t buf_w = epi_base + ew * RMSP_EPI_BUF;
    const uint32_t sbar = state_bar(ew);
    const uint64_t pol = l2_evict_first_policy();
    const bool interleave = (e.rms_cs & 4) != 0;
    uint32_t tl = 0, sphase = 0;
    for (int u = unit0; u < num_units; u += unit_step, ++tl) {
      const int m0 = unit_m0(u), n0 = unit_n0(u);
      const uint32_t acc = tl & 1u, aph = (tl >> 1) & 1u;
      mbar_wait(tfull_bar(acc), aph, 34);
      tcgen05_fence_after();
      rms_epilogue_tile(e, maps, tmem_acc + ((uint32_t)(q * 32) << 16) + acc * BN, m0 + q * 32, n0,
                        interleave ? (ew >> 2) * 32 : col_lo, interleave ? BN : col_lo + BN / 2,
                        interleave ? 64 : 32, lane, buf_w, sbar, sphase, pol, true);
      tcgen05_fence_before();
      __syncwarp();
      if (lane == 0) mbar_arrive_cluster(mapa_cluster(tempty_bar(acc), 0));
    }
    __syncwarp();
    if (elect_one()) bulk_wait_read0();
  }
  tcgen05_fence_before();
  __syncthreads();
  cluster_sync_all();
  if (warp == 1) {
    asm volatile("tcgen05.dealloc.cta_group::2.sync.aligned.b32 %0, %1;" ::"r"(tmem_acc),
                 "r"(TMEM_COLS)
                 : "memory");
  }
}

}
```

Baseline: 58330.

## Enable programmatic dependent launch across all kernels and prefetch tensor maps

Routes every kernel launch through a common cudaLaunchKernelEx helper that sets programmatic stream serialization, and adds griddepcontrol.wait at the top of each kernel, or after barrier/TMEM setup in the GEMM kernels. The next kernel's launch and prologue (mbarrier init, TMEM alloc, tensormap prefetch) can then overlap the tail of the previous kernel. The GEMM kernels also prefetch their TMA descriptors during setup. No kernel issues an explicit launch_dependents trigger, so the overlap relies on the implicit trigger at grid completion. This mainly hides launch latency in a training loop made of many small kernels.

```diff
diff --git a/cellcomm_b200/csrc/common.cuh b/cellcomm_b200/csrc/common.cuh
--- a/cellcomm_b200/csrc/common.cuh
+++ b/cellcomm_b200/csrc/common.cuh
@@ -39,6 +39,36 @@
   do {                                  \
     cc::count_launch();                 \
     CC_CHECK_CUDA(cudaGetLastError());  \
+  } while (0)
+
+__device__ __forceinline__ void pdl_wait() { asm volatile("griddepcontrol.wait;" ::: "memory"); }
+
+template <typename... KArgs, typename... Args>
+int launch(void (*kern)(KArgs...), dim3 grid, dim3 block, size_t smem, cudaStream_t st,
+           unsigned cluster, Args&&... args) {
+  cudaLaunchAttribute attr[2];
+  attr[0].id = cudaLaunchAttributeProgrammaticStreamSerialization;
+  attr[0].val.programmaticStreamSerializationAllowed = 1;
+  attr[1].id = cudaLaunchAttributeClusterDimension;
+  attr[1].val.clusterDim.x = cluster;
+  attr[1].val.clusterDim.y = 1;
+  attr[1].val.clusterDim.z = 1;
+  cudaLaunchConfig_t cfg{};
+  cfg.gridDim = grid;
+  cfg.blockDim = block;
+  cfg.dynamicSmemBytes = smem;
+  cfg.stream = st;
+  cfg.attrs = attr;
+  cfg.numAttrs = cluster > 1 ? 2 : 1;
+  count_launch();
+  CC_CHECK_CUDA(cudaLaunchKernelEx(&cfg, kern, static_cast<Args&&>(args)...));
+  return 0;
+}
+
+#define CC_LAUNCH(kern, grid, block, smem, st, ...)                                    \
+  do {                                                                                \
+    const int _rc = cc::launch(kern, grid, block, smem, st, 1u, __VA_ARGS__);         \
+    if (_rc != 0) return _rc;                                                         \
   } while (0)
 
 typedef __nv_bfloat16 bf16;
diff --git a/cellcomm_b200/csrc/gather.cu b/cellcomm_b200/csrc/gather.cu
--- a/cellcomm_b200/csrc/gather.cu
+++ b/cellcomm_b200/csrc/gather.cu
@@ -10,6 +10,7 @@
                    long long row_start, long long n_rows, long long n_cols,
                    bf16* __restrict__ out16, long long ld16, float* __restrict__ out32,
                    long long ld32, int use_smem) {
+  pdl_wait();
   extern __shared__ __align__(16) unsigned char smem[];
   bf16* srow = reinterpret_cast<bf16*>(smem);
   const int tid = threadIdx.x;
@@ -79,9 +80,8 @@
   long long grid = n_rows;
   const long long cap = (long long)sms * 16;
   if (grid > cap) grid = cap;
-  gather_rows_kernel<<<(unsigned)grid, GATHER_THREADS, smem, (cudaStream_t)stream>>>(
-      (const long long*)rowptr_dev, colidx_dev, values_dev, (const long long*)row_idx_dev,
-      row_start, n_rows, n_cols, (bf16*)out16, ld16, out32, ld32, use_smem);
-  CC_CHECK_LAUNCH();
+  CC_LAUNCH(gather_rows_kernel, (unsigned)grid, GATHER_THREADS, smem, (cudaStream_t)stream,
+            (const long long*)rowptr_dev, colidx_dev, values_dev, (const long long*)row_idx_dev,
+            row_start, n_rows, n_cols, (bf16*)out16, ld16, out32, ld32, use_smem);
   return 0;
 }
diff --git a/cellcomm_b200/csrc/gemm_sm100.cu b/cellcomm_b200/csrc/gemm_sm100.cu
--- a/cellcomm_b200/csrc/gemm_sm100.cu
+++ b/cellcomm_b200/csrc/gemm_sm100.cu
@@ -73,6 +73,15 @@
 
 __device__ __forceinline__ uint32_t smem_u32(const void* p) {
   return (uint32_t)__cvta_generic_to_shared(p);
+}
+__device__ __forceinline__ void prefetch_tmap(const CUtensorMap* m) {
+  asm volatile("prefetch.tensormap [%0];" ::"l"(reinterpret_cast<uint64_t>(m)) : "memory");
+}
+__device__ __forceinline__ void prefetch_tmaps(const TmaMaps& maps, int nseg) {
+  for (int s = 0; s < nseg; ++s) {
+    prefetch_tmap(&maps.a[s]);
+    prefetch_tmap(&maps.b[s]);
+  }
 }
 __device__ __forceinline__ void mbar_init(uint32_t bar, uint32_t count) {
   asm volatile("mbarrier.init.shared::cta.b64 [%0], %1;" ::"r"(bar), "r"(count));
@@ -515,6 +524,7 @@
     mbar_init(tmem_full_bar, 1);
     asm volatile("fence.mbarrier_init.release.cluster;" ::: "memory");
     asm volatile("fence.proxy.async.shared::cta;" ::: "memory");
+    prefetch_tmaps(maps, p.nseg);
   }
   if (warp == 1) {
     asm volatile("tcgen05.alloc.cta_group::1.sync.aligned.shared::cta.b32 [%0], %1;" ::"r"(tmem_slot),
@@ -526,6 +536,7 @@
   __syncthreads();
   tcgen05_fence_after();
   const uint32_t tmem_acc = *tmem_slot_ptr;
+  pdl_wait();
 
   if (warp == 0) {
     int seg = 0, kb_in_seg = kb_begin;
@@ -842,6 +853,7 @@
     }
     asm volatile("fence.mbarrier_init.release.cluster;" ::: "memory");
     asm volatile("fence.proxy.async.shared::cta;" ::: "memory");
+    prefetch_tmaps(maps, p.nseg);
   }
   if (warp == 1) {
     if (PAIR) {
@@ -861,6 +873,7 @@
   if (CLUSTER == 2) cluster_sync_all();
   tcgen05_fence_after();
   const uint32_t tmem_acc = *tmem_slot_ptr;
+  pdl_wait();
 
   if (warp == 0 && PAIR) {
     uint32_t it = 0;
@@ -1062,6 +1075,7 @@
 
 __global__ void splitk_finalize_kernel(const EpiParams e, const float* __restrict__ partial,
                                        long long partial_ld, long long partial_stride, int splits) {
+  pdl_wait();
   const int groups = (e.N + 3) / 4;
   const long long idx = (long long)blockIdx.x * blockDim.x + threadIdx.x;
   if (idx >= (long long)e.M * groups) return;
@@ -1329,8 +1343,7 @@
     CC_CHECK_CUDA(cudaFuncSetAttribute(kern, cudaFuncAttributeMaxDynamicSharedMemorySize, (int)smem));
     attr_set = true;
   }
-  kern<<<grid, 128, smem, st>>>(maps, p);
-  CC_CHECK_LAUNCH();
+  CC_LAUNCH(kern, grid, 128, smem, st, maps, p);
   return 0;
 }
 
@@ -1384,21 +1397,7 @@
   }
   const int units = ((mt + CLUSTER - 1) / CLUSTER) * nt * (p.psplits > 1 ? p.psplits : 1);
   int grid = units * CLUSTER < max_ctas ? units * CLUSTER : max_ctas / CLUSTER * CLUSTER;
-  cudaLaunchConfig_t cfg{};
-  cfg.gridDim = dim3((unsigned)grid);
-  cfg.blockDim = dim3(threads);
-  cfg.dynamicSmemBytes = smem;
-  cfg.stream = st;
-  cudaLaunchAttribute attr[1];
-  attr[0].id = cudaLaunchAttributeClusterDimension;
-  attr[0].val.clusterDim.x = CLUSTER;
-  attr[0].val.clusterDim.y = 1;
-  attr[0].val.clusterDim.z = 1;
-  cfg.attrs = attr;
-  cfg.numAttrs = 1;
-  CC_CHECK_CUDA(cudaLaunchKernelEx(&cfg, kern, maps, p, mt, nt));
-  count_launch();
-  return 0;
+  return launch(kern, dim3((unsigned)grid), dim3(threads), smem, st, CLUSTER, maps, p, mt, nt);
 }
 
 template <int BN, int STAGES, int EPI_WARPS>
@@ -1470,21 +1469,7 @@
   }
   const int units = ((mt + CLUSTER - 1) / CLUSTER) * nt;
   int grid = units * CLUSTER < max_ctas ? units * CLUSTER : max_ctas / CLUSTER * CLUSTER;
-  cudaLaunchConfig_t cfg{};
-  cfg.gridDim = dim3((unsigned)grid);
-  cfg.blockDim = dim3(threads);
-  cfg.dynamicSmemBytes = smem;
-  cfg.stream = st;
-  cudaLaunchAttribute attr[1];
-  attr[0].id = cudaLaunchAttributeClusterDimension;
-  attr[0].val.clusterDim.x = CLUSTER;
-  attr[0].val.clusterDim.y = 1;
-  attr[0].val.clusterDim.z = 1;
-  cfg.attrs = attr;
-  cfg.numAttrs = 1;
-  CC_CHECK_CUDA(cudaLaunchKernelEx(&cfg, kern, maps, p, mt, nt));
-  count_launch();
-  return 0;
+  return launch(kern, dim3((unsigned)grid), dim3(threads), smem, st, CLUSTER, maps, p, mt, nt);
 }
 
 int gemm_impl(const cc_gemm_desc* d, cudaStream_t st) {
@@ -1759,9 +1744,8 @@
       if (rc) return rc;
       const long long work = (long long)d->M * ((d->N + 3) / 4);
       const int threads = 256;
-      splitk_finalize_kernel<<<(unsigned)((work + threads - 1) / threads), threads, 0, st>>>(
-          p.epi, p.partial, p.partial_ld, p.partial_stride, splits);
-      CC_CHECK_LAUNCH();
+      CC_LAUNCH(splitk_finalize_kernel, (unsigned)((work + threads - 1) / threads), threads, 0, st,
+                p.epi, p.partial, p.partial_ld, p.partial_stride, splits);
       return 0;
     }
     if (bn == 256) return launch_persistent<256, 4>(maps, p, mt, nt, g_num_sms, a_mn, b_mn, st);
@@ -1779,9 +1763,8 @@
   if (splits >= 2) {
     const long long work = (long long)d->M * ((d->N + 3) / 4);
     const int threads = 256;
-    splitk_finalize_kernel<<<(unsigned)((work + threads - 1) / threads), threads, 0, st>>>(
-        p.epi, p.partial, p.partial_ld, p.partial_stride, splits);
-    CC_CHECK_LAUNCH();
+    CC_LAUNCH(splitk_finalize_kernel, (unsigned)((work + threads - 1) / threads), threads, 0, st,
+              p.epi, p.partial, p.partial_ld, p.partial_stride, splits);
   }
   return 0;
 }
diff --git a/cellcomm_b200/csrc/generate.cu b/cellcomm_b200/csrc/generate.cu
--- a/cellcomm_b200/csrc/generate.cu
+++ b/cellcomm_b200/csrc/generate.cu
@@ -59,6 +59,7 @@
 __global__ void __launch_bounds__(512, 4)
 round_csr_count_kernel(const float* __restrict__ x, long long ldx, long long cols,
                        long long* __restrict__ rowptr) {
+  pdl_wait();
   __shared__ long long scratch[32];
   const long long r = blockIdx.x;
   const float* row = x + r * ldx;
@@ -75,6 +76,7 @@
 
 __global__ void __launch_bounds__(1024)
 round_csr_scan_kernel(long long rows, long long* __restrict__ rowptr) {
+  pdl_wait();
   __shared__ long long scratch[32];
   long long carry = rowptr[0];
   for (long long r0 = 0; r0 < rows; r0 += blockDim.x) {
@@ -92,6 +94,7 @@
 round_csr_fill_kernel(const float* __restrict__ x, long long ldx, long long cols,
                       const long long* __restrict__ rowptr, int* __restrict__ colidx,
                       float* __restrict__ values) {
+  pdl_wait();
   static_assert(kFillVec <= 4, "four 16-bit count fields in a uint64");
   __shared__ unsigned long long scratch[32];
   const long long r = blockIdx.x;
@@ -166,15 +169,9 @@
   if (rows == 0) return 0;
   cudaStream_t st = (cudaStream_t)stream;
   const int threads = row_threads(cols, 4 * 4);
-  if (vec_ok(x, ldx))
-    round_csr_count_kernel<true><<<(unsigned)rows, threads, 0, st>>>(x, ldx, cols,
-                                                                     (long long*)rowptr);
-  else
-    round_csr_count_kernel<false><<<(unsigned)rows, threads, 0, st>>>(x, ldx, cols,
-                                                                      (long long*)rowptr);
-  CC_CHECK_LAUNCH();
-  round_csr_scan_kernel<<<1, 1024, 0, st>>>(rows, (long long*)rowptr);
-  CC_CHECK_LAUNCH();
+  auto count = vec_ok(x, ldx) ? round_csr_count_kernel<true> : round_csr_count_kernel<false>;
+  CC_LAUNCH(count, (unsigned)rows, threads, 0, st, x, ldx, cols, (long long*)rowptr);
+  CC_LAUNCH(round_csr_scan_kernel, 1, 1024, 0, st, rows, (long long*)rowptr);
   return 0;
 }
 
@@ -186,12 +183,8 @@
   if (rows == 0 || cols == 0) return 0;
   cudaStream_t st = (cudaStream_t)stream;
   const int threads = row_threads(cols, 4 * kFillVec);
-  if (vec_ok(x, ldx))
-    round_csr_fill_kernel<true><<<(unsigned)rows, threads, 0, st>>>(
-        x, ldx, cols, (const long long*)rowptr, colidx, values);
-  else
-    round_csr_fill_kernel<false><<<(unsigned)rows, threads, 0, st>>>(
-        x, ldx, cols, (const long long*)rowptr, colidx, values);
-  CC_CHECK_LAUNCH();
+  auto fill = vec_ok(x, ldx) ? round_csr_fill_kernel<true> : round_csr_fill_kernel<false>;
+  CC_LAUNCH(fill, (unsigned)rows, threads, 0, st, x, ldx, cols, (const long long*)rowptr, colidx,
+            values);
   return 0;
 }
diff --git a/cellcomm_b200/csrc/score.cu b/cellcomm_b200/csrc/score.cu
--- a/cellcomm_b200/csrc/score.cu
+++ b/cellcomm_b200/csrc/score.cu
@@ -10,6 +10,7 @@
                    const long long* __restrict__ rowptr, const int* __restrict__ colidx,
                    const float* __restrict__ values, long long row0, float scale,
                    float* __restrict__ out) {
+  pdl_wait();
   extern __shared__ unsigned bits[];
   __shared__ float warp_sum[32];
   const long long r = blockIdx.x;
@@ -81,12 +82,8 @@
   const size_t smem = (size_t)((cols + 31) >> 5) * sizeof(unsigned);
   cudaStream_t st = (cudaStream_t)stream;
   const bool vec = ld % 4 == 0 && (((uintptr_t)pred) & 15) == 0;
-  if (vec)
-    recon_sqerr_kernel<true><<<(unsigned)rows, threads, smem, st>>>(
-        pred, ld, cols, (const long long*)rowptr, colidx, values, row0, scale, out);
-  else
-    recon_sqerr_kernel<false><<<(unsigned)rows, threads, smem, st>>>(
-        pred, ld, cols, (const long long*)rowptr, colidx, values, row0, scale, out);
-  CC_CHECK_LAUNCH();
+  auto kern = vec ? recon_sqerr_kernel<true> : recon_sqerr_kernel<false>;
+  CC_LAUNCH(kern, (unsigned)rows, threads, smem, st, pred, ld, cols, (const long long*)rowptr,
+            colidx, values, row0, scale, out);
   return 0;
 }
diff --git a/cellcomm_b200/csrc/tail_kernels.cu b/cellcomm_b200/csrc/tail_kernels.cu
--- a/cellcomm_b200/csrc/tail_kernels.cu
+++ b/cellcomm_b200/csrc/tail_kernels.cu
@@ -151,6 +151,7 @@
                                float rate, const uint8_t* __restrict__ mask, long long ldm,
                                uint64_t seed, const uint64_t* __restrict__ counter,
                                uint32_t stream_id) {
+  pdl_wait();
   const float scale = 1.f / (1.f - rate);
   const uint64_t step = counter ? *counter : 0;
   for_each_chunk8(rows, cols, [&](long long r, long long c0, int n) {
@@ -174,6 +175,7 @@
 __global__ void dropout_mask_kernel(uint8_t* __restrict__ mask, long long ldm, long long rows,
                                     long long cols, float rate, uint64_t seed,
                                     const uint64_t* __restrict__ counter, uint32_t stream_id) {
+  pdl_wait();
   const uint64_t step = counter ? *counter : 0;
   for_each_chunk8(rows, cols, [&](long long r, long long c0, int n) {
     float u[8];
@@ -185,6 +187,7 @@
 __global__ void uniform_kernel(float* __restrict__ out32, bf16* __restrict__ out16, long long ld,
                                long long rows, long long cols, uint64_t seed,
                                const uint64_t* __restrict__ counter, uint32_t stream_id) {
+  pdl_wait();
   const uint64_t step = counter ? *counter : 0;
   for_each_chunk8(rows, cols, [&](long long r, long long c0, int n) {
     float u[8];
@@ -196,10 +199,14 @@
   });
 }
 
-__global__ void counter_add_kernel(uint64_t* counter, uint64_t inc) { *counter += inc; }
+__global__ void counter_add_kernel(uint64_t* counter, uint64_t inc) {
+  pdl_wait();
+  *counter += inc;
+}
 
 __global__ void act_bwd_kernel(const Mat dy, const Mat y, const Mat dz, long long rows,
                                long long cols, int act) {
+  pdl_wait();
   for_each_chunk8(rows, cols, [&](long long r, long long c0, int n) {
     float g[8], a[8];
     load8(dy, r, c0, n, g);
@@ -214,6 +221,7 @@
 
 __global__ void copy2d_kernel(const Mat src, const Mat dst, long long rows, long long cols,
                               int beta, float scale) {
+  pdl_wait();
   for_each_chunk8(rows, cols, [&](long long r, long long c0, int n) {
     float f[8];
     load8(src, r, c0, n, f);
@@ -231,6 +239,7 @@
 
 __global__ void split_kernel(const Mat x, const Mat hi, const Mat lo, long long rows,
                              long long cols) {
+  pdl_wait();
   for_each_chunk8(rows, cols, [&](long long r, long long c0, int n) {
     float f[8], h[8], l[8];
     load8(x, r, c0, n, f);
@@ -246,6 +255,7 @@
 
 __global__ void round_kernel(const Mat x, const Mat out, float* __restrict__ out32,
                              long long ldo32, long long rows, long long cols) {
+  pdl_wait();
   for_each_chunk8(rows, cols, [&](long long r, long long c0, int n) {
     float f[8];
     load8(x, r, c0, n, f);
@@ -260,6 +270,7 @@
 __global__ void bias_act_kernel(const float* __restrict__ bias, int act, bf16* __restrict__ out16,
                                 long long ld16, float* __restrict__ out32, long long ld32,
                                 long long rows, long long cols) {
+  pdl_wait();
   for (long long i = (long long)blockIdx.x * blockDim.x + threadIdx.x; i < rows * cols;
        i += (long long)gridDim.x * blockDim.x) {
     const long long r = i / cols, c = i - r * cols;
@@ -272,6 +283,7 @@
 }
 
 __global__ void fill_f32_kernel(float* dst, float v, long long n) {
+  pdl_wait();
   for (long long i = (long long)blockIdx.x * blockDim.x + threadIdx.x; i < n;
        i += (long long)gridDim.x * blockDim.x)
     dst[i] = v;
@@ -336,6 +348,7 @@
                  float* __restrict__ out, int accumulate, int act, float* __restrict__ part,
                  unsigned int* __restrict__ tickets,
                  const Mat dz = Mat{nullptr, 0, 0}, const Mat dzlo = Mat{nullptr, 0, 0}) {
+  pdl_wait();
   __shared__ float s0[8][128], s1[8][128];
   const int tx = threadIdx.x, ty = threadIdx.y;
   const long long c = (long long)blockIdx.x * 128 + tx * 4;
@@ -499,14 +512,11 @@
                "(cc_reduce_ws_floats)", rows, cols, (long long)ws_floats, need);
   } else if (gy > 1 && !accumulate && out != nullptr) {
     const long long n = outputs * cols;
-    fill_f32_kernel<<<ew_grid(n, 256), 256, 0, st>>>(out, 0.f, n);
-    CC_CHECK_LAUNCH();
-  }
-  colreduce_kernel<MODE><<<dim3(gx, gy), dim3(32, 8), 0, st>>>(
-      a, b, rows, cols, mean, rstd, out, accumulate, act,
-      fixed ? ws + reduce_tickets() : nullptr, fixed ? reinterpret_cast<unsigned int*>(ws) : nullptr,
-      dz, dzlo);
-  CC_CHECK_LAUNCH();
+    CC_LAUNCH(fill_f32_kernel, ew_grid(n, 256), 256, 0, st, out, 0.f, n);
+  }
+  CC_LAUNCH(colreduce_kernel<MODE>, dim3(gx, gy), dim3(32, 8), 0, st, a, b, rows, cols, mean, rstd,
+            out, accumulate, act, fixed ? ws + reduce_tickets() : nullptr,
+            fixed ? reinterpret_cast<unsigned int*>(ws) : nullptr, dz, dzlo);
   return 0;
 }
 
@@ -514,6 +524,7 @@
                                    float eps, float momentum, float* __restrict__ moving_mean,
                                    float* __restrict__ moving_var, float* __restrict__ save_mean,
                                    float* __restrict__ save_rstd) {
+  pdl_wait();
   const long long c = (long long)blockIdx.x * blockDim.x + threadIdx.x;
   if (c >= cols) return;
   const double mean_d = (double)sums[c] * inv_n;
@@ -530,6 +541,7 @@
                                 const float* __restrict__ gamma, const float* __restrict__ beta,
                                 const float* __restrict__ mean, const float* __restrict__ stat,
                                 int infer, float eps) {
+  pdl_wait();
   for_each_chunk8(rows, cols, [&](long long r, long long c0, int n) {
     float f[8], mu[8], st[8], ga[8], be[8];
     load8(x, r, c0, n, f);
@@ -552,6 +564,7 @@
                                     long long cols, const float* __restrict__ gamma,
                                     const float* __restrict__ mean, const float* __restrict__ rstd,
                                     const float* __restrict__ sums2, float inv_n) {
+  pdl_wait();
   for_each_chunk8(rows, cols, [&](long long r, long long c0, int n) {
     float g[8], a[8], mu[8], rs[8], ga[8], s0[8], s1[8];
     load8(dy, r, c0, n, g);
@@ -574,6 +587,7 @@
 
 __global__ void bn_param_grad_kernel(const float* __restrict__ sums2, long long cols,
                                      float* __restrict__ dgamma, float* __restrict__ dbeta) {
+  pdl_wait();
   const long long c = (long long)blockIdx.x * blockDim.x + threadIdx.x;
   if (c >= cols) return;
   if (dbeta) dbeta[c] = sums2[c];
@@ -583,6 +597,7 @@
 __global__ void bn_infer_bwd_kernel(const Mat dy, const Mat dx, long long rows, long long cols,
                                     const float* __restrict__ gamma,
                                     const float* __restrict__ var, float eps) {
+  pdl_wait();
   for_each_chunk8(rows, cols, [&](long long r, long long c0, int n) {
     float g[8];
     load8(dy, r, c0, n, g);
@@ -595,6 +610,7 @@
 
 __global__ void softmax_fwd_kernel(const Mat x, const Mat y, float* __restrict__ y32,
                                    long long ldy32, long long rows, long long cols) {
+  pdl_wait();
   const long long r = (long long)blockIdx.x * blockDim.x + threadIdx.x;
   if (r >= rows) return;
   float mx = -INFINITY;
@@ -611,6 +627,7 @@
 
 __global__ void softmax_bwd_kernel(const Mat dy, const Mat y, const Mat dx, long long rows,
                                    long long cols) {
+  pdl_wait();
   const long long r = (long long)blockIdx.x * blockDim.x + threadIdx.x;
   if (r >= rows) return;
   float dot = 0.f;
@@ -623,6 +640,7 @@
                                      bf16* __restrict__ out16, long long ldo,
                                      float* __restrict__ out32, long long ldo32, long long rows,
                                      long long cols) {
+  pdl_wait();
   const long long r = (long long)blockIdx.x * blockDim.x + threadIdx.x;
   if (r >= rows) return;
   long long best = 0;
@@ -661,6 +679,7 @@
 __global__ void bce_kernel(const float* __restrict__ x, long long ldx, long long rows,
                            int from_logits, float target, float inv_n,
                            float* __restrict__ loss_out, const Mat dz) {
+  pdl_wait();
   float acc = 0.f;
   for (long long r = threadIdx.x; r < rows; r += blockDim.x) {
     const float raw = x[r * ldx];
@@ -684,6 +703,7 @@
 __global__ void mse_kernel(const Mat pred, const Mat target, long long rows, long long cols,
                            float inv_total, float* __restrict__ loss_out, const Mat dpred,
                            float* __restrict__ part, unsigned int* __restrict__ ticket) {
+  pdl_wait();
   float acc = 0.f;
   for_each_chunk8(rows, cols, [&](long long r, long long c0, int n) {
     float a[8], t[8];
@@ -726,6 +746,7 @@
                                float* __restrict__ mom, long long rows, long long cols,
                                long long ld, float lr, float rho, float momentum, float eps,
                                float grad_scale) {
+  pdl_wait();
   const bool vec = (ld % 4 == 0) && ((((uintptr_t)p32) & 15) == 0) && ((((uintptr_t)g) & 15) == 0) &&
                    ((((uintptr_t)ms) & 15) == 0) && ((((uintptr_t)mom) & 15) == 0) &&
                    (p16 == nullptr || (((uintptr_t)p16) & 7) == 0);
@@ -803,8 +824,7 @@
   do {                                                                                  \
     if ((rows) <= 0 || (cols) <= 0) return 0;                                           \
     const long long _work = (long long)(rows) * (((cols) + 7) / 8);                     \
-    kern<<<ew_grid(_work, 256), 256, 0, ST(stream)>>>(__VA_ARGS__);                     \
-    CC_CHECK_LAUNCH();                                                                  \
+    CC_LAUNCH(kern, ew_grid(_work, 256), 256, 0, ST(stream), __VA_ARGS__);              \
     return 0;                                                                           \
   } while (0)
 
@@ -830,8 +850,7 @@
   if (cols <= 0) return 0;
   if (rows <= 0) {
     if (!beta) {
-      fill_f32_kernel<<<ew_grid(cols, 256), 256, 0, ST(stream)>>>(out, 0.f, cols);
-      CC_CHECK_LAUNCH();
+      CC_LAUNCH(fill_f32_kernel, ew_grid(cols, 256), 256, 0, ST(stream), out, 0.f, cols);
     }
     return 0;
   }
@@ -857,8 +876,7 @@
              "cc_bias_grad: dz_lo needs a bf16 dz (the high-order term)");
   if (rows <= 0) {
     if (!beta && out != nullptr) {
-      fill_f32_kernel<<<ew_grid(cols, 256), 256, 0, ST(stream)>>>(out, 0.f, cols);
-      CC_CHECK_LAUNCH();
+      CC_LAUNCH(fill_f32_kernel, ew_grid(cols, 256), 256, 0, ST(stream), out, 0.f, cols);
     }
     return 0;
   }
@@ -899,8 +917,7 @@
 }
 
 extern "C" int cc_counter_add(uint64_t* counter_dev, uint64_t inc, cc_stream_t stream) {
-  counter_add_kernel<<<1, 1, 0, ST(stream)>>>(counter_dev, inc);
-  CC_CHECK_LAUNCH();
+  CC_LAUNCH(counter_add_kernel, 1, 1, 0, ST(stream), counter_dev, inc);
   return 0;
 }
 
@@ -938,10 +955,8 @@
                                  float* save_rstd, int32_t dtypes, cc_stream_t stream) {
   if (cols <= 0) return 0;
   CC_REQUIRE(n_total > 0, "cc_bn_train_apply: n_total must be positive");
-  bn_finalize_kernel<<<(unsigned)((cols + 255) / 256), 256, 0, ST(stream)>>>(
-      sums, cols, 1.0 / (double)n_total, eps, momentum, moving_mean, moving_var, save_mean,
-      save_rstd);
-  CC_CHECK_LAUNCH();
+  CC_LAUNCH(bn_finalize_kernel, (unsigned)((cols + 255) / 256), 256, 0, ST(stream), sums, cols,
+            1.0 / (double)n_total, eps, momentum, moving_mean, moving_var, save_mean, save_rstd);
   EW_LAUNCH(bn_apply_kernel, rows, cols, stream, mat(x, ldx, F32(dtypes, 0)),
             mat(y, ldy, F32(dtypes, 1)), rows, cols, gamma, beta, save_mean, save_rstd, 0, eps);
 }
@@ -979,9 +994,8 @@
                                cc_stream_t stream) {
   if (cols <= 0) return 0;
   if (dgamma || dbeta) {
-    bn_param_grad_kernel<<<(unsigned)((cols + 255) / 256), 256, 0, ST(stream)>>>(sums2, cols,
-                                                                                 dgamma, dbeta);
-    CC_CHECK_LAUNCH();
+    CC_LAUNCH(bn_param_grad_kernel, (unsigned)((cols + 255) / 256), 256, 0, ST(stream), sums2, cols,
+              dgamma, dbeta);
   }
   if (dx == nullptr) return 0;
   EW_LAUNCH(bn_bwd_apply_kernel, rows, cols, stream, mat(dy, lddy, F32(dtypes, 0)),
@@ -1000,9 +1014,8 @@
                               int64_t ldy32, int64_t rows, int64_t cols, int32_t dtypes,
                               cc_stream_t stream) {
   if (rows <= 0 || cols <= 0) return 0;
-  softmax_fwd_kernel<<<(unsigned)((rows + 127) / 128), 128, 0, ST(stream)>>>(
-      mat(x, ldx, F32(dtypes, 0)), mat(y, ldy, F32(dtypes, 1)), y32, ldy32, rows, cols);
-  CC_CHECK_LAUNCH();
+  CC_LAUNCH(softmax_fwd_kernel, (unsigned)((rows + 127) / 128), 128, 0, ST(stream),
+            mat(x, ldx, F32(dtypes, 0)), mat(y, ldy, F32(dtypes, 1)), y32, ldy32, rows, cols);
   return 0;
 }
 
@@ -1010,10 +1023,9 @@
                               int64_t lddx, int64_t rows, int64_t cols, int32_t dtypes,
                               cc_stream_t stream) {
   if (rows <= 0 || cols <= 0) return 0;
-  softmax_bwd_kernel<<<(unsigned)((rows + 127) / 128), 128, 0, ST(stream)>>>(
-      mat(dy, lddy, F32(dtypes, 0)), mat(y, ldy, F32(dtypes, 1)), mat(dx, lddx, F32(dtypes, 2)),
-      rows, cols);
-  CC_CHECK_LAUNCH();
+  CC_LAUNCH(softmax_bwd_kernel, (unsigned)((rows + 127) / 128), 128, 0, ST(stream),
+            mat(dy, lddy, F32(dtypes, 0)), mat(y, ldy, F32(dtypes, 1)),
+            mat(dx, lddx, F32(dtypes, 2)), rows, cols);
   return 0;
 }
 
@@ -1021,9 +1033,8 @@
                               float target, int64_t n_total, float* loss_out, void* dz,
                               int64_t lddz, int32_t dtypes, cc_stream_t stream) {
   CC_REQUIRE(rows > 0 && n_total > 0, "cc_bce_fwd_bwd: empty batch");
-  bce_kernel<<<1, 256, 0, ST(stream)>>>(x32, ldx, rows, from_logits, target, 1.f / (float)n_total,
-                                        loss_out, mat(dz, lddz, F32(dtypes, 0)));
-  CC_CHECK_LAUNCH();
+  CC_LAUNCH(bce_kernel, 1, 256, 0, ST(stream), x32, ldx, rows, from_logits, target,
+            1.f / (float)n_total, loss_out, mat(dz, lddz, F32(dtypes, 0)));
   return 0;
 }
 
@@ -1049,11 +1060,10 @@
                "(cc_reduce_ws_floats)", (long long)rows, (long long)cols, (long long)ws_floats,
                need);
   }
-  mse_kernel<<<(unsigned)blocks, 256, 0, ST(stream)>>>(
-      mat(pred, ldp, F32(dtypes, 0)), mat(target, ldt, F32(dtypes, 1)), rows, cols, inv_total,
-      loss_out, mat(dpred, lddp, F32(dtypes, 2)), ws ? ws + reduce_tickets() : nullptr,
-      reinterpret_cast<unsigned int*>(ws));
-  CC_CHECK_LAUNCH();
+  CC_LAUNCH(mse_kernel, (unsigned)blocks, 256, 0, ST(stream), mat(pred, ldp, F32(dtypes, 0)),
+            mat(target, ldt, F32(dtypes, 1)), rows, cols, inv_total, loss_out,
+            mat(dpred, lddp, F32(dtypes, 2)), ws ? ws + reduce_tickets() : nullptr,
+            reinterpret_cast<unsigned int*>(ws));
   return 0;
 }
 
@@ -1068,9 +1078,8 @@
                                 float* out32, int64_t ldo32, int64_t rows, int64_t cols,
                                 cc_stream_t stream) {
   if (rows <= 0 || cols <= 0) return 0;
-  argmax_onehot_kernel<<<(unsigned)((rows + 127) / 128), 128, 0, ST(stream)>>>(
-      p32, ldp, (bf16*)out16, ldo, out32, ldo32, rows, cols);
-  CC_CHECK_LAUNCH();
+  CC_LAUNCH(argmax_onehot_kernel, (unsigned)((rows + 127) / 128), 128, 0, ST(stream), p32, ldp,
+            (bf16*)out16, ldo, out32, ldo32, rows, cols);
   return 0;
 }
 
@@ -1087,25 +1096,21 @@
   }
   long long blocks = (work + 255) / 256;
   if (blocks > (long long)num_sms() * bps) blocks = (long long)num_sms() * bps;
-  rmsprop_kernel<<<(unsigned)blocks, 256, 0, ST(stream)>>>(p32, (bf16*)p16, g, ms, mom, rows,
-                                                             cols, ld, lr, rho, momentum, eps,
-                                                             grad_scale);
-  CC_CHECK_LAUNCH();
+  CC_LAUNCH(rmsprop_kernel, (unsigned)blocks, 256, 0, ST(stream), p32, (bf16*)p16, g, ms, mom, rows,
+            cols, ld, lr, rho, momentum, eps, grad_scale);
   return 0;
 }
 
 extern "C" int cc_bias_act(const float* bias, int32_t act, void* out16, int64_t ld16, float* out32,
                            int64_t ld32, int64_t rows, int64_t cols, cc_stream_t stream) {
   if (rows <= 0 || cols <= 0) return 0;
-  bias_act_kernel<<<ew_grid(rows * cols, 256), 256, 0, ST(stream)>>>(bias, act, (bf16*)out16, ld16,
-                                                                    out32, ld32, rows, cols);
-  CC_CHECK_LAUNCH();
+  CC_LAUNCH(bias_act_kernel, ew_grid(rows * cols, 256), 256, 0, ST(stream), bias, act, (bf16*)out16,
+            ld16, out32, ld32, rows, cols);
   return 0;
 }
 
 extern "C" int cc_fill_f32(float* dst, float value, int64_t n, cc_stream_t stream) {
   if (n <= 0) return 0;
-  fill_f32_kernel<<<ew_grid(n, 256), 256, 0, ST(stream)>>>(dst, value, n);
-  CC_CHECK_LAUNCH();
+  CC_LAUNCH(fill_f32_kernel, ew_grid(n, 256), 256, 0, ST(stream), dst, value, n);
   return 0;
 }
diff --git a/cellcomm_b200/csrc/wgrad_rmsprop_kernel.cuh b/cellcomm_b200/csrc/wgrad_rmsprop_kernel.cuh
--- a/cellcomm_b200/csrc/wgrad_rmsprop_kernel.cuh
+++ b/cellcomm_b200/csrc/wgrad_rmsprop_kernel.cuh
@@ -7,6 +7,16 @@
   CUtensorMap b[MAX_SEG];
   CUtensorMap p32, ms, mom, p16;
 };
+
+__device__ __forceinline__ void prefetch_tmaps(const RmsMaps& maps, int nseg) {
+  for (int s = 0; s < nseg; ++s) {
+    prefetch_tmap(&maps.a[s]);
+    prefetch_tmap(&maps.b[s]);
+  }
+  prefetch_tmap(&maps.p32);
+  prefetch_tmap(&maps.ms);
+  prefetch_tmap(&maps.mom);
+}
 
 __device__ __forceinline__ uint64_t l2_evict_first_policy() {
   uint64_t pol;
@@ -219,6 +229,7 @@
     for (int w = 0; w < EPI_WARPS; ++w) mbar_init(state_bar(w), 1);
     asm volatile("fence.mbarrier_init.release.cluster;" ::: "memory");
     asm volatile("fence.proxy.async.shared::cta;" ::: "memory");
+    prefetch_tmaps(maps, p.nseg);
   }
   if (warp == 1) {
     asm volatile("tcgen05.alloc.cta_group::1.sync.aligned.shared::cta.b32 [%0], %1;" ::"r"(tmem_slot),
@@ -231,6 +242,7 @@
   if (CLUSTER == 2) cluster_sync_all();
   tcgen05_fence_after();
   const uint32_t tmem_acc = *tmem_slot_ptr;
+  pdl_wait();
 
   if (warp == 0) {
     uint32_t it = 0;
@@ -386,6 +398,7 @@
     for (int w = 0; w < EPI_WARPS; ++w) mbar_init(state_bar(w), 1);
     asm volatile("fence.mbarrier_init.release.cluster;" ::: "memory");
     asm volatile("fence.proxy.async.shared::cta;" ::: "memory");
+    prefetch_tmaps(maps, p.nseg);
   }
   if (warp == 1) {
     asm volatile("tcgen05.alloc.cta_group::2.sync.aligned.shared::cta.b32 [%0], %1;" ::"r"(tmem_slot),
@@ -398,6 +411,7 @@
   cluster_sync_all();
   tcgen05_fence_after();
   const uint32_t tmem_acc = *tmem_slot_ptr;
+  pdl_wait();
 
   if (warp == 0) {
     uint32_t it = 0;
```

After: 58380, median of 6. Within noise of the previous version (+0.1%).
